# kaftanski/fissure-segmentation

Measured on AMD Instinct MI355X. Metric: points/sec fwd+bwd DGCNN-seg N=2048 k=20, higher is better.
Workload: dtype f32

## Files before the change

### fissure-segmentation_amd/_lib.py

```python
import ctypes
import os

import torch

_HERE = os.path.dirname(os.path.abspath(__file__))
LIB_PATH = os.environ.get("FSG_HIP_LIB") or os.path.join(_HERE, "libfsg_hip.so")

if not os.path.exists(LIB_PATH):
    raise ImportError(f"{LIB_PATH} not found: build it with `python -c 'import __graft_entry__ as g; g.build()'` "
                      f"or `make -C {os.path.join(_HERE, 'csrc')}`; there is no CPU fallback.")

lib = ctypes.CDLL(LIB_PATH)

_P, _I, _L, _F = ctypes.c_void_p, ctypes.c_int, ctypes.c_int64, ctypes.c_float
SIGNATURES = {
    "fsg_version": ([], _I),
    "fsg_last_error": ([], ctypes.c_char_p),
    "fsg_knn_dense_f32": ([_P, _I, _I, _L, _L, _I, _I, _I, _P, _P, _P, _P], _I),
    "fsg_knn_dense_workspace_bytes": ([_I, _I, _I], ctypes.c_size_t),
    "fsg_knn_dense_ws_f32": ([_P, _I, _I, _L, _L, _I, _I, _I, _P, _P, _P, ctypes.c_size_t, _P], _I),
    "fsg_knn_dense_prepared_f32": ([_P, _I, _I, _I, _I, _I, _P, _P, _P, ctypes.c_size_t, _P], _I),
    "fsg_knn_dense_ws_pq_f32": ([_P, _I, _I, _L, _L, _I, _I, _I, _P, _P, _P, ctypes.c_size_t, _P, _I, _P, _P], _I),
    "fsg_edgeconv_apply_f32": ([_P, _P, _P, _P, _P, _I, _I, _I, _F, _P, _P, _P, ctypes.c_size_t, _P], _I),
    "fsg_edgeconv_apply_pq_f32": ([_P, _P, _P, _P, _P, _I, _I, _I, _F, _P, _P, _P, ctypes.c_size_t, _P, _I, _P, _P], _I),
    "fsg_edge_gather_fwd_f32": ([_P, _P, _P, _I, _I, _I, _I, _P], _I),
    "fsg_edge_gather_bwd_f32": ([_P, _P, _P, _I, _I, _I, _I, _P], _I),
    "fsg_knn_gather_fused_f32": ([_P, _I, _I, _I, _I, _I, _P, _P, _P, _P], _I),
    "fsg_knn_gather_fused_ws_f32": ([_P, _I, _I, _I, _I, _I, _P, _P, _P, ctypes.c_size_t, _P], _I),
    "fsg_edge_gather_fwd_bf16": ([_P, _P, _P, _I, _I, _I, _I, _P], _I),
    "fsg_edge_gather_bwd_bf16": ([_P, _P, _P, _I, _I, _I, _I, _P], _I),
    "fsg_graph_reverse_csr_workspace_bytes": ([_I, _I, _I], ctypes.c_size_t),
    "fsg_graph_reverse_csr": ([_P, _I, _I, _I, _P, _P, _P, _P], _I),
    "fsg_edge_weights_fwd_f32": ([_P, _I, _I, _P, _P], _I),
    "fsg_edge_weights_bwd_f32": ([_P, _I, _I, _P, _P], _I),
    "fsg_edge_weights_many_f32": ([_P, _I, _P], _I),
    "fsg_edgeconv1_workspace_bytes": ([_I, _I, _I], ctypes.c_size_t),
    "fsg_edgeconv1_fwd_f32": ([_P, _P, _P, _P, _P, _P, _I, _I, _I, _I, _I, _F, _F, _F, _P, _P, _P, _P, _P, _P, _P, _P, _P],
                              _I),
    "fsg_edgeconv1_bwd_f32": ([_P, _P, _L, _P, _L, _P, _P, _P, _P, _P, _P, _P, _P, _P, _P, _I, _I, _I, _I, _I, _F, _P, _P,
                               _P, _P, _P, _P], _I),
    "fsg_edgeconv2_workspace_bytes": ([_I, _I, _I, _I], ctypes.c_size_t),
    "fsg_edgeconv2_bwd_workspace_bytes": ([_I, _I, _I, _I], ctypes.c_size_t),
    "fsg_edgeconv2_fwd_f32": ([_P] * 11 + [_I] * 5 + [_F] * 5 + [_P] * 12, _I),
    "fsg_edgeconv2_bwd_f32": ([_P, _P, _L, _P, _L] + [_P] * 16 + [_I] * 5 + [_F] + [_P] * 8, _I),
    "fsg_edgeconv2_fwd_bf16": ([_P] * 11 + [_I] * 5 + [_F] * 5 + [_P] * 12, _I),
    "fsg_edgeconv2_bwd_bf16": ([_P, _P, _L, _P, _L] + [_P] * 16 + [_I] * 5 + [_F] + [_P] * 8, _I),
    "fsg_bn_act_workspace_bytes": ([ctypes.c_long, _I], ctypes.c_size_t),
    "fsg_bn_act_fwd_f32": ([_P, _P, _P, _P, _P, ctypes.c_long, _I, _I, _F, _F, _F, _P, _P, _P, _P, _P], _I),
    "fsg_bn_act_bwd_f32": ([_P, _P, _P, _P, _P, _P, ctypes.c_long, _I, _I, _F, _P, _P, _P, _P, _P], _I),
    "fsg_bn_act_max_workspace_bytes": ([_I, _I, _I], ctypes.c_size_t),
    "fsg_bn_act_max_fwd_f32": ([_P, _P, _P, _P, _P, _I, _I, _I, _I, _F, _F, _F, _P, _P, _P, _P, _P, _P, _P], _I),
    "fsg_bn_act_max_bwd_f32": ([_P, _P, _P, _P, _P, _P, _P, _P, _I, _I, _I, _I, _F, _P, _P, _P, _P], _I),
    "fsg_bn_act_maxavg_workspace_bytes": ([_I, _I, _I], ctypes.c_size_t),
    "fsg_bn_act_maxavg_fwd_f32": ([_P, _P, _P, _P, _P, _I, _I, _I, _I, _F, _F, _F, _P, _P, _P, _P, _P, _P], _I),
    "fsg_bn_act_maxavg_bwd_f32": ([_P, _P, _P, _P, _P, _P, _P, _I, _I, _I, _I, _F, _P, _P, _P, _P, _P], _I),
    "fsg_chamfer_nn_f32": ([_P, _P, _I, _I, _I, _P, _P, _P], _I),
    "fsg_chamfer_nn_bwd_workspace_bytes": ([_I, _I, _I], ctypes.c_size_t),
    "fsg_chamfer_nn_bwd_f32": ([_P, _P, _P, _P, _I, _I, _I, _P, _P, _P, _P], _I),
    "fsg_point_mesh_dist_f32": ([_P, _P, _P, _I, _I, _I, _I, _I, _P, _P, _P, _P], _I),
    "fsg_mesh_labelmap_dist_f32": ([_P, _P, _P, _I, _I, _I, _I, _I, _F, _F, _F, _F, _P, _P, _P, _P], _I),
    "fsg_mesh_labelmap_cover_f32": ([_P, _P, _P, _I, _I, _I, _I, _I, _F, _F, _F, _P, _P], _I),
    "fsg_ensemble_accumulate_workspace_bytes": ([_I, _L], ctypes.c_size_t),
    "fsg_ensemble_accumulate_f32": ([_P, _I, _I, _I, _I, _P, _L, _P, _P, _P], _I),
    "fsg_sample_transform_f32": ([_P, _I, _I, _L, _P, _I, _P, _P, _P], _I),
    "fsg_ssm_decode_bwd_workspace_bytes": ([_I, _I, _I], ctypes.c_size_t),
    "fsg_ssm_decode_fwd_f32": ([_P, _P, _P, _P, _P, _P, _I, _I, _I, _P, _P], _I),
    "fsg_ssm_decode_bwd_f32": ([_P, _P, _P, _P, _P, _P, _I, _I, _I, _P, _P, _P, _P, _P, ctypes.c_size_t, _P], _I),
    "fsg_colsum_narrow_f32": ([_P, _L, _I, _P, _P], _I),
    "fsg_fold_layer1_f32": ([_P, _I, _P, _L, _P, _I, _I, _I, _I, _P, _P], _I),
    "fsg_adam_flat_f32": ([_P, _P, _P, _P, _P, _L, _F, _P, _F, _F, _F, _F, _P], _I),
    "fsg_nnu_loss_workspace_bytes": ([_I], ctypes.c_size_t),
    "fsg_nnu_loss_f32": ([_P, _L, _L, _L, _P, _P, _I, _I, _I, _F, _F, _F, _P, _P, _L, _L, _L, _P, _P], _I),
    "fsg_bn_rows_workspace_bytes": ([ctypes.c_long, _I], ctypes.c_size_t),
    "fsg_bn_rows_fwd_f32": ([_P, _P, _P, _P, _P, _P, ctypes.c_long, _I, _I, _F, _F, _I, _P, _P, _P, _P, _P], _I),
    "fsg_bn_rows_bwd_f32": ([_P, _P, _P, _P, _P, _P, ctypes.c_long, _I, _I, _I, _P, _P, _P, _P, _P, _P], _I),
    "fsg_gemm_small_workspace_bytes": ([_I, _I, _I], ctypes.c_size_t),
    "fsg_gemm_small_f32": ([_P, _L, _L, _P, _L, _L, _P, _P, _L, _I, _I, _I, _P, _P], _I),
    "fsg_gemm_small_rowsum_f32": ([_P, _L, _L, _P, _L, _L, _P, _P, _L, _I, _I, _I, _P, _P, _P], _I),
    "fsg_gemm_small_deferred_f32": ([_P, _L, _L, _P, _L, _L, _P, _L, _I, _I, _I, _P, _P, _P, _P], _I),
    "fsg_gemm_small_reduce_many_f32": ([_P, _P], _I),
    "fsg_gemm_small_bf16": ([_P, _L, _L, _P, _L, _L, _P, _P, _L, _I, _I, _I, _P, _P, _P, _P], _I),
    "fsg_pt_attn_workspace_bytes": ([_I, _I, _I], ctypes.c_size_t),
    "fsg_pt_attn_fwd_f32": ([_P, _P, _P, _P, _P, _L, _P, _I, _I, _I, _I, _P, _P, _P, _P, _P, _P], _I),
    "fsg_pt_attn_bwd_f32": ([_P, _P, _P, _P, _P, _L, _P, _I, _I, _I, _I, _P, _P, _P, _P, _P, _P, _P, _L, _P, _P, _P, _P], _I),
    "fsg_knn_segment_f32": ([_P, _P, _P, _P, _I, _I, _I, _I, _P, _P, _P], _I),
    "fsg_fps_f32": ([_P, _P, _P, _I, _I, _P, _P, _P], _I),
    "fsg_group_gather_fwd_f32": ([_P, _P, _P, _I, _I, _I, _I, _P], _I),
    "fsg_group_gather_bwd_f32": ([_P, _P, _P, _I, _I, _I, _I, _P], _I),
    "fsg_group_xyz_feat_fwd_f32": ([_P, _P, _P, _P, _P, _I, _I, _I, _I, _P], _I),
    "fsg_group_xyz_feat_bwd_f32": ([_P, _P, _P, _I, _I, _I, _I, _P], _I),
    "fsg_rows_max_fwd_f32": ([_P, _P, _P, _I, _I, _I, _P], _I),
    "fsg_rows_max_bwd_f32": ([_P, _P, _P, _I, _I, _I, _P], _I),
    "fsg_interp_fwd_f32": ([_P, _P, _P, _P, _I, _I, _I, _I, _P], _I),
    "fsg_interp_bwd_f32": ([_P, _P, _P, _P, _I, _I, _I, _I, _P], _I),
    "fsg_vec_attn_fwd_f32": ([_P, _P, _P, _P, _P, _I, _I, _I, _I, _P], _I),
    "fsg_vec_attn_bwd_f32": ([_P, _P, _P, _P, _P, _P, _P, _P, _I, _I, _I, _I, _P], _I),
    "fsg_pw_weight_image_bytes": ([_I, _I], ctypes.c_size_t),
    "fsg_pw_weight_image_f32": ([_P, _L, _L, _I, _I, _F, _I, _I, _P, _P], _I),
# ... 60 lines not shown
    "fsg_pcl_normals_f32": ([_P, _P, _P, _I, _I, _I, _I, _P, _P, _P, _P], _I),
    "fsg_orient_normals_workspace_bytes": ([_I, _I], ctypes.c_size_t),
    "fsg_orient_normals_f32": ([_P, _P, _P, _P, _I, _I, _I, _P, ctypes.c_size_t, _P, _P, _P, _P], _I),
    "fsg_face_union_i32": ([_P, _P, _I, _P, _P, _P], _I),
    "fsg_cluster_stats_f64": ([_P, _P, _P, _P, _P, _I, _I, _I, _P, _P, _P, _P], _I),
    "fsg_mesh_keep_flags_u8": ([_P, _I, _P, _I, _P, _P, _P, _I, _I, _I, _F, _F, _F, _P, _P], _I),
    "fsg_mesh_face_flags_u8": ([_P, _I, _I, _P, _P, _P, _P, _P], _I),
    "fsg_mesh_compact_f32": ([_P, _P, _P, _I, _I, _P, _I, _P, _P, _P, _P, _P, _P, _P, _P], _I),
}
for _name, (_args, _res) in SIGNATURES.items():
    _fn = getattr(lib, _name)
    _fn.argtypes, _fn.restype = _args, _res

GRID_TORCH, GRID_SAP = 0, 1
MORPH_MAX_RADIUS = 8
PCL_NORMALS_MAX_K = 64
ORIENT_MAX_POINTS = 1 << 20
RW_BINARY, RW_INTENSITY, RW_MAX_LABELS = 0, 1, 8
KNN_FIX_DIAG, KNN_DROP_FIRST, KNN_FORCE_ROWS, KNN_FORCE_MFMA, KNN_MAX_K = 1, 2, 4, 8, 64
KNN_DBG_HALF_CHUNKS, KNN_DBG_TWO_PHASE, KNN_DBG_ALL_SLOW, KNN_DBG_STATS = 1 << 11, 1 << 21, 1 << 22, 1 << 25
KNN_DBG_STAMPS, KNN_DBG_ONE_LAUNCH, KNN_DBG_BF16 = 1 << 28, 1 << 29, 1 << 30


_timing = None


def start_timing():
    global _timing
    _timing = {}


def stop_timing():
    global _timing
    rec, _timing = _timing, None
    torch.cuda.synchronize()
    return {name: [s.elapsed_time(e) for s, e in evs] for name, evs in (rec or {}).items()}


class PTLayerParams(ctypes.Structure):
    _fields_ = [(n, _P) for n in ("lp1_w", "lp1_b", "bnp_g", "bnp_b", "bnp_rm", "bnp_rv", "lp2_w", "lp2_b", "bn1_g", "bn1_b",
                                  "bn1_rm", "bn1_rv", "lw1_w", "lw1_b", "bn2_g", "bn2_b", "bn2_rm", "bn2_rv", "lw2_w",
                                  "lw2_b")] + [(n, _F) for n in ("eps_p", "eps_1", "eps_2", "mom_p", "mom_1", "mom_2")]


GEMM_REDUCE_MAX_JOBS = 48


class GemmReduceJobs(ctypes.Structure):
    _fields_ = [("part", _P * GEMM_REDUCE_MAX_JOBS), ("C", _P * GEMM_REDUCE_MAX_JOBS), ("rowsum", _P * GEMM_REDUCE_MAX_JOBS),
                ("ldc", _L * GEMM_REDUCE_MAX_JOBS), ("S", _I * GEMM_REDUCE_MAX_JOBS), ("I", _I * GEMM_REDUCE_MAX_JOBS),
                ("J", _I * GEMM_REDUCE_MAX_JOBS), ("blocks", _I * GEMM_REDUCE_MAX_JOBS), ("n", _I)]


class EdgeWeightJobs(ctypes.Structure):
    _fields_ = [("src", _P * 8), ("dst", _P * 8), ("Co", _I * 8), ("C", _I * 8), ("n", _I)]


class PWRowGemmArgs(ctypes.Structure):
    _fields_ = [("A1", _P), ("Y1", _P), ("A2", _P), ("lda1", _L), ("lda2", _L), ("K1", _I), ("K2", _I), ("Bimg", _P),
                ("M", _I), ("N", _I), ("rows_per_cloud", _I), ("alpha", _P), ("delta", _P), ("P", _P), ("Q", _P),
                ("tstride", _I), ("slope", _F), ("C", _P), ("ldc", _L), ("store_n0", _I), ("bias", _P), ("rec", _P),
                ("sgn", _P), ("sel_val", _P), ("sel_arg", _P), ("sel_n", _I), ("Yp", _P), ("ldyp", _L), ("ealpha", _P),
                ("edelta", _P), ("emu", _P), ("er", _P), ("etstride", _I), ("rec2", _P)]


PW_MAX_IMAGE_JOBS = 10


class PWImageJobs(ctypes.Structure):
    _fields_ = [("W", _P * PW_MAX_IMAGE_JOBS), ("stride_n", _L * PW_MAX_IMAGE_JOBS), ("stride_k", _L * PW_MAX_IMAGE_JOBS),
                ("N", _I * PW_MAX_IMAGE_JOBS), ("K", _I * PW_MAX_IMAGE_JOBS), ("ks0", _I * PW_MAX_IMAGE_JOBS),
                ("KS", _I * PW_MAX_IMAGE_JOBS), ("scale", _F * PW_MAX_IMAGE_JOBS), ("image", _P * PW_MAX_IMAGE_JOBS), ("n", _I)]


PW_MAX_REDUCE_JOBS = 6


class PWTnReduceJobs(ctypes.Structure):
    _fields_ = [("workspace", _P * PW_MAX_REDUCE_JOBS), ("C1", _P * PW_MAX_REDUCE_JOBS), ("C2", _P * PW_MAX_REDUCE_JOBS),
                ("ldc1", _L * PW_MAX_REDUCE_JOBS), ("ldc2", _L * PW_MAX_REDUCE_JOBS), ("S", _I * PW_MAX_REDUCE_JOBS),
                ("N1", _I * PW_MAX_REDUCE_JOBS), ("N2", _I * PW_MAX_REDUCE_JOBS), ("N1a", _I * PW_MAX_REDUCE_JOBS), ("n", _I)]


class PWTnArgs(ctypes.Structure):
    _fields_ = [("L1", _P), ("LY1", _P), ("L2", _P), ("ldl1", _L), ("ldl2", _L), ("N1a", _I), ("N1b", _I), ("lpro", _I),
                ("lalpha", _P), ("ldelta", _P), ("lP", _P), ("lQ", _P), ("lts", _I), ("R", _P), ("ldr", _L), ("N2", _I),
                ("rpro", _I), ("ralpha", _P), ("rdelta", _P), ("rts", _I), ("slope", _F), ("M", _I), ("rows_per_cloud", _I),
                ("rows_per_slice", _I), ("ones", _I)]


class PTLayerGrads(ctypes.Structure):
    _fields_ = [(n, _P) for n in ("lp1_w", "lp1_b", "bnp_g", "bnp_b", "lp2_w", "lp2_b", "bn1_g", "bn1_b", "lw1_w", "lw1_b",
                                  "bn2_g", "bn2_b", "lw2_w", "lw2_b")]


_experiments = None


def experiments():
    global _experiments
    if _experiments is None:
        path = os.path.join(_HERE, "libfsg_hip_experiments.so")
        if not os.path.exists(path):
            raise ImportError(f"{path} not found: `make -C {os.path.join(_HERE, 'csrc')} all` builds it")
        x = ctypes.CDLL(path)
        x.fsg_knn_experiment_f32.argtypes, x.fsg_knn_experiment_f32.restype = SIGNATURES["fsg_knn_dense_f32"][0], _I
# ... 22 lines not shown
```

### fissure-segmentation_amd/csrc/edgeconv.hip

```cpp
#include <type_traits>

#include "edgeconv_internal.h"
#include "knn_internal.h"

namespace {

constexpr int TP = 16;
constexpr int FSG_CSR_SPLIT = 16;
constexpr int TPW = 2;

__global__ __launch_bounds__(1024) void csr_build_kernel(const int32_t *__restrict__ idx, int N, int k,
                                                          int32_t *__restrict__ rowptr, int32_t *__restrict__ col) {
    extern __shared__ int sh[];
    int *hist = sh;
    int *part = sh + N;
    const int b = blockIdx.x, tid = threadIdx.x;
    const long NK = (long)N * k;
    const int32_t *ib = idx + b * NK;
    for (int j = tid; j < N; j += 1024) hist[j] = 0;
    __syncthreads();
    for (long e0 = tid; e0 < NK; e0 += 8 * 1024) {
        int dst[8];
#pragma unroll
        for (int u = 0; u < 8; ++u) dst[u] = (e0 + u * 1024 < NK) ? ib[e0 + u * 1024] : -1;
// ... 151 lines not shown
    for (long e = e0 + tid; e < e1; e += 1024) {
        const int pos = atomicAdd(&sh[ib[e]], 1);
        const int i = (int)(e / k), sl = (int)(e - (long)i * k);
        col[b * NK + pos] = (i << 6) | sl;
    }
}

constexpr int CSR_SORT_CAP = 1024;
__global__ __launch_bounds__(256) void csr_sort_rows_kernel(const int32_t *__restrict__ rowptr, int32_t *__restrict__ col, int N,
                                                            int NK, int32_t *__restrict__ tmp) {
    __shared__ int32_t buf[4][CSR_SORT_CAP];
    const int b = blockIdx.y, wave = __builtin_amdgcn_readfirstlane(threadIdx.x >> 6), lane = threadIdx.x & 63;
    const int j = blockIdx.x * 4 + wave;
    if (j >= N) return;
    const int32_t *rp = rowptr + (long)b * (N + 1);
    const int beg = rp[j], deg = rp[j + 1] - beg;
    if (deg < 2) return;
    int32_t *row = col + (long)b * NK + beg;
    if (deg > CSR_SORT_CAP) {
        if (!tmp) return;
        int32_t *cp = tmp + (long)b * NK + beg;
        for (int t = lane; t < deg; t += 64) cp[t] = row[t];
        __threadfence_block();
        __builtin_amdgcn_wave_barrier();
        for (int t0 = 0; t0 < deg; t0 += 64) {
            const int t = t0 + lane;
            const int32_t e = t < deg ? __builtin_nontemporal_load(cp + t) : 0x7fffffff;
            int rank = 0;
            for (int u = 0; u < deg; ++u) rank += __builtin_nontemporal_load(cp + u) < e ? 1 : 0;
            if (t < deg) row[rank] = e;
        }
        return;
    }
    int32_t *mine = buf[wave];
    for (int t = lane; t < deg; t += 64) mine[t] = row[t];
    __builtin_amdgcn_wave_barrier();
    for (int t0 = 0; t0 < deg; t0 += 64) {
        const int t = t0 + lane;
        const int32_t e = t < deg ? mine[t] : 0x7fffffff;
        int rank = 0;
#pragma unroll 8
        for (int u = 0; u < deg; ++u) rank += mine[u] < e ? 1 : 0;
        if (t < deg) row[rank] = e;
    }
}

template <bool SELECT>
__global__ __launch_bounds__(512) void ec1_stats_select_kernel(const float *__restrict__ pq,
                                                                const int32_t *__restrict__ idx,
                                                                const float *__restrict__ gamma, int N, int k, int Co,
                                                                int training, float *__restrict__ ysel,
                                                                uint8_t *__restrict__ arg, float *__restrict__ ssum,
                                                                float *__restrict__ partials) {
    typedef f32x2 f2;
    typedef f32x4 f4;
    typedef u32x4 u4;
    constexpr int NW = 4 * TPW;
    __shared__ float red[2][4 * NW][64];
    const int b = blockIdx.x, tile = blockIdx.y, cg = blockIdx.z;
    const int lane = threadIdx.x & 63, wave = __builtin_amdgcn_readfirstlane(threadIdx.x >> 6);
    const int g = lane >> 4, c16 = lane & 15;
    const int c0 = cg * 64 + 4 * c16;
    const int ld = 2 * Co;
    const __amdgpu_buffer_rsrc_t rs = buffer_rsrc(pq + (long)b * N * ld, __builtin_amdgcn_readfirstlane((int)((long)N * ld * 4)));
    f2 sgn[2] = {{1.f, 1.f}, {1.f, 1.f}};
    if (SELECT) {
        const f4 gm = *reinterpret_cast<const f4 *>(gamma + c0);
        sgn[0] = f2{gm[0] >= 0.f ? 1.f : -1.f, gm[1] >= 0.f ? 1.f : -1.f};
        sgn[1] = f2{gm[2] >= 0.f ? 1.f : -1.f, gm[3] >= 0.f ? 1.f : -1.f};
    }
    const int i = tile * TP * TPW + wave * (TP / 4) + g;
    const bool live = i < N;
    const int ic = live ? i : N - 1;
    int ids[4] = {0, 0, 0, 0};
#pragma unroll
    for (int r = 0; r < 4; ++r)
        if (16 * r < k) ids[r] = (16 * r + c16 < k) ? idx[((long)b * N + ic) * k + 16 * r + c16] : 0;
    const f4 q4 = __builtin_bit_cast(f4, __builtin_amdgcn_raw_buffer_load_b128(
        rs, (unsigned)ic * (unsigned)(ld * 4) + (unsigned)((Co + c0) * 4), 0, 0));
    const f2 q[2] = {{q4[0], q4[1]}, {q4[2], q4[3]}};
    f2 tot[2] = {{0.f, 0.f}, {0.f, 0.f}}, shift[2] = {{0.f, 0.f}, {0.f, 0.f}}, s1[2] = {{0.f, 0.f}, {0.f, 0.f}},
       s2[2] = {{0.f, 0.f}, {0.f, 0.f}};
    float best[4] = {-INFINITY, -INFINITY, -INFINITY, -INFINITY};
    int barg[4] = {0, 0, 0, 0};
    constexpr int RB = SELECT ? 8 : 10;
    auto request = [&](int s0, u4 (&y)[RB]) {
#pragma unroll
        for (int u = 0; u < RB; ++u) {
            const int s = min(s0 + u, k - 1);
            const int r = s >> 4;
            const int held = r == 0 ? ids[0] : (r == 1 ? ids[1] : (r == 2 ? ids[2] : ids[3]));
            const int j = __builtin_amdgcn_ds_bpermute(4 * ((lane & 48) | (s & 15)), held);
            y[u] = __builtin_amdgcn_raw_buffer_load_b128(rs, (unsigned)j * (unsigned)(ld * 4) + (unsigned)(c0 * 4), 0, 0);
        }
    };
    auto consume = [&](int s0, const u4 (&y)[RB]) {
#pragma unroll
        for (int u = 0; u < RB; ++u) {
            const int s = s0 + u;
            if (s < k) {
                const f4 yv = __builtin_bit_cast(f4, y[u]);
#pragma unroll
                for (int hf = 0; hf < 2; ++hf) {
                    const f2 yy = f2{yv[2 * hf], yv[2 * hf + 1]} + q[hf];
                    tot[hf] += yy;
                    if (training) {
                        if (s == 0) shift[hf] = yy;
                        const f2 d = yy - shift[hf];
                        s1[hf] += d;
                        s2[hf] = __builtin_elementwise_fma(d, d, s2[hf]);
                    }
                    if (SELECT) {
                        const f2 v = sgn[hf] * yy;
#pragma unroll
                        for (int e = 0; e < 2; ++e)
                            if (v[e] > best[2 * hf + e]) { best[2 * hf + e] = v[e]; barg[2 * hf + e] = s; }
                    }
                }
            }
        }
    };
    u4 ya[RB], yb[RB];
    request(0, ya);
    for (int s0 = 0; s0 < k; s0 += 2 * RB) {
        if (s0 + RB < k) request(s0 + RB, yb);
        consume(s0, ya);
        if (s0 + 2 * RB < k) request(s0 + 2 * RB, ya);
        if (s0 + RB < k) consume(s0 + RB, yb);
    }
    if (live) {
        const long o = ((long)b * N + i) * Co + c0;
        if (SELECT) {
            *reinterpret_cast<f4 *>(ysel + o) = f4{sgn[0][0] * best[0], sgn[0][1] * best[1], sgn[1][0] * best[2], sgn[1][1] * best[3]};
            *reinterpret_cast<unsigned *>(arg + o) =
                (unsigned)barg[0] | ((unsigned)barg[1] << 8) | ((unsigned)barg[2] << 16) | ((unsigned)barg[3] << 24);
        }
        if (ssum) *reinterpret_cast<f4 *>(ssum + o) = f4{tot[0][0], tot[0][1], tot[1][0], tot[1][1]};
    }
    if (!training) return;
#pragma unroll
    for (int e = 0; e < 4; ++e) {
        const float s1e = s1[e >> 1][e & 1], s2e = s2[e >> 1][e & 1], she = shift[e >> 1][e & 1];
        red[0][wave * 4 + g][4 * c16 + e] = she + s1e / (float)k;
        red[1][wave * 4 + g][4 * c16 + e] = fmaxf(s2e - s1e * s1e / (float)k, 0.f);
    }
    __syncthreads();
    if (wave == 0) {
        const int c = cg * 64 + lane;
        const int live_groups = min(4 * NW, max(0, N - tile * TP * TPW));
        float sm = 0.f, sM = 0.f;
#pragma unroll 8
        for (int w = 0; w < 4 * NW; ++w) {
            const bool on = w < live_groups;
            sm += on ? red[0][w][lane] : 0.f;
            sM += on ? red[1][w][lane] : 0.f;
        }
        const float mu = live_groups > 0 ? sm / (float)live_groups : 0.f;
        float dev = 0.f;
#pragma unroll 8
        for (int w = 0; w < 4 * NW; ++w) {
            const float d = red[0][w][lane] - mu;
            dev = __builtin_fmaf(w < live_groups ? d : 0.f, d, dev);
        }
        const long rec = (long)b * gridDim.y + tile;
        float *pr = partials + rec * 3 * Co;
        pr[c] = (float)live_groups * (float)k;
        pr[Co + c] = mu;
        pr[2 * Co + c] = sM + (float)k * dev;
    }
}

constexpr int FIN_S = 16;

constexpr int FIN_CH = 8, FIN_SL = 128;
__global__ __launch_bounds__(FIN_CH * FIN_SL) void bn_finalize_kernel(const float *__restrict__ partials, int R, int Co,
                                                                      float eps, float momentum,
                                                                      float *__restrict__ mean_out,
                                                                      float *__restrict__ invstd_out,
                                                                      float *__restrict__ running_mean,
                                                                      float *__restrict__ running_var) {
    __shared__ double red[3][FIN_SL][FIN_CH];
    const int ch = threadIdx.x & (FIN_CH - 1), sl = threadIdx.x / FIN_CH;
    const int c = blockIdx.x * FIN_CH + ch;
    double a = 0.0, bm = 0.0, cm = 0.0;
    for (int r0 = sl; r0 < R; r0 += 4 * FIN_SL) {
        float nv[4], mv[4], qv[4];
#pragma unroll
        for (int u = 0; u < 4; ++u) {
            const int r = min(r0 + u * FIN_SL, R - 1);
            const float *pr = partials + (long)r * 3 * Co + c;
            nv[u] = pr[0];
            mv[u] = pr[Co];
            qv[u] = pr[2 * Co];
        }
#pragma unroll
        for (int u = 0; u < 4; ++u)
            if (r0 + u * FIN_SL < R) {
                const double n = nv[u], mu = mv[u];
                a += n;
                bm += n * mu;
                cm += (double)qv[u] + n * mu * mu;
            }
    }
    red[0][sl][ch] = a;
    red[1][sl][ch] = bm;
    red[2][sl][ch] = cm;
    __syncthreads();
    __shared__ double red2[3][16][FIN_CH];
    if (sl < 16) {
        double x0 = 0.0, x1 = 0.0, x2 = 0.0;
#pragma unroll
        for (int u = 0; u < 8; ++u) {
            x0 += red[0][8 * sl + u][ch];
            x1 += red[1][8 * sl + u][ch];
            x2 += red[2][8 * sl + u][ch];
        }
        red2[0][sl][ch] = x0;
        red2[1][sl][ch] = x1;
        red2[2][sl][ch] = x2;
    }
    __syncthreads();
// ... 474 lines not shown
    const int j = blockIdx.y;
    const int Co = jobs.Co[j], C = jobs.C[j];
    const int t = blockIdx.x * 256 + threadIdx.x;
    if (t >= 2 * Co * C) return;
    const float *src = jobs.src[j];
    float *dst = jobs.dst[j];
    if (!backward) {
        const int r = t / C, c = t - r * C;
        dst[t] = r < Co ? src[(long)r * 2 * C + c] : src[(long)(r - Co) * 2 * C + C + c] - src[(long)(r - Co) * 2 * C + c];
    } else {
        const int r = t / (2 * C), c2 = t - r * 2 * C;
        dst[t] = c2 < C ? src[(long)r * C + c2] - src[(long)(Co + r) * C + c2] : src[(long)(Co + r) * C + (c2 - C)];
    }
}

extern "C" int fsg_edge_weights_many_f32(const fsg_edge_weight_jobs *jobs, int backward, fsg_stream_t stream) {
    FSG_REQUIRE(jobs && jobs->n >= 1 && jobs->n <= FSG_EDGE_WEIGHT_MAX_JOBS, "fsg_edge_weights_many_f32: 1..%d jobs",
                FSG_EDGE_WEIGHT_MAX_JOBS);
    long most = 0;
    for (int j = 0; j < jobs->n; ++j) {
        FSG_REQUIRE(jobs->src[j] && jobs->dst[j] && jobs->Co[j] > 0 && jobs->C[j] > 0, "fsg_edge_weights_many_f32: bad job %d", j);
        const long e = 2L * jobs->Co[j] * jobs->C[j];
        most = e > most ? e : most;
    }
    hipLaunchKernelGGL(edge_weights_many_kernel, dim3(fsg_cdiv(most, 256), jobs->n), dim3(256), 0, (hipStream_t)stream, *jobs,
                       backward);
    FSG_CHECK_LAUNCH("fsg_edge_weights_many_f32");
    return FSG_OK;
}

extern "C" int fsg_edge_weights_fwd_f32(const float *W, int Co, int C, float *Wt, fsg_stream_t stream) {
    FSG_REQUIRE(W && Wt && Co > 0 && C > 0, "fsg_edge_weights_fwd_f32: bad arguments");
    hipLaunchKernelGGL(edge_weights_fwd_kernel, dim3(fsg_cdiv(2L * Co * C, 256)), dim3(256), 0, (hipStream_t)stream, W, Co, C, Wt);
    FSG_CHECK_LAUNCH("fsg_edge_weights_fwd_f32");
    return FSG_OK;
}
extern "C" int fsg_edge_weights_bwd_f32(const float *grad_Wt, int Co, int C, float *grad_W, fsg_stream_t stream) {
    FSG_REQUIRE(grad_Wt && grad_W && Co > 0 && C > 0, "fsg_edge_weights_bwd_f32: bad arguments");
    hipLaunchKernelGGL(edge_weights_bwd_kernel, dim3(fsg_cdiv(2L * Co * C, 256)), dim3(256), 0, (hipStream_t)stream, grad_Wt, Co,
                       C, grad_W);
    FSG_CHECK_LAUNCH("fsg_edge_weights_bwd_f32");
    return FSG_OK;
}

extern "C" size_t fsg_edgeconv1_workspace_bytes(int B, int N, int Co) {
    const size_t rec = (size_t)B * (size_t)fsg_cdiv(N, TP * TPW);
    return sizeof(float) * (rec * 3 * (size_t)Co + fsg_ec_finalize_stage_floats(Co));
}

extern "C" int fsg_edgeconv1_fwd_f32(const float *pq, const int32_t *idx, const float *gamma, const float *beta,
                                     float *running_mean, float *running_var, int B, int N, int k, int Co, int training,
                                     float momentum, float eps, float slope, float *out, float *out_pm, float *ysel,
                                     uint8_t *arg, float *ssum, float *mean, float *invstd, float *workspace,
                                     fsg_stream_t stream) {
    FSG_REQUIRE(pq && idx && gamma && beta && ysel && arg && mean && invstd, "fsg_edgeconv1_fwd_f32: NULL pointer");
    FSG_REQUIRE(B > 0 && N > 0 && k > 0 && k <= 64 && Co > 0 && Co % 64 == 0 && B <= 65535,
                "fsg_edgeconv1_fwd_f32: bad shape B=%d N=%d k=%d Co=%d (Co must be a multiple of 64)", B, N, k, Co);
    FSG_REQUIRE(!training || workspace, "fsg_edgeconv1_fwd_f32: training needs the workspace");
    FSG_REQUIRE((long)N * 2 * Co * 4 < (1L << 31), "fsg_edgeconv1_fwd_f32: a cloud's [P | Q] rows must stay below 2 GiB (N=%d, Co=%d)", N, Co);
    hipStream_t st = (hipStream_t)stream;
    const int tiles = fsg_cdiv(N, TP * TPW);
    hipLaunchKernelGGL(ec1_stats_select_kernel<true>, dim3(B, tiles, Co / 64), dim3(256 * TPW), 0, st, pq, idx, gamma, N, k, Co,
                       training, ysel, arg, ssum, workspace);
    FSG_CHECK_LAUNCH("fsg_edgeconv1_fwd_f32/stats");
    if (training) {
        const int rc = fsg_ec_finalize_launch(workspace, B * tiles, Co, eps, momentum, mean, invstd, running_mean,
                                              running_var, st);
        if (rc != FSG_OK) return rc;
    }
    if (!out) return FSG_OK;
    hipLaunchKernelGGL(ec1_apply_kernel, dim3(B, fsg_cdiv(N, 64), Co / 64), dim3(256), 0, st, ysel, gamma, beta, mean,
                       invstd, N, Co, slope, out, out_pm);
    FSG_CHECK_LAUNCH("fsg_edgeconv1_fwd_f32/apply");
    return FSG_OK;
}

extern "C" int fsg_edgeconv_apply_f32(const float *ysel, const float *gamma, const float *beta, const float *mean,
                                      const float *invstd, int B, int N, int Co, float slope, float *out, float *out_pm,
                                      void *knn_workspace, size_t knn_workspace_bytes, fsg_stream_t stream) {
    FSG_REQUIRE(ysel && gamma && beta && mean && invstd && out, "fsg_edgeconv_apply_f32: NULL pointer");
    FSG_REQUIRE(B > 0 && N > 0 && Co > 0 && Co % 64 == 0 && B <= 65535, "fsg_edgeconv_apply_f32: bad shape B=%d N=%d Co=%d", B, N, Co);
    if (knn_workspace)
        return fsg_ec_apply_prep_launch(ysel, gamma, beta, mean, invstd, B, N, Co, slope, out, out_pm, knn_workspace,
                                        knn_workspace_bytes, nullptr, nullptr, (hipStream_t)stream);
    return fsg_ec_apply_launch(ysel, gamma, beta, mean, invstd, B, N, Co, slope, out, out_pm, (hipStream_t)stream);
}

extern "C" int fsg_edgeconv_apply_pq_f32(const float *ysel, const float *gamma, const float *beta, const float *mean,
                                         const float *invstd, int B, int N, int Co, float slope, float *out, float *out_pm,
                                         void *knn_workspace, size_t knn_workspace_bytes, const float *w_next, int rows_next,
                                         float *pq_next, fsg_stream_t stream) {
    FSG_REQUIRE(ysel && gamma && beta && mean && invstd && out && out_pm && knn_workspace && w_next && pq_next,
                "fsg_edgeconv_apply_pq_f32: NULL pointer");
    FSG_REQUIRE(B > 0 && N > 0 && Co == 64 && rows_next == 128 && B <= 65535,
                "fsg_edgeconv_apply_pq_f32: bad shape B=%d N=%d Co=%d rows_next=%d (Co must be 64, the next block 64 wide)", B, N, Co,
                rows_next);
    return fsg_ec_apply_prep_launch(ysel, gamma, beta, mean, invstd, B, N, Co, slope, out, out_pm, knn_workspace,
                                    knn_workspace_bytes, w_next, pq_next, (hipStream_t)stream);
}

extern "C" int fsg_edgeconv1_bwd_f32(const float *grad_out, const float *grad_out_pm, int64_t ld_pm, const float *grad_out_pm2,
                                     int64_t ld_pm2, const float *pq, const int32_t *rowptr, const int32_t *col,
                                     const float *gamma, const float *beta, const float *mean, const float *invstd,
                                     const float *ysel, const uint8_t *arg, const float *ssum, int B, int N, int k,
                                     int Co, int training, float slope, float *grad_pq, float *grad_gamma,
                                     float *grad_beta, float *h_scratch, float *workspace, fsg_stream_t stream) {
    FSG_REQUIRE((grad_out || grad_out_pm || grad_out_pm2) && pq && rowptr && col && gamma && beta && mean && invstd && ysel &&
                    arg && grad_pq && grad_gamma && grad_beta && h_scratch && workspace,
                "fsg_edgeconv1_bwd_f32: NULL pointer");
    FSG_REQUIRE((!grad_out_pm || ld_pm >= Co) && (!grad_out_pm2 || ld_pm2 >= Co),
                "fsg_edgeconv1_bwd_f32: row stride of a point-major gradient below Co=%d", Co);
    FSG_REQUIRE(!training || ssum, "fsg_edgeconv1_bwd_f32: training needs ssum");
    FSG_REQUIRE(B > 0 && N > 0 && k > 0 && k <= 64 && Co > 0 && Co % 64 == 0 && B <= 65535,
                "fsg_edgeconv1_bwd_f32: bad shape B=%d N=%d k=%d Co=%d", B, N, k, Co);
    hipStream_t st = (hipStream_t)stream;
    const int tiles64 = fsg_cdiv(N, 64);
    hipLaunchKernelGGL(ec1_bwd_point_kernel, dim3(B, tiles64, Co / 64), dim3(256), 0, st, grad_out, grad_out_pm, (long)ld_pm,
// ... 13 lines not shown
```

### fissure-segmentation_amd/csrc/edgeconv2.hip

```cpp

#include "edgeconv_internal.h"

namespace {

__device__ __forceinline__ bf16x8 pack8(const float (&v)[8]) {
    bf16x8 r;
#pragma unroll
    for (int i = 0; i < 8; ++i) r[i] = (__bf16)v[i];
    return r;
}

constexpr int C1 = 64;
constexpr int LD1 = C1 + 1;
constexpr int MAXPAIR = 3;

struct Tile {
    int TP, R, Rpad;
};

template <int C2, bool BF>
__global__ __launch_bounds__(256) void ec2_fwd_kernel(const float *__restrict__ pq, const int32_t *__restrict__ idx,
                                                       const float *__restrict__ w2, const float *__restrict__ gamma1,
                                                       const float *__restrict__ beta1, const float *__restrict__ mean1,
                                                       const float *__restrict__ invstd1,
// ... 1022 lines not shown
static void ec2s_tiling(int k, int B, int N, bool bwd, bool bf16, int &RT, int &TP, int &G) {
    const int tp2 = 64 / k, tp4 = 128 / k;
    const float u2 = tp2 * k / 64.f, u4 = tp4 * k / 128.f;
    RT = u4 > 1.15f * u2 ? 4 : 2;
    if (!bwd && !bf16) RT = 2;
    TP = RT == 4 ? tp4 : tp2;
    if (TP < 1) TP = 1;
    if (TP > 16) TP = 16;
    const int ntiles = (N + TP - 1) / TP;
    G = (bwd ? 512 : 768) / (B > 0 ? B : 1);
    if (G < 1) G = 1;
    if (G > ntiles) G = ntiles;
}

static size_t ec2s_fwd_lds(int NP, int RT, int TP) {
    return (size_t)NP * RT * 32 * 128 + sizeof(float) * ((size_t)RT * 32 * 65 + 3 * 4 * 64 + 2 * C1 + 2 * (size_t)TP * C1);
}
static size_t ec2s_bwd_lds(int NP, int RT, int TP) {
    return (size_t)2 * NP * RT * 32 * 128 +
           sizeof(float) * ((size_t)RT * 32 * (C1 + 4) + 2 * 64 + 64 + 2 * C1 + (size_t)TP * 64 * 2 + 2 * (size_t)TP * C1);
}

static void ec2_tiling(int k, int C2, int &TP, int &Rpad, int &G, int B, int N) {
    TP = 64 / k;
    if (TP < 1) TP = 1;
    Rpad = (TP * k + 31) & ~31;
    const int ntiles = (N + TP - 1) / TP;
    G = 1024 / (B > 0 ? B : 1);
    if (G < 1) G = 1;
    if (G > ntiles) G = ntiles;
}

extern "C" size_t fsg_edgeconv2_workspace_bytes(int B, int N, int k, int C2) {
    int TP, Rpad, G;
    ec2_tiling(k, C2, TP, Rpad, G, B, N);
    if (ec2_split(C2)) {
        int RT, TPs, Gs;
        ec2s_tiling(k, B, N, false, false, RT, TPs, Gs);
        { int RTb, TPb, Gb; ec2s_tiling(k, B, N, false, true, RTb, TPb, Gb); if (Gb > Gs) Gs = Gb; }
        if (Gs > G) G = Gs;
    }
    const size_t rec1 = (size_t)fsg_ec_stats1_records(B, N) * 3 * C1 + fsg_ec_finalize_stage_floats(C1);
    const size_t rec2 = (size_t)B * G * 3 * C2 + fsg_ec_finalize_stage_floats(C2);
    const size_t scratch1 = (size_t)B * N * C1 * sizeof(float) + (size_t)B * N * C1;
    return sizeof(float) * (rec1 + rec2) + scratch1 + 256;
}

static int ec2_fwd_impl(bool bf16, const float *pq, const int32_t *idx, const float *w2, const float *gamma1,
                                     const float *beta1, float *running_mean1, float *running_var1, const float *gamma2,
                                     const float *beta2, float *running_mean2, float *running_var2, int B, int N, int k,
                                     int C2, int training, float momentum1, float momentum2, float eps1, float eps2,
                                     float slope, float *out, float *out_pm, float *ssum1, float *mean1, float *invstd1,
                                     float *ysel2, uint8_t *arg2, float *ssum2, float *mean2, float *invstd2,
                                     void *workspace, fsg_stream_t stream) {
    FSG_REQUIRE(pq && idx && w2 && gamma1 && beta1 && gamma2 && beta2 && mean1 && invstd1 && ysel2 && arg2 &&
                    mean2 && invstd2 && workspace,
                "fsg_edgeconv2_fwd_f32: NULL pointer");
    FSG_REQUIRE(B > 0 && N > 0 && N <= (1 << 21) && k > 0 && k <= 64 && (C2 == 64 || C2 == 128) && B <= 65535,
                "fsg_edgeconv2_fwd_f32: bad shape B=%d N=%d k=%d C2=%d (layer widths 64 -> 64|128 only, N <= 2^21)", B, N, k, C2);
    FSG_REQUIRE(!training || (ssum1 && ssum2), "fsg_edgeconv2_fwd_f32: training needs ssum1/ssum2");
    hipStream_t st = (hipStream_t)stream;
    int TP, Rpad, G;
    ec2_tiling(k, C2, TP, Rpad, G, B, N);
    int RTs = 0, TPs = 0, Gs = 0, Gws = G;
    if (ec2_split(C2)) {
        ec2s_tiling(k, B, N, false, bf16, RTs, TPs, Gs);
        if (Gs > Gws) Gws = Gs;
    }
    const int rec1 = fsg_ec_stats1_records(B, N);
    float *part1 = (float *)workspace;
    float *part2 = part1 + (size_t)rec1 * 3 * C1 + fsg_ec_finalize_stage_floats(C1);
    float *ysel1 = part2 + (size_t)B * Gws * 3 * C2 + fsg_ec_finalize_stage_floats(C2);
    uint8_t *arg1 = (uint8_t *)(ysel1 + (size_t)B * N * C1);
    int rc;
    if (training) {
        if ((rc = fsg_ec_stats1_launch(pq, idx, gamma1, B, N, k, C1, ysel1, arg1, ssum1, part1, st)) != FSG_OK) return rc;
        if ((rc = fsg_ec_finalize_launch(part1, rec1, C1, eps1, momentum1, mean1, invstd1, running_mean1, running_var1,
                                         st)) != FSG_OK)
            return rc;
    }
    const size_t lds = sizeof(float) * ((size_t)C2 * LD1 + (size_t)Rpad * (C2 + 1) + 3 * 4 * C2);
#define FSG_EC2_FWD(CC, BFX)                                                                                             \
    do {                                                                                                                 \
        FSG_GRANT_LDS("fsg_edgeconv2_fwd", (ec2_fwd_kernel<CC, BFX>), FSG_LDS_WHOLE_CU);                             \
        hipLaunchKernelGGL((ec2_fwd_kernel<CC, BFX>), dim3(B, G), dim3(256), lds, st, pq, idx, w2, gamma1, beta1, mean1,    \
                           invstd1, gamma2, N, k, TP, Rpad, training, slope, ysel2, arg2, ssum2, part2);                 \
    } while (0)
#define FSG_EC2S_FWD(NPX, RTX)                                                                                            \
    do {                                                                                                                 \
        FSG_GRANT_LDS("fsg_edgeconv2_fwd", (ec2s_fwd_kernel<NPX, RTX>), FSG_LDS_WHOLE_CU);                           \
        hipLaunchKernelGGL((ec2s_fwd_kernel<NPX, RTX>), dim3(B, G), dim3(256), ec2s_fwd_lds(NPX, RTX, TPs), st, pq, idx, w2,    \
                           gamma1, beta1, mean1, invstd1, gamma2, N, k, TPs, training, slope, ysel2, arg2, ssum2, part2); \
    } while (0)
    if (ec2_split(C2)) {
        G = Gs;
        if (bf16) { if (RTs == 4) FSG_EC2S_FWD(1, 4); else FSG_EC2S_FWD(1, 2); }
        else { if (RTs == 4) FSG_EC2S_FWD(3, 4); else FSG_EC2S_FWD(3, 2); }
    } else if (C2 == 64) { if (bf16) FSG_EC2_FWD(64, true); else FSG_EC2_FWD(64, false); }
    else { if (bf16) FSG_EC2_FWD(128, true); else FSG_EC2_FWD(128, false); }
#undef FSG_EC2_FWD
#undef FSG_EC2S_FWD
    FSG_CHECK_LAUNCH("fsg_edgeconv2_fwd_f32/mlp");
    if (training) {
        if ((rc = fsg_ec_finalize_launch(part2, B * G, C2, eps2, momentum2, mean2, invstd2, running_mean2, running_var2,
                                         st)) != FSG_OK)
            return rc;
    }
    if (!out) return FSG_OK;
    return fsg_ec_apply_launch(ysel2, gamma2, beta2, mean2, invstd2, B, N, C2, slope, out, out_pm, st);
}

extern "C" int fsg_edgeconv2_fwd_f32(const float *pq, const int32_t *idx, const float *w2, const float *gamma1,
                                     const float *beta1, float *running_mean1, float *running_var1, const float *gamma2,
                                     const float *beta2, float *running_mean2, float *running_var2, int B, int N, int k,
                                     int C2, int training, float momentum1, float momentum2, float eps1, float eps2,
                                     float slope, float *out, float *out_pm, float *ssum1, float *mean1, float *invstd1,
                                     float *ysel2, uint8_t *arg2, float *ssum2, float *mean2, float *invstd2,
                                     void *workspace, fsg_stream_t stream) {
    return ec2_fwd_impl(false, pq, idx, w2, gamma1, beta1, running_mean1, running_var1, gamma2, beta2, running_mean2, running_var2, B, N, k, C2, training, momentum1, momentum2, eps1, eps2, slope, out, out_pm, ssum1, mean1, invstd1, ysel2, arg2, ssum2, mean2, invstd2, workspace, stream);
}

extern "C" int fsg_edgeconv2_fwd_bf16(const float *pq, const int32_t *idx, const float *w2, const float *gamma1,
                                     const float *beta1, float *running_mean1, float *running_var1, const float *gamma2,
                                     const float *beta2, float *running_mean2, float *running_var2, int B, int N, int k,
                                     int C2, int training, float momentum1, float momentum2, float eps1, float eps2,
                                     float slope, float *out, float *out_pm, float *ssum1, float *mean1, float *invstd1,
                                     float *ysel2, uint8_t *arg2, float *ssum2, float *mean2, float *invstd2,
                                     void *workspace, fsg_stream_t stream) {
    return ec2_fwd_impl(true, pq, idx, w2, gamma1, beta1, running_mean1, running_var1, gamma2, beta2, running_mean2, running_var2, B, N, k, C2, training, momentum1, momentum2, eps1, eps2, slope, out, out_pm, ssum1, mean1, invstd1, ysel2, arg2, ssum2, mean2, invstd2, workspace, stream);
}

static void ec2_bwd_tiling(int k, int C2, int &TP, int &Rpad, int &G, int B, int N) {
    TP = 64 / k;
    if (TP < 1) TP = 1;
    Rpad = (TP * k + 31) & ~31;
    const int ntiles = (N + TP - 1) / TP;
    G = 768 / (B > 0 ? B : 1);
    if (G < 1) G = 1;
    if (G > ntiles) G = ntiles;
}

extern "C" size_t fsg_edgeconv2_bwd_workspace_bytes(int B, int N, int k, int C2) {
    int TP, Rpad, G;
    ec2_bwd_tiling(k, C2, TP, Rpad, G, B, N);
    if (ec2_split(C2)) {
        int RT, TPs, Gs;
        ec2s_tiling(k, B, N, true, false, RT, TPs, Gs);
        if (Gs > G) G = Gs;
    }
    const size_t point_rec = (size_t)B * fsg_cdiv(N, 64) * 2 * C2;
    const size_t dw = (size_t)B * G * C2 * C1, p1 = (size_t)B * G * 2 * C1;
    const size_t du = (size_t)B * N * k * C1;
    return sizeof(float) * (point_rec + dw + p1 + du + (size_t)B * N * C2) + 256;
}

static int ec2_bwd_impl(bool bf16, const float *grad_out, const float *grad_out_pm, int64_t ld_pm, const float *grad_out_pm2,
                                     int64_t ld_pm2, const float *pq, const int32_t *idx,
                                     const int32_t *rowptr, const int32_t *col, const float *w2, const float *gamma1,
                                     const float *beta1, const float *mean1, const float *invstd1, const float *ssum1,
                                     const float *gamma2, const float *beta2, const float *mean2, const float *invstd2,
                                     const float *ysel2, const uint8_t *arg2, int B, int N, int k, int C2, int training,
                                     float slope, float *grad_pq, float *grad_w2, float *grad_gamma1, float *grad_beta1,
                                     float *grad_gamma2, float *grad_beta2, void *workspace, fsg_stream_t stream) {
    FSG_REQUIRE((!grad_out_pm || ld_pm >= C2) && (!grad_out_pm2 || ld_pm2 >= C2),
                "fsg_edgeconv2_bwd_f32: row stride of a point-major gradient below C2=%d", C2);
    FSG_REQUIRE((grad_out || grad_out_pm || grad_out_pm2) && pq && idx && rowptr && col && w2 && gamma1 && beta1 && mean1 && invstd1 &&
                    gamma2 && beta2 && mean2 && invstd2 && ysel2 && arg2 && grad_pq && grad_w2 && grad_gamma1 &&
                    grad_beta1 && grad_gamma2 && grad_beta2 && workspace,
                "fsg_edgeconv2_bwd_f32: NULL pointer");
    FSG_REQUIRE(!training || ssum1, "fsg_edgeconv2_bwd_f32: training needs ssum1");
    FSG_REQUIRE(B > 0 && N > 0 && N <= (1 << 21) && k > 0 && k <= 64 && (C2 == 64 || C2 == 128) && B <= 65535,
                "fsg_edgeconv2_bwd_f32: bad shape B=%d N=%d k=%d C2=%d (N <= 2^21)", B, N, k, C2);
    hipStream_t st = (hipStream_t)stream;
    int TP, Rpad, G;
    ec2_bwd_tiling(k, C2, TP, Rpad, G, B, N);
    int RTs = 0, TPs = 0, Gs = 0, Gws = G;
    if (ec2_split(C2)) {
        ec2s_tiling(k, B, N, true, bf16, RTs, TPs, Gs);
        if (Gs > Gws) Gws = Gs;
    }
    float *point_part = (float *)workspace;
    float *dw_part = point_part + (size_t)B * fsg_cdiv(N, 64) * 2 * C2;
// ... 65 lines not shown
```

### fissure-segmentation_amd/csrc/edgeconv_internal.h

```cpp
#pragma once
#include "fsg_common.h"

int fsg_ec_stats1_records(int B, int N);
int fsg_ec_stats1_launch(const float *pq, const int32_t *idx, const float *gamma, int B, int N, int k, int Co,
                         float *ysel, uint8_t *arg, float *ssum, float *partials, hipStream_t st);
int fsg_ec_apply_launch(const float *ysel, const float *gamma, const float *beta, const float *mean, const float *invstd,
                        int B, int N, int Co, float slope, float *out, float *out_pm, hipStream_t st);
int fsg_ec_apply_prep_launch(const float *ysel, const float *gamma, const float *beta, const float *mean, const float *invstd,
                             int B, int N, int Co, float slope, float *out, float *out_pm, void *knn_ws, size_t knn_ws_bytes,
                             const float *w_next, float *pq_next, hipStream_t st);
int fsg_ec_bwd_point_launch(const float *gout, const float *gout_pm, long ld_pm, const float *gout_pm2, long ld_pm2,
                            const float *ysel, const float *gamma, const float *beta, const float *mean, const float *invstd,
                            int B, int N, int Co, float slope, float *h, float *partials, float *dbeta, float *dgamma,
                            hipStream_t st);

size_t fsg_ec_finalize_stage_floats(int Co);
int fsg_ec_finalize_launch(const float *partials, int R, int Co, float eps, float momentum, float *mean, float *invstd,
                           float *running_mean, float *running_var, hipStream_t st);
int fsg_ec_sum_launch(const float *partials, int R, int L, int nvec, float *out0, float *out1, hipStream_t st);

int fsg_csr_bipartite_launch(const int32_t *idx, int B, int NS, int N, int k, int32_t *rowptr, int32_t *col, int32_t *cnt,
                             int32_t *tmp, hipStream_t st);
```

### fissure-segmentation_amd/csrc/knn_dense.hip

```cpp
#include <float.h>

#include <stdlib.h>

#include <type_traits>

#include "knn_internal.h"

namespace {

constexpr int BLOCK = 256;

template <int QB>
__global__ __launch_bounds__(BLOCK) void knn_dense_rows_kernel(
    const float *__restrict__ x, int N, int Npad, long sb, long sc, int c_knn, int k, int flags,
    int32_t *__restrict__ idx_out, float *__restrict__ dist_out) {
    extern __shared__ __attribute__((aligned(16))) float smem[];
    float *qv = smem;
    float *xxq = qv + c_knn * QB;
    float *rows = smem + (((c_knn * QB + QB) + 3) & ~3);

    const int b = blockIdx.y;
    const int q0 = blockIdx.x * QB;
    const int tid = threadIdx.x;
    const float *xb = x + (long)b * sb;
// ... 54 lines not shown
                if (v.z < bd) { bd = v.z; bj = j + 2; }
                if (v.w < bd) { bd = v.w; bj = j + 3; }
            }
#pragma unroll
            for (int off = 32; off >= 1; off >>= 1) {
                const float od = __shfl_xor(bd, off);
                const int oj = __shfl_xor(bj, off);
                if (od < bd || (od == bd && oj < bj)) { bd = od; bj = oj; }
            }
            if (lane == 0) {
                if (bj < N) row[bj] = INFINITY;
                if (r >= drop) {
                    const long o = ((long)b * N + qg) * k + (r - drop);
                    idx_out[o] = bj < N ? bj : 0;
                    if (dist_out) dist_out[o] = bd;
                }
            }
            __builtin_amdgcn_wave_barrier();
        }
    }
}

}

extern "C" size_t fsg_knn_dense_workspace_bytes(int B, int N, int c_knn) {
    if (B <= 0 || N <= 0 || c_knn <= 0) return 0;
    const size_t xxb = sizeof(float) * (size_t)B * N, sp = fsg_knn_split_workspace_bytes(B, N, c_knn);
    return sp > xxb ? sp : xxb;
}

extern "C" int fsg_knn_dense_ws_f32(const float *x, int B, int N, int64_t stride_b, int64_t stride_c, int c_knn, int k,
                                    int flags, int32_t *idx_out, float *dist_out, void *workspace,
                                    size_t workspace_bytes, fsg_stream_t stream) {
    const int drop = (flags & FSG_KNN_DROP_FIRST) ? 1 : 0;
    FSG_KNN_REQUIRE_FLAGS("fsg_knn_dense_ws_f32", flags);
    FSG_REQUIRE(x && idx_out, "fsg_knn_dense_ws_f32: NULL pointer");
    FSG_REQUIRE(B >= 0 && N > 0 && c_knn > 0, "fsg_knn_dense_ws_f32: bad shape B=%d N=%d c_knn=%d", B, N, c_knn);
    FSG_REQUIRE(k >= 1 && k + drop <= N && k + drop <= FSG_KNN_MAX_K,
                "fsg_knn_dense_ws_f32: need 1 <= k and k+drop <= min(N, %d); got k=%d N=%d", FSG_KNN_MAX_K, k, N);
    FSG_REQUIRE(workspace == nullptr || workspace_bytes >= sizeof(float) * (size_t)B * N,
                "fsg_knn_dense_ws_f32: workspace of %zu bytes is smaller than the (B,N) squared norms", workspace_bytes);
    if (B == 0) return FSG_OK;
    if (workspace && !(flags & KNN_BYPASS_SPLIT)) {
        const int rc = fsg_knn_split_launch(x, B, N, stride_b, stride_c, c_knn, k, flags, idx_out, dist_out, workspace,
                                            workspace_bytes, (hipStream_t)stream);
        if (rc != FSG_ERR_UNSUPPORTED) return rc;
    }
    return fsg_knn_dense_f32(x, B, N, stride_b, stride_c, c_knn, k, flags & ~KNN_DBG_TWO_PHASE, idx_out, dist_out,
                             static_cast<float *>(workspace), stream);
}

extern "C" int fsg_knn_dense_ws_pq_f32(const float *x, int B, int N, int64_t stride_b, int64_t stride_c, int c_knn, int k,
                                       int flags, int32_t *idx_out, float *dist_out, void *workspace, size_t workspace_bytes,
                                       const float *w_pq, int rows_pq, float *pq_out, fsg_stream_t stream) {
    FSG_KNN_REQUIRE_FLAGS("fsg_knn_dense_ws_pq_f32", flags);
    FSG_REQUIRE(x && idx_out && w_pq && pq_out, "fsg_knn_dense_ws_pq_f32: NULL pointer");
    FSG_REQUIRE(c_knn >= 1 && c_knn <= 4 && rows_pq >= 1 && 256 % rows_pq == 0,
                "fsg_knn_dense_ws_pq_f32: needs 1 <= c_knn <= 4 and rows_pq dividing 256; got c_knn=%d rows_pq=%d", c_knn, rows_pq);
    const int drop = (flags & FSG_KNN_DROP_FIRST) ? 1 : 0;
    FSG_REQUIRE(B >= 0 && N > 0 && k >= 1 && k + drop <= N && k + drop <= FSG_KNN_MAX_K, "fsg_knn_dense_ws_pq_f32: bad shape B=%d N=%d k=%d",
                B, N, k);
    if (B == 0) return FSG_OK;
    hipStream_t st = (hipStream_t)stream;
    if (workspace && !(flags & KNN_BYPASS_SPLIT)) {
        bool fused = false;
        KnnSplitOpts o;
        o.pq_w = w_pq, o.pq_rows = rows_pq, o.pq_out = pq_out, o.pq_fused = &fused;
        const int rc = fsg_knn_split_launch(x, B, N, stride_b, stride_c, c_knn, k, flags, idx_out, dist_out, workspace, workspace_bytes,
                                            st, o);
        if (rc == FSG_OK) return fused ? FSG_OK : fsg_knn_pq_rows_launch(x, B, N, stride_b, stride_c, c_knn, w_pq, rows_pq, pq_out, st);
        if (rc != FSG_ERR_UNSUPPORTED) return rc;
    }
    const int rc = fsg_knn_dense_ws_f32(x, B, N, stride_b, stride_c, c_knn, k, flags, idx_out, dist_out, workspace, workspace_bytes,
                                        stream);
    if (rc != FSG_OK) return rc;
    return fsg_knn_pq_rows_launch(x, B, N, stride_b, stride_c, c_knn, w_pq, rows_pq, pq_out, st);
}

extern "C" int fsg_knn_dense_prepared_f32(const float *x_pm, int B, int N, int c_knn, int k, int flags, int32_t *idx_out,
                                          float *dist_out, void *workspace, size_t workspace_bytes, fsg_stream_t stream) {
    const int drop = (flags & FSG_KNN_DROP_FIRST) ? 1 : 0;
    FSG_KNN_REQUIRE_FLAGS("fsg_knn_dense_prepared_f32", flags);
    FSG_REQUIRE(x_pm && idx_out && workspace, "fsg_knn_dense_prepared_f32: NULL pointer");
    FSG_REQUIRE(B > 0 && N > 0 && c_knn > 0 && k >= 1 && k + drop <= N && k + drop <= FSG_KNN_MAX_K,
                "fsg_knn_dense_prepared_f32: bad shape B=%d N=%d c_knn=%d k=%d", B, N, c_knn, k);
    KnnSplitOpts o;
    o.prepared_xt = x_pm;
    const int rc = fsg_knn_split_launch(nullptr, B, N, 0, 0, c_knn, k, flags, idx_out, dist_out, workspace, workspace_bytes,
                                        (hipStream_t)stream, o);
    if (rc == FSG_ERR_UNSUPPORTED) fsg_set_error("fsg_knn_dense_prepared_f32: shape outside the prepared path's envelope");
    return rc;
}

extern "C" int fsg_knn_dense_f32(const float *x, int B, int N, int64_t stride_b, int64_t stride_c,
                                 int c_knn, int k, int flags, int32_t *idx_out, float *dist_out,
                                 float *xx_scratch, fsg_stream_t stream) {
    const int drop = (flags & FSG_KNN_DROP_FIRST) ? 1 : 0;
    FSG_KNN_REQUIRE_FLAGS("fsg_knn_dense_f32", flags);
    FSG_REQUIRE(x && idx_out, "fsg_knn_dense_f32: NULL pointer");
    FSG_REQUIRE(B >= 0 && N > 0 && c_knn > 0, "fsg_knn_dense_f32: bad shape B=%d N=%d c_knn=%d", B, N, c_knn);
    FSG_REQUIRE(k >= 1 && k + drop <= N && k + drop <= FSG_KNN_MAX_K,
                "fsg_knn_dense_f32: need 1 <= k and k+drop <= min(N, %d); got k=%d N=%d", FSG_KNN_MAX_K, k, N);
    FSG_REQUIRE(N <= 32768, "fsg_knn_dense_f32: N=%d > 32768 unsupported", N);
    if (B == 0) return FSG_OK;
    hipStream_t st = (hipStream_t)stream;
    FSG_REQUIRE(!(flags & FSG_KNN_FORCE_MFMA),
                "fsg_knn_dense_f32: flags %d select an experimental kernel: call fsg_knn_experiment_f32 of "
                "libfsg_hip_experiments.so", flags);
    if (!(flags & FSG_KNN_FORCE_ROWS)) {
        const int rc = fsg_knn_rows_mfma_launch(x, B, N, stride_b, stride_c, c_knn, k, flags, idx_out, dist_out, xx_scratch, st);
        if (rc != FSG_ERR_UNSUPPORTED) return rc;
    }
    const int Npad = (N + 255) & ~255;
    auto launch = [&](auto qb) -> int {
        constexpr int QB = decltype(qb)::value;
        const auto kern = knn_dense_rows_kernel<QB>;
        const size_t lds = sizeof(float) * ((((size_t)c_knn * QB + QB + 3) & ~(size_t)3) + (size_t)QB * Npad);
        if (lds > 160 * 1024) {
            fsg_set_error("fsg_knn_dense_f32: LDS need %zu B > 160 KiB (N=%d c_knn=%d)", lds, N, c_knn);
            return FSG_ERR_UNSUPPORTED;
        }
        FSG_GRANT_LDS("fsg_knn_dense_f32", kern, lds);
        dim3 grid(fsg_cdiv(N, QB), B);
        hipLaunchKernelGGL(kern, grid, dim3(BLOCK), lds, st, x, N, Npad, (long)stride_b, (long)stride_c, c_knn, k,
                           flags, idx_out, dist_out);
        FSG_CHECK_LAUNCH("fsg_knn_dense_f32");
        return FSG_OK;
    };
    if (N <= 4096) return launch(std::integral_constant<int, 8>{});
    if (N <= 8192) return launch(std::integral_constant<int, 4>{});
    if (N <= 16384) return launch(std::integral_constant<int, 2>{});
    return launch(std::integral_constant<int, 1>{});
}
```

### fissure-segmentation_amd/csrc/knn_internal.h

```cpp
#pragma once
#include "fsg_common.h"

enum : int {
    KNN_DBG_HALF_CHUNKS = 1 << 11,
    KNN_DBG_TWO_PHASE = 1 << 21,
    KNN_DBG_ALL_SLOW = 1 << 22,
    KNN_DBG_STATS = 1 << 25,
    KNN_DBG_STAMPS = 1 << 28,
    KNN_DBG_ONE_LAUNCH = 1 << 29,
    KNN_DBG_BF16 = 1 << 30,
};
constexpr int KNN_FLAGS_ALL = FSG_KNN_FIX_DIAG | FSG_KNN_DROP_FIRST | FSG_KNN_FORCE_ROWS | FSG_KNN_FORCE_MFMA | KNN_DBG_HALF_CHUNKS |
                              KNN_DBG_TWO_PHASE | KNN_DBG_ALL_SLOW | KNN_DBG_STATS | KNN_DBG_STAMPS | KNN_DBG_ONE_LAUNCH | KNN_DBG_BF16;
constexpr int KNN_BYPASS_SPLIT = KNN_DBG_TWO_PHASE | FSG_KNN_FORCE_ROWS | FSG_KNN_FORCE_MFMA | KNN_DBG_HALF_CHUNKS;

#define FSG_KNN_REQUIRE_FLAGS(entry, flags) \
    FSG_REQUIRE(!((flags) & ~KNN_FLAGS_ALL), "%s: unknown flag bit(s) %u (a removed debug bit?)", entry, (unsigned)((flags) & ~KNN_FLAGS_ALL))

int fsg_knn_rows_mfma_launch(const float *x, int B, int N, int64_t stride_b, int64_t stride_c, int c_knn, int k, int flags,
                             int32_t *idx_out, float *dist_out, float *xx_scratch, hipStream_t st);
int fsg_knn_segment_rows_launch(const float *xyz, const float *new_xyz, const int32_t *offset, const int32_t *new_offset,
                                int b, int n, int m, int nsample, int32_t *idx, float *dist2, hipStream_t st);
int fsg_knn_mfma_launch(const float *x, int B, int N, int64_t stride_b, int64_t stride_c, int c_knn, int k, int flags,
                        int32_t *idx_out, float *dist_out, float *xx_scratch, hipStream_t st);

struct KnnSplitOpts {
    const float *prepared_xt = nullptr;
    const float *pq_w = nullptr;
    int pq_rows = 0;
    float *pq_out = nullptr;
    bool *pq_fused = nullptr;
};
size_t fsg_knn_split_workspace_bytes(int B, int N, int c_knn);
int fsg_knn_split_launch(const float *x, int B, int N, int64_t stride_b, int64_t stride_c, int c_knn, int k, int flags,
                         int32_t *idx_out, float *dist_out, void *ws, size_t ws_bytes, hipStream_t st, const KnnSplitOpts &o = {});
int fsg_knn_pq_rows_launch(const float *x, int B, int N, int64_t stride_b, int64_t stride_c, int c_knn, const float *pq_w,
                           int pq_rows, float *pq_out, hipStream_t st);
int fsg_knn_split_ws_pointers(void *ws, size_t ws_bytes, int B, int N, int c_knn, float **xx, float **xs, void **cand,
                              float **cscale);

#ifdef __HIPCC__
template <int WGS, int WPG, int SLOTS>
__device__ __forceinline__ void knn_stamp(unsigned long long *buf, bool on, int wave, int lane, int i) {
    if (on) {
        const unsigned wg = blockIdx.x + gridDim.x * blockIdx.y;
        const unsigned long long t = __builtin_amdgcn_s_memtime();
        if (wg < WGS && lane == 0) buf[(wg * WPG + wave) * SLOTS + i] = t;
    }
}
#endif
```

### fissure-segmentation_amd/csrc/knn_split.hip

```cpp
#include <type_traits>

#include "knn_internal.h"

__device__ unsigned long long fsg_knn_split_stats[4];
extern "C" int fsg_debug_knn_split_stats(unsigned long long *out, int reset) {
    if (hipMemcpyFromSymbol(out, HIP_SYMBOL(fsg_knn_split_stats), sizeof(fsg_knn_split_stats)) != hipSuccess) return 1;
    if (reset) {
        unsigned long long z[4] = {0, 0, 0, 0};
        if (hipMemcpyToSymbol(HIP_SYMBOL(fsg_knn_split_stats), z, sizeof(z)) != hipSuccess) return 1;
    }
    return 0;
}

__device__ unsigned long long fsg_knn_split_stamps[256 * 8 * 16];
extern "C" int fsg_debug_knn_split_stamps(unsigned long long *out) {
    return hipMemcpyFromSymbol(out, HIP_SYMBOL(fsg_knn_split_stamps), sizeof(fsg_knn_split_stamps)) != hipSuccess;
}

namespace {

constexpr int QB = 64;
constexpr int WAVES = 8;
constexpr int MSL = 4;
constexpr int NMIN = 2 * WAVES * MSL;

template <int KS, bool PACK, bool HALF>
__global__ __launch_bounds__(256) void knn_split_prep_kernel(const float *__restrict__ x, int N, int Np, long sb, long sc,
                                                             int c_knn, float *__restrict__ xx, float *__restrict__ xt,
                                                             u32x4 *__restrict__ cand, float *__restrict__ xs,
                                                             float *__restrict__ cscale) {
    constexpr int CP = PACK ? 4 : 16 * KS;
    __shared__ float slab[CP][33];
    __shared__ float mu[CP < 64 ? 64 : CP], wred[4];
    const int tid = threadIdx.x, b = blockIdx.y, tile = blockIdx.x, j0 = tile * 32;
    const float *xb = x + (long)b * sb;
    {
        const int pt = tid & 31;
#pragma unroll
        for (int c = tid >> 5; c < CP; c += 8)
            slab[c][pt] = (c < c_knn && j0 + pt < N) ? xb[c * sc + j0 + pt] : 0.f;
    }
    float sigma = 1.f;
    if (HALF) {
        const int sp = tid & 63, w = tid >> 6;
        const int pos = min((int)(((long)(sp >> 4) * N / 4) & ~15L), N - 16) + (sp & 15);
        constexpr int NR = CP <= 64 ? 16 : CP / 4;
        float sv[NR];
#pragma unroll
        for (int r = 0; r < NR; ++r) sv[r] = (w + 4 * r) < c_knn ? xb[(long)(w + 4 * r) * sc + pos] : 0.f;
        float dv = 0.f;
#pragma unroll
        for (int r = 0; r < NR; ++r) {
            const float m = wave_sum_bcast_f(sv[r]) * (1.0f / 64.0f);
            if (sp == 0) mu[w + 4 * r] = m;
// ... 1187 lines not shown
        f32x4 qraw = {0.f, 0.f, 0.f, 0.f};
        if (RAW) qraw = raw_row(q0 + q, xq);
        else xq = xxb[q0 + q];
        __syncthreads();
        for (int j = tid; j < N; j += WAVES * 64) {
            const float *row = xtb + (long)j * CP;
            float dot = 0.f, xj = 0.f;
            if (RAW) {
                const f32x4 v = raw_row(j, xj);
#pragma unroll
                for (int e = 0; e < 4; ++e) dot = __builtin_fmaf(qraw[e], v[e], dot);
            } else {
#pragma unroll 4
                for (int c4 = 0; c4 < CP / 4; ++c4) {
                    const f32x4 v = *reinterpret_cast<const f32x4 *>(row + 4 * c4);
                    const f32x4 qv = *reinterpret_cast<const f32x4 *>(qr + 4 * c4);
#pragma unroll
                    for (int e = 0; e < 4; ++e) dot = __builtin_fmaf(qv[e], v[e], dot);
                }
                xj = xxb[j];
            }
            const float tt = xq - 2.0f * dot;
            float d = tt + xj;
            if (fix_diag && j == q0 + q) d = 0.f;
            dl[j] = d;
        }
        __syncthreads();
        if (wave == 0) {
            u64 last = 0;
            const long ob = ((long)b * N + q0 + q) * k - drop;
            for (int r = 0; r < KK; ++r) {
                u64 best = ~0ull;
                for (int j = lane; j < N; j += 64) {
                    const u64 kj = ((u64)f2o(dl[j]) << 32) | (unsigned)j;
                    if ((r == 0 || kj > last) && kj < best) best = kj;
                }
#pragma unroll
                for (int off = 32; off >= 1; off >>= 1) {
                    const u64 o = __shfl_xor(best, off);
                    best = o < best ? o : best;
                }
                last = best;
                if (lane == 0 && r >= drop) {
                    idx_out[ob + r] = (int)(unsigned)(best & 0xFFFFFFFFull);
                    if (dist_out) dist_out[ob + r] = o2f((unsigned)(best >> 32));
                }
            }
        }
    }
}

constexpr int RQW = 8;
constexpr int RECAP = 256;
template <int CP>
__global__ __launch_bounds__(128) void knn_refine_kernel(const float *__restrict__ xx, const float *__restrict__ xt,
                                                         const unsigned *__restrict__ bmg, int N, int Np, int TS, int k,
                                                         int flags, int PCAP, int32_t *__restrict__ idx_out,
                                                         float *__restrict__ dist_out) {
    constexpr int QW = RQW, ECAP = RECAP, RW = 2;
    constexpr int CPQ = CP + 4;
    constexpr bool STAGE = CP > 4;
    constexpr int CS = CP > 32 ? 32 : CP;
    constexpr int NSLAB = CP / CS;
    constexpr int CSQ = CS + 4;
    constexpr int LS = STAGE ? CS / 4 : 1;
    constexpr int RPI = 64 / LS;
    constexpr int NI = STAGE ? 64 / RPI : 1;
    extern __shared__ __attribute__((aligned(16))) unsigned char smem[];
    const int tid = threadIdx.x, lane = tid & 63, wave = __builtin_amdgcn_readfirstlane(tid >> 6);
    constexpr size_t wbytes = (size_t)8 * ECAP + (STAGE ? (size_t)4 * 64 * CSQ : 0) + (size_t)4 * QW * CPQ + 128;
    u64 *keys = reinterpret_cast<u64 *>(smem + wave * wbytes);
    unsigned *klo = reinterpret_cast<unsigned *>(keys);
    float *stg = reinterpret_cast<float *>(keys + ECAP);
    float *qrows = stg + (STAGE ? 64 * CSQ : 0);
    int *seg = reinterpret_cast<int *>(qrows + QW * CPQ);
    unsigned *dump = reinterpret_cast<unsigned *>(seg + 2 * QW);
    const bool stamps = (flags & KNN_DBG_STAMPS) != 0;
    auto stamp = [&](int i) { knn_stamp<512, RW, 8>(fsg_knn_refine_stamps, stamps, wave, lane, i); };
    stamp(0);
    int b = blockIdx.y, qw0 = blockIdx.x * RW * QW;
    {
        const unsigned L = blockIdx.x + gridDim.x * blockIdx.y, total = gridDim.x * gridDim.y;
        if ((total & 7u) == 0) {
            const unsigned V = (L & 7u) * (total >> 3) + (L >> 3);
            b = (int)(V / gridDim.x);
            qw0 = (int)(V % gridDim.x) * RW * QW;
        }
    }
    const int drop = (flags & FSG_KNN_DROP_FIRST) ? 1 : 0;
    const int KK = k + drop;
    const bool fix_diag = (flags & FSG_KNN_FIX_DIAG) != 0;
    const float *xxb = xx + (long)b * Np;
    const float *xtb = xt + (long)b * Np * CP;
    const int qbeg = qw0 + wave * QW;
    if (qbeg >= N) return;
    const int qi = lane >> 3, l8 = lane & 7;
    const int NCH = (TS + 63) >> 6;
    const unsigned *brow = bmg + ((long)b * Np + qbeg + qi) * TS + 8 * l8;

    u32x4 wa = {0u, 0u, 0u, 0u}, wb = wa;
    auto load_chunk = [&](int ch, u32x4 &a, u32x4 &c) {
        a = u32x4{0u, 0u, 0u, 0u};
        c = a;
        if (64 * ch + 8 * l8 < TS) {
            a = *reinterpret_cast<const u32x4 *>(brow + 64 * ch);
            c = *reinterpret_cast<const u32x4 *>(brow + 64 * ch + 4);
        }
    };
    auto popc8 = [](const u32x4 &a, const u32x4 &c) {
        return __popc(a[0]) + __popc(a[1]) + __popc(a[2]) + __popc(a[3]) + __popc(c[0]) + __popc(c[1]) + __popc(c[2]) + __popc(c[3]);
    };
    auto sum8 = [](int c) {
        c += dpp_mov0<0xB1, 0xf, true>(c);
        c += dpp_mov0<0x4E, 0xf, true>(c);
        c += dpp_mov0<0x141, 0xf, true>(c);
        return c;
    };
    load_chunk(0, wa, wb);
    {
        constexpr int LQ = CP / 4;
        constexpr int RQ = 64 / LQ > QW ? QW : 64 / LQ;
#pragma unroll
        for (int r0 = 0; r0 < QW; r0 += RQ) {
            const int r = r0 + lane / LQ, c = lane % LQ;
            if (lane < RQ * LQ && r < QW)
                *reinterpret_cast<f32x4 *>(qrows + r * CPQ + 4 * c) =
                    *reinterpret_cast<const f32x4 *>(xtb + (long)min(qbeg + r, Np - 1) * CP + 4 * c);
        }
        if (lane < QW) qrows[lane * CPQ + CP] = xxb[min(qbeg + lane, Np - 1)];
    }
    int tq = popc8(wa, wb);
    for (int ch = 1; ch < NCH; ++ch) {
        u32x4 a, c;
        load_chunk(ch, a, c);
        tq += popc8(a, c);
    }
    tq = sum8(tq);
    const bool qvalid = qbeg + qi < N && tq >= KK && tq <= PCAP;
    const int tqv = qvalid ? tq : 0;
    const int tq2 = (tqv + 1) & ~1;
    int totu[QW];
#pragma unroll
    for (int u = 0; u < QW; ++u) totu[u] = __builtin_amdgcn_readlane(tq2, 8 * u);
    constexpr unsigned PADF = 0x80000000u;
    stamp(1);

    int qa = 0;
    while (qa < QW) {
// ... 124 lines not shown
            }
            if (sl == NSLAB - 1 && p < E) {
                const int jc = (int)(ent & 0xFFFFu);
                const float tt = qr[CP] - 2.0f * dot;
                float d = tt + xc;
                if (fix_diag && jc == qbeg + (int)((ent >> 16) & 7u)) d = 0.f;
                keys[p] = (ent & PADF) ? ~0ull : (((u64)f2o(d) << 32) | ent);
            }
            __builtin_amdgcn_sched_barrier(0);
            __builtin_amdgcn_wave_barrier();
        };
        using S0 = std::integral_constant<int, 0>;
        using S1 = std::integral_constant<int, 1>;
        if (NT > 0) issue(S0{}, 0);
        if (NT > 1) issue(S1{}, 1);
        for (int t = 0; t < NT; t += 2) {
            step(S0{}, t);
            if (t + 1 < NT) step(S1{}, t + 1);
        }
        __builtin_amdgcn_wave_barrier();
        if (qa == 0) stamp(3);
        {
            u64 key[4];
            int sb[4], se[4], r[4];
#pragma unroll
            for (int m = 0; m < 4; ++m) {
                const int p = 64 * m + lane;
                key[m] = keys[min(p, ECAP - 1)];
                const int tg = (int)(((unsigned)key[m] >> 16) & 7u);
                const bool ok = p < E;
                sb[m] = ok ? seg[2 * tg] : 0;
                se[m] = ok ? seg[2 * tg + 1] : 0;
                r[m] = 0;
            }
            for (int it = 0; it < maxlen; it += 2) {
                u32x4 kk[4];
#pragma unroll
                for (int m = 0; m < 4; ++m) kk[m] = *reinterpret_cast<const u32x4 *>(keys + sb[m] + it);
#pragma unroll
                for (int m = 0; m < 4; ++m) {
                    const u64 k0 = ((u64)kk[m][1] << 32) | kk[m][0], k1 = ((u64)kk[m][3] << 32) | kk[m][2];
                    const int c2 = (k0 < key[m] ? 1 : 0) + (k1 < key[m] ? 1 : 0);
                    r[m] += sb[m] + it < se[m] ? c2 : 0;
                }
            }
#pragma unroll
            for (int m = 0; m < 4; ++m) {
                const int p = 64 * m + lane;
                if (p < E && r[m] >= drop && r[m] < KK && !((unsigned)key[m] & PADF)) {
                    const int tg = (int)(((unsigned)key[m] >> 16) & 7u);
                    const long o = ((long)b * N + qbeg + tg) * k - drop + r[m];
                    idx_out[o] = (int)((unsigned)key[m] & 0xFFFFu);
                    if (dist_out) dist_out[o] = o2f((unsigned)(key[m] >> 32));
                }
            }
        }
        __builtin_amdgcn_wave_barrier();
        if (qa == 0) stamp(4);
        qa = qb;
    }
    stamp(5);
}


size_t align256(size_t v) { return (v + 255) & ~(size_t)255; }

struct SplitPlan {
    bool ok;
    int KS, CP, Np;
    bool pack;
    size_t off_xx, off_xt, off_cand, off_xs, off_scale, off_bm, total;
};

SplitPlan plan(int B, int N, int c_knn) {
    SplitPlan p{};
    p.ok = N >= 1024 && N <= (c_knn > 64 ? 4096 : 8192) && c_knn >= 1 && c_knn <= 128;
    p.pack = c_knn <= 4;
    p.KS = p.pack ? 1 : (c_knn <= 16 ? 1 : (c_knn <= 32 ? 2 : (c_knn <= 64 ? 4 : 8)));
    p.CP = p.pack ? 4 : 16 * p.KS;
    p.Np = (N + 63) & ~63;
    const size_t T = p.Np / 32, opt = p.pack ? 1 : (p.KS == 8 ? 8 : 2 * p.KS);
    p.off_xx = 0;
    p.off_xt = align256(sizeof(float) * (size_t)B * p.Np);
    p.off_cand = p.off_xt + align256(sizeof(float) * (size_t)B * p.Np * p.CP);
    p.off_xs = p.off_cand + align256((size_t)B * T * opt * 1024);
    p.off_scale = p.off_xs + align256(sizeof(float) * (size_t)B * p.Np);
    p.off_bm = p.off_scale + align256(sizeof(float) * (size_t)B);
    p.total = p.off_bm + align256(sizeof(unsigned) * (size_t)B * p.Np * ((T + 7) & ~(size_t)7));
    return p;
}

}

size_t fsg_knn_split_workspace_bytes(int B, int N, int c_knn) {
    const SplitPlan p = plan(B, N, c_knn);
    return p.ok ? p.total : 0;
}

int fsg_knn_split_ws_pointers(void *ws, size_t ws_bytes, int B, int N, int c_knn, float **xx, float **xs, void **cand,
                              float **cscale) {
    const SplitPlan p = plan(B, N, c_knn);
    if (!p.ok || p.pack || ws == nullptr || ws_bytes < p.total || p.Np != N) return FSG_ERR_UNSUPPORTED;
    unsigned char *w = static_cast<unsigned char *>(ws);
    *xx = reinterpret_cast<float *>(w + p.off_xx);
    *cand = w + p.off_cand;
    *xs = reinterpret_cast<float *>(w + p.off_xs);
    *cscale = reinterpret_cast<float *>(w + p.off_scale);
    return FSG_OK;
}


namespace {

struct SplitArgs {
    SplitPlan p;
    const float *x;
    bool prepared;
    int B, N;
    long sb, sc;
    int c_knn, k, flags;
    int32_t *idx_out;
    float *dist_out;
    float *xx, *xt;
    u32x4 *cand;
    float *xs, *cscale;
    unsigned *bmg;
    hipStream_t st;
};

template <int KS, bool PK, bool HF>
void launch_prep(const SplitArgs &a) {
    if (a.prepared) return;
    hipLaunchKernelGGL((knn_split_prep_kernel<KS, PK, HF>), dim3(a.p.Np / 32, a.B), dim3(256), 0, a.st, a.x, a.N, a.p.Np, a.sb, a.sc,
                       a.c_knn, a.xx, a.xt, a.cand, a.xs, a.cscale);
}

template <int KS, bool PK, bool HF>
int launch_monolithic(const SplitArgs &a) {
    const SplitPlan &p = a.p;
    const size_t T = p.Np / 32, CPQ = p.CP + 4, PR = p.CP > 64 ? 16 : 48;
    size_t bmb = 4 * ((QB * (T + 1) + 1) & ~(size_t)1);
    if (bmb < (size_t)4 * QB * NMIN) bmb = (size_t)4 * QB * NMIN;
    size_t usz = sizeof(float) * p.Np + bmb;
    if (usz < 4 * (size_t)WAVES * PR * CPQ) usz = 4 * (size_t)WAVES * PR * CPQ;
    const size_t fixed = ((usz + 15) & ~(size_t)15) + sizeof(float) * QB * CPQ + sizeof(float) * QB + sizeof(int) * QB +
                         sizeof(float) * 24 + sizeof(int) * WAVES * (QB / WAVES) * 2;
    int PC = 512;
    while (PC >= 256 && fixed + 8 * (size_t)WAVES * PC > 160 * 1024) PC /= 2;
    if (PC < 256) return FSG_ERR_UNSUPPORTED;
    const size_t lds = fixed + 8 * (size_t)WAVES * PC;
    FSG_GRANT_LDS("fsg_knn_dense_ws_f32", (knn_split_kernel<KS, PK, HF>), 160 * 1024);
    launch_prep<KS, PK, HF>(a);
    hipLaunchKernelGGL((knn_split_kernel<KS, PK, HF>), dim3(p.Np / 64, a.B), dim3(WAVES * 64), lds, a.st, a.xx, a.xt, a.cand, a.xs,
                       a.cscale, a.N, p.Np, a.k, a.flags, PC, a.idx_out, a.dist_out);
    FSG_CHECK_LAUNCH("fsg_knn_dense_ws_f32/split-monolithic");
    return FSG_OK;
}

template <int KS, bool PK, bool HF, bool RES, bool RAW>
int launch_nominate(const SplitArgs &a, size_t lds, int PCAP, int TS, const RawPoints &raw) {
    FSG_GRANT_LDS("fsg_knn_dense_ws_f32", (knn_nominate_kernel<KS, PK, HF, RES, RAW>), lds);
    hipLaunchKernelGGL((knn_nominate_kernel<KS, PK, HF, RES, RAW>), dim3(a.p.Np / 64, a.B), dim3(WAVES * 64), lds, a.st, a.xx, a.xt,
                       a.cand, a.xs, a.cscale, a.N, a.p.Np, a.k, a.flags, PCAP, a.bmg, TS, a.idx_out, a.dist_out, raw);
    return FSG_OK;
}

template <int KS, bool PK, bool HF>
int launch_pair(const SplitArgs &a, const KnnSplitOpts &o) {
    const SplitPlan &p = a.p;
    const size_t T = p.Np / 32, CPQ = p.CP + 4;
    size_t bmw = (QB * (T + 1) + 3) & ~(size_t)3;
    if (bmw < (size_t)QB * NMIN) bmw = (size_t)QB * NMIN;
    const size_t lds1 = sizeof(float) * 32 * WAVES * ((T + WAVES - 1) / WAVES) + 4 * bmw + sizeof(float) * QB + sizeof(unsigned) * 4 + sizeof(float) * 24;
    const int PCAP = 256, TS = (int)((T + 7) & ~(size_t)7);
    const size_t CS = p.CP > 32 ? 32 : p.CP;
    const size_t lds2 = 2 * ((size_t)8 * RECAP + (p.CP > 4 ? 4 * 64 * (CS + 4) : 0) + 4 * (size_t)RQW * CPQ + 128);
    if (lds1 > 160 * 1024 || lds2 > 64 * 1024) return FSG_ERR_UNSUPPORTED;
    const bool res = T == 64;
    constexpr bool RES_OK = (HF && KS <= 4) || PK;
    const bool raw_ok = PK && res && !a.prepared && p.Np == a.N && a.sb % 4 == 0 && a.sc % 4 == 0 &&
                        (reinterpret_cast<uintptr_t>(a.x) & 15) == 0;
    int rc;
    if constexpr (PK) {
        if (raw_ok) {
            if (o.pq_out && (WAVES * 64) % o.pq_rows != 0) return FSG_ERR_UNSUPPORTED;
            if (o.pq_fused) *o.pq_fused = o.pq_out != nullptr;
            const RawPoints raw{a.x, a.sb, a.sc, a.c_knn, a.xx, a.xt, o.pq_w, o.pq_rows, o.pq_out};
            rc = launch_nominate<1, true, false, true, true>(a, lds1, PCAP, TS, raw);
        }
    }
    if (!raw_ok) {
        launch_prep<KS, PK, HF>(a);
        rc = res && RES_OK ? launch_nominate<KS, PK, HF, RES_OK, false>(a, lds1, PCAP, TS, RawPoints{})
                           : launch_nominate<KS, PK, HF, false, false>(a, lds1, PCAP, TS, RawPoints{});
    }
    if (rc != FSG_OK) return rc;
    hipLaunchKernelGGL((knn_refine_kernel<(PK ? 4 : 16 * KS)>), dim3(p.Np / (2 * RQW), a.B), dim3(128), lds2, a.st, a.xx, a.xt, a.bmg,
                       a.N, p.Np, TS, a.k, a.flags, PCAP, a.idx_out, a.dist_out);
    FSG_CHECK_LAUNCH("fsg_knn_dense_ws_f32/split");
    return FSG_OK;
}

}

int fsg_knn_pq_rows_launch(const float *x, int B, int N, int64_t stride_b, int64_t stride_c, int c_knn, const float *pq_w,
                           int pq_rows, float *pq_out, hipStream_t st) {
    if (c_knn < 1 || c_knn > 4 || pq_rows < 1 || 256 % pq_rows != 0) return FSG_ERR_UNSUPPORTED;
    const RawPoints raw{x, (long)stride_b, (long)stride_c, c_knn, nullptr, nullptr, pq_w, pq_rows, pq_out};
    hipLaunchKernelGGL(knn_pq_rows_kernel, dim3(fsg_cdiv(N, 64), B), dim3(256), 0, st, raw, N);
    FSG_CHECK_LAUNCH("fsg_knn_dense_ws_pq_f32/rows");
    return FSG_OK;
}

int fsg_knn_split_launch(const float *x, int B, int N, int64_t stride_b, int64_t stride_c, int c_knn, int k, int flags,
                         int32_t *idx_out, float *dist_out, void *ws, size_t ws_bytes, hipStream_t st, const KnnSplitOpts &o) {
    if (o.pq_fused) *o.pq_fused = false;
    const int drop = (flags & FSG_KNN_DROP_FIRST) ? 1 : 0;
    const bool bf16 = (flags & KNN_DBG_BF16) != 0;
    const SplitPlan p = plan(B, N, c_knn);
    if (!p.ok || k + drop > 64 || ws == nullptr || ws_bytes < p.total) return FSG_ERR_UNSUPPORTED;
    if (o.prepared_xt && (p.pack || p.CP != c_knn || p.Np != N || bf16)) return FSG_ERR_UNSUPPORTED;
    if (p.KS == 8 && bf16) return FSG_ERR_UNSUPPORTED;
    unsigned char *w = static_cast<unsigned char *>(ws);
    const SplitArgs a{p, x, o.prepared_xt != nullptr, B, N, (long)stride_b, (long)stride_c, c_knn, k, flags, idx_out, dist_out,
                      reinterpret_cast<float *>(w + p.off_xx),
                      o.prepared_xt ? const_cast<float *>(o.prepared_xt) : reinterpret_cast<float *>(w + p.off_xt),
                      reinterpret_cast<u32x4 *>(w + p.off_cand), reinterpret_cast<float *>(w + p.off_xs),
                      reinterpret_cast<float *>(w + p.off_scale), reinterpret_cast<unsigned *>(w + p.off_bm), st};
    const bool mono = (flags & KNN_DBG_ONE_LAUNCH) || (k + drop > 32 && p.CP >= 64 && N > 4096 && !(flags & KNN_DBG_STAMPS));
    auto form = [&](auto ks, auto pk, auto hf) {
        constexpr int KS = decltype(ks)::value;
        constexpr bool PK = decltype(pk)::value, HF = decltype(hf)::value;
        return mono ? launch_monolithic<KS, PK, HF>(a) : launch_pair<KS, PK, HF>(a, o);
    };
    using std::integral_constant;
    const std::true_type yes;
    const std::false_type no;
    if (p.pack) return form(integral_constant<int, 1>{}, yes, no);
    if (bf16) {
        if (p.KS == 1) return form(integral_constant<int, 1>{}, no, no);
        if (p.KS == 2) return form(integral_constant<int, 2>{}, no, no);
        return form(integral_constant<int, 4>{}, no, no);
    }
    if (p.KS == 1) return form(integral_constant<int, 1>{}, no, yes);
    if (p.KS == 2) return form(integral_constant<int, 2>{}, no, yes);
    if (p.KS == 4) return form(integral_constant<int, 4>{}, no, yes);
    return form(integral_constant<int, 8>{}, no, yes);
}
```

### fissure-segmentation_amd/functional.py

```python
import contextlib as _contextlib
import ctypes
import os as _os

import torch

from . import _lib


def _need_gpu(*tensors):
    for t in tensors:
        if t is not None and not t.is_cuda:
            raise RuntimeError("fissure_segmentation_amd runs on the GPU only (got a CPU tensor); "
                               "the CPU restatement lives in oracle/ and is test infrastructure")


def _p(t):
    return ctypes.c_void_p(t.data_ptr() if t is not None else 0)


def _stream():
    return ctypes.c_void_p(torch.cuda.current_stream().cuda_stream)


def _f32c(t):
# ... 5 lines not shown


def _amp_bwd(fn):
    return torch.amp.custom_bwd(fn, device_type="cuda")


def no_autocast():
    if torch.is_autocast_enabled("cuda"):
        return torch.autocast("cuda", enabled=False)
    return _contextlib.nullcontext()


_mfma_mode = "f32"


def set_mfma_operands(kind):
    global _mfma_mode
    if kind not in ("f32", "bf16"):
        raise ValueError("MFMA operand type must be 'f32' or 'bf16'")
    _mfma_mode = kind


@_contextlib.contextmanager
def mfma_operands(kind):
    global _mfma_mode
    old = _mfma_mode
    set_mfma_operands(kind)
    try:
        yield
    finally:
        _mfma_mode = old


def bf16_operands():
    return _mfma_mode == "bf16"


def _ambient_bf16():
    return torch.is_autocast_enabled("cuda") and torch.get_autocast_dtype("cuda") == torch.bfloat16


_deterministic = bool(_os.environ.get("FSG_DETERMINISTIC"))


def set_deterministic(flag=True):
    global _deterministic
    _deterministic = bool(flag)


def deterministic():
    return _deterministic or torch.are_deterministic_algorithms_enabled()


def knn_graph(x, k, c_knn=None, fix_diag=True, drop_first=False, return_dist=False, force_rows_kernel=False,
              _debug_flags=0, out=None, prepared=None, pq_weight=None):
    _need_gpu(x)
    if x.dim() != 3:
        raise ValueError(f"expected (B,C,N), got {tuple(x.shape)}")
    x = x.detach()
    if x.dtype != torch.float32:
        x = x.float()
    if x.stride(2) != 1:
        x = x.contiguous()
    B, C, N = x.shape
    c_knn = C if c_knn is None else c_knn
    if out is not None:
        if out.shape != (B, N, k) or out.dtype != torch.int32 or not out.is_contiguous() or out.device != x.device:
            raise ValueError("knn_graph: `out` must be a contiguous (B,N,k) int32 tensor on the input's device")
        idx = out
    else:
        idx = torch.empty(B, N, k, dtype=torch.int32, device=x.device)
    dist = torch.empty(B, N, k, dtype=torch.float32, device=x.device) if return_dist else None
    flags = (_lib.KNN_FIX_DIAG if fix_diag else 0) | (_lib.KNN_DROP_FIRST if drop_first else 0) | \
        (_lib.KNN_FORCE_ROWS if force_rows_kernel else 0) | _debug_flags
    if prepared is not None and c_knn == C and not return_dist and not force_rows_kernel and not _debug_flags:
        ws, x_pm = prepared
        with torch.cuda.device(x.device):
            _lib.call("fsg_knn_dense_prepared_f32", _p(x_pm), B, N, C, k, flags, _p(idx), None, _p(ws), ws.numel() * ws.element_size(),
                      _stream())
        return idx
    xx = _lib.workspace("fsg_knn_dense", B, N, c_knn, device=x.device)
    ws_bytes = xx.numel() if xx is not None else 0
    if pq_weight is not None:
        rows = pq_weight.shape[0]
        if (C == c_knn and c_knn <= 4 and tuple(pq_weight.shape) == (rows, C) and 256 % rows == 0 and not return_dist and
                not (_debug_flags & _lib.KNN_FORCE_MFMA)):
            pq = torch.empty(B, N, rows, dtype=torch.float32, device=x.device)
            with torch.cuda.device(x.device):
                _lib.call("fsg_knn_dense_ws_pq_f32", _p(x), B, N, x.stride(0), x.stride(1), c_knn, k, flags, _p(idx), None, _p(xx),
                          ws_bytes, _p(_f32c(pq_weight.detach())), rows, _p(pq), _stream())
            return idx, pq
    with torch.cuda.device(x.device):
        rc = 3
        if flags & _lib.KNN_FORCE_MFMA:
            xl = _lib.experiments()
            rc = xl.fsg_knn_experiment_f32(_p(x), B, N, x.stride(0), x.stride(1), c_knn, k, flags, _p(idx), _p(dist), _p(xx),
                                           _stream())
            if rc not in (0, 3):
                raise RuntimeError(xl.fsg_last_error().decode())
        if rc == 3:
            _lib.call("fsg_knn_dense_ws_f32", _p(x), B, N, x.stride(0), x.stride(1), c_knn, k, flags & ~_lib.KNN_FORCE_MFMA, _p(idx),
                      _p(dist), _p(xx), ws_bytes, _stream())
    if pq_weight is not None:
        return idx, None
    return (idx, dist) if return_dist else idx


class _EdgeGather(torch.autograd.Function):
    @staticmethod
    @_amp_fwd
    def forward(ctx, x, idx):
        B, C, N = x.shape
        k = idx.shape[2]
        half = x.dtype == torch.bfloat16
        xc = x.detach().contiguous() if half else _f32c(x)
        out = torch.empty(B, 2 * C, N, k, dtype=xc.dtype, device=x.device)
        with torch.cuda.device(x.device):
            _lib.call("fsg_edge_gather_fwd_bf16" if half else "fsg_edge_gather_fwd_f32", _p(xc), _p(idx), _p(out), B, C, N, k,
                      _stream())
        ctx.save_for_backward(idx)
        ctx.shape = (B, C, N, k)
        ctx.half = half
        return out

    @staticmethod
    @_amp_bwd
    def backward(ctx, g):
        (idx,) = ctx.saved_tensors
        B, C, N, k = ctx.shape
        half = ctx.half and g.dtype == torch.bfloat16
        g = g.detach().contiguous() if half else _f32c(g)
        gx = torch.empty(B, C, N, dtype=torch.float32, device=g.device)
        with torch.cuda.device(g.device):
            _lib.call("fsg_edge_gather_bwd_bf16" if half else "fsg_edge_gather_bwd_f32", _p(g), _p(idx), _p(gx), B, C, N, k,
                      _stream())
        return (gx.to(torch.bfloat16) if ctx.half else gx), None


def knn_edge_features(x, k, knn_only_over_coords=False):
    _need_gpu(x)
    xc = _f32c(x)
    B, C, N = xc.shape
    idx = torch.empty(B, N, k, dtype=torch.int32, device=x.device)
# ... 505 lines not shown
        return None
    return _lib.workspace("fsg_knn_dense", B, N, C, device=device)


def build_reverse_graphs(graphs):
    g0 = graphs[0]
    G = len(graphs)
    B, N, k = g0.shape
    step = B * N * k * g0.element_size()
    if any(g.shape != g0.shape or g.data_ptr() != g0.data_ptr() + i * step or not g.is_contiguous() for i, g in enumerate(graphs)):
        return
    if all(getattr(g, "_fsg_csr", None) is not None for g in graphs):
        return
    flat = torch.as_strided(g0, (G * B, N, k), (N * k, k, 1))
    rowptr, col = _build_csr(flat)
    for i, g in enumerate(graphs):
        g._fsg_csr = (rowptr[i * B:(i + 1) * B], col[i * B:(i + 1) * B])


def reverse_graph(idx):
    cached = getattr(idx, "_fsg_csr", None)
    if cached is None:
        cached = idx._fsg_csr = _build_csr(idx)
    return cached


def _pm_grad(g, B, N, C):
    if g is None:
        return None, 0
    if g.dtype == torch.float32 and g.shape == (B, N, C) and g.stride(2) == 1 and g.stride(1) >= C and \
            (B == 1 or g.stride(0) == N * g.stride(1)):
        return g, g.stride(1)
    return _f32c(g), C


def _apply_pass(ysel, gamma, beta, mean, invstd, B, N, Co, slope, out, out_pm, knn_ws, w_next):
    if knn_ws is None:
        return None
    nb = knn_ws.numel() * knn_ws.element_size()
    if w_next is not None and Co == 64 and tuple(w_next.shape) == (128, 64):
        w_next = _f32c(w_next.detach())
        pq_next = torch.empty(B, N, 128, dtype=torch.float32, device=ysel.device)
        _lib.call("fsg_edgeconv_apply_pq_f32", _p(ysel), _p(gamma), _p(beta), _p(mean), _p(invstd), B, N, Co, slope, _p(out),
                  _p(out_pm), _p(knn_ws), nb, _p(w_next), 128, _p(pq_next), _stream())
        return pq_next
    _lib.call("fsg_edgeconv_apply_f32", _p(ysel), _p(gamma), _p(beta), _p(mean), _p(invstd), B, N, Co, slope, _p(out),
              _p(out_pm), _p(knn_ws), nb, _stream())
    return None


class _EdgeConv1(torch.autograd.Function):
    @staticmethod
    @_amp_fwd
    def forward(ctx, pq, idx, gamma, beta, running_mean, running_var, training, momentum, eps, slope, knn_ws=None, w_next=None):
        pq = _f32c(pq)
        B, N, two_co = pq.shape
        Co, k, dev = two_co // 2, idx.shape[2], pq.device
        gamma, beta = _f32c(gamma), _f32c(beta)
        out = torch.empty(B, Co, N, dtype=torch.float32, device=dev)
        out_pm = torch.empty(B, N, Co, dtype=torch.float32, device=dev)
        ysel = torch.empty(B, N, Co, dtype=torch.float32, device=dev)
        arg = torch.empty(B, N, Co, dtype=torch.uint8, device=dev)
        if training:
            ssum = torch.empty(B, N, Co, dtype=torch.float32, device=dev)
            mean = torch.empty(Co, dtype=torch.float32, device=dev)
            invstd = torch.empty(Co, dtype=torch.float32, device=dev)
            ws = _lib.workspace("fsg_edgeconv1", B, N, Co, device=dev)
        else:
            ssum, ws = None, None
            mean, invstd = _bn_eval_stats(running_mean, running_var, eps)
        with torch.cuda.device(dev):
            _lib.call("fsg_edgeconv1_fwd_f32", _p(pq), _p(idx), _p(gamma), _p(beta),
                      _p(running_mean if training else None), _p(running_var if training else None), B, N, k, Co,
                      int(training), momentum, eps, slope, _p(None if knn_ws is not None else out), _p(out_pm), _p(ysel), _p(arg),
                      _p(ssum), _p(mean), _p(invstd), _p(ws), _stream())
            pq_next = _apply_pass(ysel, gamma, beta, mean, invstd, B, N, Co, slope, out, out_pm, knn_ws, w_next)
        ctx.save_for_backward(pq, idx, gamma, beta, mean, invstd, ysel, arg, ssum)
        ctx.meta = (B, N, k, Co, bool(training), slope)
        ctx.set_materialize_grads(False)
        if pq_next is None:
            return out, out_pm, out_pm.view(B, N, Co)
        ctx.mark_non_differentiable(pq_next)
        return out, out_pm, out_pm.view(B, N, Co), pq_next

    @staticmethod
    @_amp_bwd
    def backward(ctx, g, g_pm, g_pm2, _g_pq_next=None):
        pq, idx, gamma, beta, mean, invstd, ysel, arg, ssum = ctx.saved_tensors
        B, N, k, Co, training, slope = ctx.meta
        dev = pq.device
        g = _f32c(g) if g is not None else None
        g_pm, ld1 = _pm_grad(g_pm, B, N, Co)
        g_pm2, ld2 = _pm_grad(g_pm2, B, N, Co)
        rowptr, col = reverse_graph(idx)
        gpq = torch.empty_like(pq)
        dgamma = torch.empty(Co, dtype=torch.float32, device=dev)
        dbeta = torch.empty(Co, dtype=torch.float32, device=dev)
        h = torch.empty(B, N, Co, dtype=torch.float32, device=dev)
        ws = torch.empty(B * ((N + 63) // 64) * 2 * Co, dtype=torch.float32, device=dev)
        with torch.cuda.device(dev):
            _lib.call("fsg_edgeconv1_bwd_f32", _p(g), _p(g_pm), ld1, _p(g_pm2), ld2, _p(pq), _p(rowptr), _p(col), _p(gamma),
                      _p(beta), _p(mean),
                      _p(invstd), _p(ysel), _p(arg), _p(ssum), B, N, k, Co, int(training), slope, _p(gpq), _p(dgamma),
                      _p(dbeta), _p(h), _p(ws), _stream())
        return gpq, None, dgamma, dbeta, None, None, None, None, None, None, None, None


def edgeconv1_supported(out_channels, k):
    return out_channels % 64 == 0 and k <= 64


def edgeconv1(x, idx, conv_weight, bn, slope, x_pm=None, both=False, w_cat=None, knn_ws=None, w_next=None, pq_given=None):
    _need_gpu(x, idx, conv_weight)
    Co, C2 = conv_weight.shape[0], conv_weight.shape[1]
    C = C2 // 2
    if w_cat is None:
        w_cat = _EdgeWeights.apply(conv_weight.reshape(Co, C2).to(torch.float32))
    if x_pm is None:
        x_pm = x.transpose(1, 2)
    if pq_given is not None:
        pq = _LinearPMGiven.apply(x_pm.to(torch.float32), w_cat, pq_given)
    else:
        pq = linear_pm(x_pm.to(torch.float32).contiguous(), w_cat)
    bn_args = _bn_args(bn)
    if idx.dtype != torch.int32:
        idx = idx.to(torch.int32)
    idx = idx.contiguous()
    res = _EdgeConv1.apply(pq, idx, *bn_args, float(slope), knn_ws, w_next if knn_ws is not None else None)
    return _edgeconv_outputs(res, both, w_next is not None)


class _EdgeConv2(torch.autograd.Function):
    @staticmethod
    @_amp_fwd
    def forward(ctx, pq, idx, w2, g1, b1, rm1, rv1, g2, b2, rm2, rv2, training, mom1, mom2, eps1, eps2, slope, knn_ws=None,
                w_next=None):
        pq, w2 = _f32c(pq), _f32c(w2)
        g1, b1, g2, b2 = _f32c(g1), _f32c(b1), _f32c(g2), _f32c(b2)
        B, N, _ = pq.shape
        C2, k, dev = w2.shape[0], idx.shape[2], pq.device

        def new(*shape, dtype=torch.float32):
            return torch.empty(*shape, dtype=dtype, device=dev)
        out, out_pm = new(B, C2, N), new(B, N, C2)
        ysel2, arg2 = new(B, N, C2), new(B, N, C2, dtype=torch.uint8)
        if training:
            ssum1, ssum2 = new(B, N, 64), new(B, N, C2)
            mean1, invstd1, mean2, invstd2 = new(64), new(64), new(C2), new(C2)
        else:
            ssum1 = ssum2 = None
            mean1, invstd1 = _bn_eval_stats(rm1, rv1, eps1)
            mean2, invstd2 = _bn_eval_stats(rm2, rv2, eps2)
        ws = _lib.workspace("fsg_edgeconv2", B, N, k, C2, device=dev)
        t = bool(training)
        ctx.bf16 = bf16_operands()
        with torch.cuda.device(dev):
            _lib.call("fsg_edgeconv2_fwd_bf16" if ctx.bf16 else "fsg_edgeconv2_fwd_f32", _p(pq), _p(idx), _p(w2), _p(g1), _p(b1),
                      _p(rm1 if t else None),
                      _p(rv1 if t else None), _p(g2), _p(b2), _p(rm2 if t else None), _p(rv2 if t else None), B, N, k, C2,
                      int(t), mom1, mom2, eps1, eps2, slope, _p(None if knn_ws is not None else out), _p(out_pm), _p(ssum1), _p(mean1),
                      _p(invstd1), _p(ysel2), _p(arg2), _p(ssum2), _p(mean2), _p(invstd2), _p(ws), _stream())
            pq_next = _apply_pass(ysel2, g2, b2, mean2, invstd2, B, N, C2, slope, out, out_pm, knn_ws, w_next)
        ctx.save_for_backward(pq, idx, w2, g1, b1, mean1, invstd1, ssum1, g2, b2, mean2, invstd2, ysel2, arg2)
        ctx.meta = (B, N, k, C2, t, slope)
        ctx.set_materialize_grads(False)
        if pq_next is None:
            return out, out_pm, out_pm.view(B, N, C2)
        ctx.mark_non_differentiable(pq_next)
        return out, out_pm, out_pm.view(B, N, C2), pq_next

    @staticmethod
    @_amp_bwd
    def backward(ctx, g, g_pm, g_pm2, _g_pq_next=None):
        pq, idx, w2, g1, b1, mean1, invstd1, ssum1, g2, b2, mean2, invstd2, ysel2, arg2 = ctx.saved_tensors
        B, N, k, C2, training, slope = ctx.meta
        dev = pq.device
        g = _f32c(g) if g is not None else None
        g_pm, ld1 = _pm_grad(g_pm, B, N, C2)
        g_pm2, ld2 = _pm_grad(g_pm2, B, N, C2)
        rowptr, col = reverse_graph(idx)
        gpq, gw2 = torch.empty_like(pq), torch.empty_like(w2)
        dg1, db1 = torch.empty_like(g1), torch.empty_like(b1)
        dg2, db2 = torch.empty_like(g2), torch.empty_like(b2)
        ws = _lib.workspace("fsg_edgeconv2_bwd", B, N, k, C2, device=dev)
        with torch.cuda.device(dev):
            _lib.call("fsg_edgeconv2_bwd_bf16" if ctx.bf16 else "fsg_edgeconv2_bwd_f32", _p(g), _p(g_pm), ld1, _p(g_pm2), ld2,
                      _p(pq), _p(idx), _p(rowptr), _p(col),
                      _p(w2), _p(g1),
                      _p(b1), _p(mean1), _p(invstd1), _p(ssum1), _p(g2), _p(b2), _p(mean2), _p(invstd2), _p(ysel2),
                      _p(arg2), B, N, k, C2, int(training), slope, _p(gpq), _p(gw2), _p(dg1), _p(db1), _p(dg2), _p(db2),
                      _p(ws), _stream())
        return (gpq, None, gw2, dg1, db1, None, None, dg2, db2) + (None,) * 10


def edgeconv2_supported(c_mid, c_out, k):
    return c_mid == 64 and c_out in (64, 128) and k <= 64


def _edgeconv_outputs(res, both, want_pq_next):
    out, out_pm, out_pm2 = res[:3]
    pq_next = res[3] if len(res) > 3 else None
    if both == "twice":
        r = (out, out_pm, out_pm2)
    elif both:
        r = (out, out_pm)
    else:
        r = (out,)
    if want_pq_next:
        return r + (pq_next,)
    return r if len(r) > 1 else r[0]


def edgeconv2(x, idx, conv1_weight, bn1, conv2_weight, bn2, slope, x_pm=None, both=False, w_cat=None, knn_ws=None, w_next=None,
              pq_given=None):
    _need_gpu(x, idx, conv1_weight, conv2_weight)
    C1, CC = conv1_weight.shape[0], conv1_weight.shape[1]
    C = CC // 2
    if w_cat is None:
        w_cat = _EdgeWeights.apply(conv1_weight.reshape(C1, CC).to(torch.float32))
    if x_pm is None:
        x_pm = x.transpose(1, 2)
    if pq_given is not None:
        pq = _LinearPMGiven.apply(x_pm.to(torch.float32), w_cat, pq_given)
    else:
        pq = linear_pm(x_pm.to(torch.float32).contiguous(), w_cat)
    w2 = conv2_weight.reshape(conv2_weight.shape[0], C1)
    t1, m1 = _bn_step(bn1)
    t2, m2 = _bn_step(bn2)
    if t1 != t2:
        raise RuntimeError("edgeconv2: both BatchNorm layers must be in the same mode")
    if idx.dtype != torch.int32:
        idx = idx.to(torch.int32)
    idx = idx.contiguous()
    res = _EdgeConv2.apply(pq, idx, w2, bn1.weight, bn1.bias, bn1.running_mean, bn1.running_var,
                           bn2.weight, bn2.bias, bn2.running_mean, bn2.running_var, t1, m1, m2,
                           float(bn1.eps), float(bn2.eps), float(slope), knn_ws, w_next if knn_ws is not None else None)
    return _edgeconv_outputs(res, both, w_next is not None)


def pw_weight_image(w, scale=1.0, out=None, ks0=0, KS=None):
    _need_gpu(w)
    N, K = w.shape
    ks = (K + 15) // 16
    KS = ks if KS is None else KS
    if out is None:
        out = torch.empty(((N + 31) // 32) * KS * 3 * 1024, dtype=torch.uint8, device=w.device)
    with torch.cuda.device(w.device):
        _lib.call("fsg_pw_weight_image_f32", _p(w), w.stride(0), w.stride(1), N, K, float(scale), ks0, KS, _p(out), _stream())
    return out


def pw_weight_images(specs):
    jobs = _lib.PWImageJobs()
    outs = []
    assert 1 <= len(specs) <= _lib.PW_MAX_IMAGE_JOBS
    for j, (w, scale, out, ks0, KS) in enumerate(specs):
        N, K = w.shape
        KS = (K + 15) // 16 if KS is None else KS
        if out is None:
            out = torch.empty(((N + 31) // 32) * KS * 3 * 1024, dtype=torch.uint8, device=w.device)
        jobs.W[j], jobs.stride_n[j], jobs.stride_k[j], jobs.N[j], jobs.K[j] = w.data_ptr(), w.stride(0), w.stride(1), N, K
        jobs.ks0[j], jobs.KS[j], jobs.scale[j], jobs.image[j] = ks0, KS, float(scale), out.data_ptr()
        outs.append(out)
    jobs.n = len(specs)
    with torch.cuda.device(specs[0][0].device):
        _lib.call("fsg_pw_weight_images_f32", ctypes.byref(jobs), _stream())
    return outs


_bf16_linear = False


def set_bf16_linear(flag):
    global _bf16_linear
    old, _bf16_linear = _bf16_linear, bool(flag)
    return old


def _pw_bf16_ok(x2, w):
    return (_bf16_linear and bf16_operands() and x2.is_cuda and x2.dtype == torch.float32 and w.dtype == torch.float32 and x2.dim() == 2 and
            x2.stride(1) == 1 and x2.stride(0) % 4 == 0 and x2.data_ptr() % 16 == 0 and x2.shape[1] % 32 == 0 and x2.shape[0] > 0)


def pw_linear_bf16(x, w, bias=None, tile=0, out=None):
    M, K = x.shape
    N = w.shape[0]
    dev = x.device
    img = torch.empty(((N + 31) // 32) * ((K + 15) // 16) * 1024, dtype=torch.uint8, device=dev)
    y = torch.empty(M, N, dtype=torch.float32, device=dev) if out is None else out
# ... 2242 lines not shown
```

### fissure-segmentation_amd/models/dgcnn.py

```python
import torch
from torch import nn

from .. import functional as F_hip
from ..norm import BatchNorm1d, BatchNorm2d
from ..utils.general_utils import knn
from ..utils.model_utils import init_weights
from .point_seg_net import PointSegmentationModelBase


def create_neighbor_features(x, k, fixed_knn_graph=None, knn_only_over_coords=False):
    if fixed_knn_graph is None:
        graph = F_hip.knn_graph(x, k, c_knn=3 if knn_only_over_coords else None, fix_diag=True)
    else:
        graph = fixed_knn_graph
    return F_hip.edge_features(x, graph)


class ConvBlock(nn.Module):

    def __init__(self, in_channels, out_channels, kernel_size=3, stride=1, padding=True, dim=2,
                 negative_slope=1e-2, bn=True, activation=True):
        super().__init__()
        try:
            conv, norm = {1: (nn.Conv1d, BatchNorm1d), 2: (nn.Conv2d, BatchNorm2d),
# ... 4 lines not shown
                     padding=(kernel_size // 2) if padding else 0)]
        if bn:
            mods.append(norm(out_channels))
        if activation:
            mods.append(nn.LeakyReLU(negative_slope))
        self.layers = nn.ModuleList(mods)

    def forward(self, x):
        for layer in self.layers:
            if (isinstance(layer, nn.modules.conv._ConvNd) and x.is_cuda and all(k == 1 for k in layer.kernel_size)
                    and all(v == 1 for v in layer.stride) and all(v == 0 for v in layer.padding)
                    and all(v == 1 for v in layer.dilation) and layer.groups == 1):
                w = layer.weight.reshape(layer.out_channels, layer.in_channels)
                y = torch.matmul(w, x.flatten(2))
                if layer.bias is not None:
                    y = y + layer.bias.view(1, -1, 1)
                x = y.view(x.shape[0], layer.out_channels, *x.shape[2:])
            else:
                x = layer(x)
        return x


class SharedFullyConnected(ConvBlock):

    def __init__(self, in_features, out_features, dim=2, last_layer=False):
        super().__init__(in_features, out_features, dim=dim, kernel_size=1, padding=False,
                         bn=not last_layer, activation=not last_layer, negative_slope=0.2)


class EdgeConv(nn.Module):

    def __init__(self, in_features, out_features_list, k, first_layer=False):
        super().__init__()
        self.k = k
        self.first_layer = first_layer
        widths = [2 * in_features, *out_features_list]
        self.shared_mlp = nn.ModuleList(SharedFullyConnected(a, b) for a, b in zip(widths[:-1], widths[1:]))

    @property
    def fused(self):
        mlp = self.shared_mlp
        if len(mlp) == 1 and len(mlp[0].layers) == 3:
            return F_hip.edgeconv1_supported(mlp[0].layers[0].out_channels, self.k)
        return len(mlp) == 2 and all(len(m.layers) == 3 for m in mlp) and \
            F_hip.edgeconv2_supported(mlp[0].layers[0].out_channels, mlp[1].layers[0].out_channels, self.k)

    @staticmethod
    def pq_weights(blocks):
        fused = [b for b in blocks if b.fused]
        ws = F_hip.edge_weights_many([b.shared_mlp[0].layers[0].weight for b in fused]) if fused else []
        it = iter(ws)
        return [next(it) if b.fused else None for b in blocks]

    def forward(self, x, fixed_knn_graph=None, x_pm=None, both=False, w_cat=None, knn_ws=None, w_next=None, pq_given=None):
        if len(self.shared_mlp) == 1 and len(self.shared_mlp[0].layers) == 3 and \
                F_hip.edgeconv1_supported(self.shared_mlp[0].layers[0].out_channels, self.k):
            graph = fixed_knn_graph
            if graph is None:
                graph = F_hip.knn_graph(x, self.k, c_knn=3 if self.first_layer else None, fix_diag=True)
            conv, bn, act = self.shared_mlp[0].layers
            return F_hip.edgeconv1(x, graph, conv.weight, bn, act.negative_slope, x_pm=x_pm, both=both, w_cat=w_cat,
                                   knn_ws=knn_ws, w_next=w_next, pq_given=pq_given)
        if len(self.shared_mlp) == 2 and all(len(m.layers) == 3 for m in self.shared_mlp) and \
                F_hip.edgeconv2_supported(self.shared_mlp[0].layers[0].out_channels,
                                          self.shared_mlp[1].layers[0].out_channels, self.k):
            graph = fixed_knn_graph
            if graph is None:
                graph = F_hip.knn_graph(x, self.k, c_knn=3 if self.first_layer else None, fix_diag=True)
            (conv1, bn1, act), (conv2, bn2, _) = self.shared_mlp[0].layers, self.shared_mlp[1].layers
            return F_hip.edgeconv2(x, graph, conv1.weight, bn1, conv2.weight, bn2, act.negative_slope, x_pm=x_pm,
                                   both=both, w_cat=w_cat, knn_ws=knn_ws, w_next=w_next, pq_given=pq_given)
        e = create_neighbor_features(x, self.k, fixed_knn_graph, knn_only_over_coords=self.first_layer)
        for layer in self.shared_mlp:
            e = layer(e)
        out = e.max(dim=-1)[0]
        if not both:
            return out
        pm = out.transpose(1, 2).contiguous()
        return (out, pm, pm) if both == "twice" else (out, pm)


def pointwise_block(x_pm, block):
    conv = block.layers[0]
    y = F_hip.linear_pm(x_pm, conv.weight.view(conv.out_channels, conv.in_channels), conv.bias)
    return _norm_act(y, list(block.layers)[1:])


def _norm_act(y, tail):
    if len(tail) == 2 and isinstance(tail[1], nn.LeakyReLU) and F_hip.bn_act_supported(y, tail[0]):
        return F_hip.bn_act(y, tail[0], tail[1].negative_slope)
    for layer in tail:
        y = layer(y)
    return y


class SpatialTransformer(nn.Module):

    def __init__(self, k):
        super().__init__()
        self.in_features = 3
        self.ec = EdgeConv(3, [64, 128], k)
        self.shared_fc = SharedFullyConnected(128, 1024, dim=1)
        self.mlp = nn.Sequential(nn.Linear(1024, 512), BatchNorm1d(512), nn.LeakyReLU(0.2),
                                 nn.Linear(512, 256), BatchNorm1d(256), nn.LeakyReLU(0.2))
        self.transform = nn.Linear(256, 9)

    def forward(self, x, fixed_knn_graph=None):
        xyz = x[:, :3].contiguous()
        t = self.shared_fc(self.ec(xyz, fixed_knn_graph)).max(dim=-1)[0]
        t = self.transform(self.mlp(t)).view(-1, 3, 3)
        xyz = torch.bmm(xyz.transpose(1, 2), t).transpose(1, 2)
        return torch.cat([xyz, x[:, 3:]], dim=1)

    def init_weights(self):
        self.apply(init_weights)
        nn.init.zeros_(self.transform.weight)
        nn.init.eye_(self.transform.bias.view(3, 3))


class ImageFeatures(nn.Module):

    def __init__(self, in_channels=6, out_channels=(6, 12), kernel_size=1):
        super().__init__()
        chans = [in_channels, *out_channels]
# ... 2 lines not shown

    def forward(self, x):
        f = x[:, 3:]
        for layer in self.layers:
            f = layer(f)
        return torch.cat([x[:, :3], f], dim=1)


class DGCNNBase(PointSegmentationModelBase):

    def __init__(self, k, in_features, num_classes, spatial_transformer=False, dynamic=True,
                 image_feat_module=False):
        super().__init__(in_features, num_classes, k=k, spatial_transformer=spatial_transformer,
                         dynamic=dynamic, image_feat_module=image_feat_module)
        self.k = k
        self.dynamic = dynamic
        self.knn_graph = None
        if image_feat_module:
            if in_features < 4:
                raise ValueError('Number of In-Features for DGCNN too low if you want to use the image feature '
                                 'module! Need at 3, as the first 3 are assumed to be the point coordinates.')
            self.image_feature_module = ImageFeatures(in_channels=in_features - 3, out_channels=(6, 12))
            self.in_features = 3 + 12
        else:
            self.image_feature_module = None
        self.spatial_transformer = SpatialTransformer(k) if spatial_transformer else None
        self.output_activation = nn.Identity()

    def forward(self, x):
        if not x.is_cuda:
            raise RuntimeError("DGCNN (HIP path) needs its input on the GPU")
        if not self.dynamic:
            self.knn_graph = F_hip.knn_graph(x, self.k, c_knn=3, fix_diag=True, drop_first=True)
        if self.image_feature_module is not None:
            x = self.image_feature_module(x)
        if self.spatial_transformer is not None:
            x = self.spatial_transformer(x)
        return x

    def init_weights(self):
        self.apply(init_weights)
        if self.spatial_transformer is not None:
            self.spatial_transformer.init_weights()


class DGCNNSeg(DGCNNBase):

    def __init__(self, k, in_features, num_classes, spatial_transformer=False, dynamic=True,
                 image_feat_module=False):
        super().__init__(k, in_features, num_classes, spatial_transformer, dynamic, image_feat_module)
        self.ec1 = EdgeConv(self.in_features, [64, 64], k, first_layer=True)
        self.ec2 = EdgeConv(64, [64], k)
        self.ec3 = EdgeConv(64, [64], k)
        self.global_feature = nn.Sequential(SharedFullyConnected(192, 1024, dim=1), nn.AdaptiveMaxPool1d(1))
        self.segmentation = nn.Sequential(SharedFullyConnected(192 + 1024, 256, dim=1),
                                          SharedFullyConnected(256, 256, dim=1),
                                          SharedFullyConnected(256, 128, dim=1),
                                          SharedFullyConnected(128, self.num_classes, dim=1, last_layer=True))
        self.init_weights()

    @F_hip.with_deferred_bn_counters
    def forward(self, x):
        x = super().forward(x)
        B, _, N = x.shape
        p1c, p2c, p3 = self.edge_levels(x)
        levels = torch.cat([p1c, p2c, p3], dim=2).view(B * N, 192)
        gf = self.global_feature[0].layers
        seg0 = self.segmentation[0]
        w = lambda conv: conv.weight.view(conv.out_channels, -1)
        if F_hip.seg_head_supported(levels, B, N, w(gf[0]), w(seg0.layers[0]), w(self.segmentation[1].layers[0]),
                                    w(self.segmentation[2].layers[0]), w(self.segmentation[3].layers[0]),
                                    blocks=[self.global_feature[0]] + list(self.segmentation)):
            y = F_hip.seg_head(levels, B, N, self.global_feature[0], list(self.segmentation))
        else:
            y = self._head_unfused(levels, B, N)
        out = y.view(B, N, self.num_classes).transpose(1, 2)
        return out if self.training and torch.is_grad_enabled() else out.contiguous()

    def edge_levels(self, x):
        B, _, N = x.shape
        w1, w2, w3 = EdgeConv.pq_weights([self.ec1, self.ec2, self.ec3])
        if self.dynamic and all(e.fused for e in (self.ec1, self.ec2, self.ec3)):
            graphs = list(torch.empty(3, B, N, self.k, dtype=torch.int32, device=x.device).unbind(0))
            ws2, ws3 = F_hip.knn_prep_workspace(B, N, 64, x.device), F_hip.knn_prep_workspace(B, N, 64, x.device)
            g1, pq1 = F_hip.knn_graph(x, self.k, c_knn=3, fix_diag=True, out=graphs[0], pq_weight=w1)
            x1, p1, p1c, pq2 = self.ec1(x, g1, both="twice", w_cat=w1, knn_ws=ws2, w_next=w2, pq_given=pq1)
            g2 = F_hip.knn_graph(x1, self.k, fix_diag=True, out=graphs[1], prepared=None if ws2 is None else (ws2, p1))
            x2, p2, p2c, pq3 = self.ec2(x1, g2, x_pm=p1, both="twice", w_cat=w2, knn_ws=ws3, w_next=w3, pq_given=pq2)
            g3 = F_hip.knn_graph(x2, self.k, fix_diag=True, out=graphs[2], prepared=None if ws3 is None else (ws3, p2))
            _, p3 = self.ec3(x2, g3, x_pm=p2, both=True, w_cat=w3, pq_given=pq3)
            if torch.is_grad_enabled() and any(p.requires_grad for p in self.parameters()):
                F_hip.build_reverse_graphs([g1, g2, g3])
        else:
            x1, p1, p1c = self.ec1(x, self.knn_graph, both="twice", w_cat=w1)
            x2, p2, p2c = self.ec2(x1, self.knn_graph, x_pm=p1, both="twice", w_cat=w2)
            _, p3 = self.ec3(x2, self.knn_graph, x_pm=p2, both=True, w_cat=w3)
        return p1c, p2c, p3

    def _head_unfused(self, levels, B, N):
        gf = self.global_feature[0].layers
        seg0 = self.segmentation[0]
        w0 = seg0.layers[0].weight.view(seg0.layers[0].out_channels, -1)
        w0_levels, w0_global = F_hip.split_cols(w0, 192)
        yg, y0 = F_hip.linear_pm2(levels, gf[0].weight.view(gf[0].out_channels, -1), w0_levels)
        if yg.shape[1] % 64 == 0:
            g = F_hip.bn_act_max(yg.view(B, N, -1), gf[1], gf[2].negative_slope)
        else:
            g = _norm_act(yg, list(gf)[1:]).view(B, N, -1).max(dim=1)[0]
        y = F_hip.add_per_cloud(y0.view(B, N, -1), nn.functional.linear(g, w0_global))
        y = _norm_act(y.view(B * N, -1), list(seg0.layers)[1:])
        for block in list(self.segmentation)[1:]:
            y = pointwise_block(y, block)
        return y


class DGCNNReg(DGCNNBase):

    def __init__(self, k, in_features, num_classes, spatial_transformer=False, dynamic=True,
                 image_feat_module=False):
        super().__init__(k, in_features, num_classes, spatial_transformer, dynamic, image_feat_module)
        self.ec1 = EdgeConv(self.in_features, [64], k, first_layer=True)
        self.ec2 = EdgeConv(64, [64], k)
        self.ec3 = EdgeConv(64, [128], k)
        self.ec4 = EdgeConv(128, [256], k)
        self.global_feature = nn.Sequential(SharedFullyConnected(512, 1024, dim=1), nn.AdaptiveMaxPool1d(1))
        self.regression = nn.Sequential(SharedFullyConnected(1024, 512, dim=1),
                                        SharedFullyConnected(512, 256, dim=1),
                                        SharedFullyConnected(256, self.num_classes, dim=1, last_layer=True))
        self.init_weights()

    @F_hip.with_deferred_bn_counters
    def forward(self, x):
        x = super().forward(x)
        feats = []
        for ec in (self.ec1, self.ec2, self.ec3, self.ec4):
            x = ec(x, self.knn_graph)
            feats.append(x)
        return self.regression(self.global_feature(torch.cat(feats, dim=1)))

    def predict_full_pointcloud(self, pc, sample_points=1024, n_runs_min=50):
        acc = torch.zeros(pc.shape[0], self.num_classes, 1, device=pc.device)
        if self._ensemble_batchable(pc):
            B, per = pc.shape[0], max(1, self.ensemble_max_clouds // max(pc.shape[0], 1))
# ... 11 lines not shown
```

### include/fsg_hip.h

```cpp
#ifndef FSG_HIP_H
#define FSG_HIP_H

#include <stddef.h>
#include <stdint.h>

#ifdef __cplusplus
extern "C" {
#endif

#define FSG_OK 0
#define FSG_ERR_ARG 1
#define FSG_ERR_HIP 2
#define FSG_ERR_UNSUPPORTED 3

#define FSG_KNN_FIX_DIAG 1
#define FSG_KNN_DROP_FIRST 2

#define FSG_KNN_FORCE_ROWS 4

#define FSG_KNN_FORCE_MFMA 8

#define FSG_KNN_MAX_K 64

typedef void *fsg_stream_t;

int fsg_version(void);
const char *fsg_last_error(void);

int fsg_knn_dense_f32(const float *x, int B, int N, int64_t stride_b, int64_t stride_c, int c_knn,
                      int k, int flags, int32_t *idx_out, float *dist_out, float *xx_scratch,
                      fsg_stream_t stream);

size_t fsg_knn_dense_workspace_bytes(int B, int N, int c_knn);
int fsg_knn_dense_ws_f32(const float *x, int B, int N, int64_t stride_b, int64_t stride_c, int c_knn,
                         int k, int flags, int32_t *idx_out, float *dist_out, void *workspace,
                         size_t workspace_bytes, fsg_stream_t stream);

int fsg_knn_dense_ws_pq_f32(const float *x, int B, int N, int64_t stride_b, int64_t stride_c, int c_knn, int k, int flags,
                            int32_t *idx_out, float *dist_out, void *workspace, size_t workspace_bytes, const float *w_pq,
                            int rows_pq, float *pq_out, fsg_stream_t stream);

int fsg_knn_dense_prepared_f32(const float *x_pm, int B, int N, int c_knn, int k, int flags, int32_t *idx_out, float *dist_out,
                               void *workspace, size_t workspace_bytes, fsg_stream_t stream);

int fsg_edge_gather_fwd_f32(const float *x, const int32_t *idx, float *edge, int B, int C, int N,
                            int k, fsg_stream_t stream);
int fsg_edge_gather_bwd_f32(const float *grad_edge, const int32_t *idx, float *grad_x, int B, int C,
                            int N, int k, fsg_stream_t stream);
int fsg_knn_gather_fused_f32(const float *x, int B, int C, int N, int k, int c_knn, int32_t *idx_out, float *edge,
                             float *xx_scratch, fsg_stream_t stream);
int fsg_knn_gather_fused_ws_f32(const float *x, int B, int C, int N, int k, int c_knn, int32_t *idx_out, float *edge,
                                void *workspace, size_t workspace_bytes, fsg_stream_t stream);
int fsg_edge_gather_fwd_bf16(const void *x, const int32_t *idx, void *edge, int B, int C, int N, int k,
                             fsg_stream_t stream);
int fsg_edge_gather_bwd_bf16(const void *grad_edge, const int32_t *idx, float *grad_x, int B, int C, int N,
                             int k, fsg_stream_t stream);

size_t fsg_graph_reverse_csr_workspace_bytes(int B, int N, int k);
int fsg_graph_reverse_csr(const int32_t *idx, int B, int N, int k, int32_t *rowptr, int32_t *col,
                          void *workspace, fsg_stream_t stream);

int fsg_edge_weights_fwd_f32(const float *W, int Co, int C, float *Wt, fsg_stream_t stream);
int fsg_edge_weights_bwd_f32(const float *grad_Wt, int Co, int C, float *grad_W, fsg_stream_t stream);
#define FSG_EDGE_WEIGHT_MAX_JOBS 8
typedef struct fsg_edge_weight_jobs {
    const float *src[FSG_EDGE_WEIGHT_MAX_JOBS];
    float *dst[FSG_EDGE_WEIGHT_MAX_JOBS];
    int Co[FSG_EDGE_WEIGHT_MAX_JOBS];
    int C[FSG_EDGE_WEIGHT_MAX_JOBS];
    int n;
} fsg_edge_weight_jobs;
int fsg_edge_weights_many_f32(const fsg_edge_weight_jobs *jobs, int backward, fsg_stream_t stream);

int fsg_edgeconv_apply_f32(const float *ysel, const float *gamma, const float *beta, const float *mean, const float *invstd,
                           int B, int N, int Co, float slope, float *out, float *out_pm, void *knn_workspace,
                           size_t knn_workspace_bytes, fsg_stream_t stream);

int fsg_edgeconv_apply_pq_f32(const float *ysel, const float *gamma, const float *beta, const float *mean, const float *invstd,
                              int B, int N, int Co, float slope, float *out, float *out_pm, void *knn_workspace,
                              size_t knn_workspace_bytes, const float *w_next, int rows_next, float *pq_next,
                              fsg_stream_t stream);

size_t fsg_edgeconv1_workspace_bytes(int B, int N, int Co);
int fsg_edgeconv1_fwd_f32(const float *pq, const int32_t *idx, const float *gamma, const float *beta,
                          float *running_mean, float *running_var, int B, int N, int k, int Co, int training,
                          float momentum, float eps, float slope, float *out, float *out_pm, float *ysel,
                          uint8_t *arg, float *ssum, float *mean, float *invstd, float *workspace,
                          fsg_stream_t stream);
int fsg_edgeconv1_bwd_f32(const float *grad_out, const float *grad_out_pm, int64_t ld_pm, const float *grad_out_pm2,
                          int64_t ld_pm2, const float *pq, const int32_t *rowptr, const int32_t *col,
                          const float *gamma, const float *beta, const float *mean, const float *invstd,
                          const float *ysel, const uint8_t *arg, const float *ssum, int B, int N, int k, int Co,
                          int training, float slope, float *grad_pq, float *grad_gamma, float *grad_beta,
                          float *h_scratch, float *workspace, fsg_stream_t stream);

size_t fsg_edgeconv2_workspace_bytes(int B, int N, int k, int C2);
size_t fsg_edgeconv2_bwd_workspace_bytes(int B, int N, int k, int C2);
int fsg_edgeconv2_fwd_f32(const float *pq, const int32_t *idx, const float *w2, const float *gamma1,
                          const float *beta1, float *running_mean1, float *running_var1, const float *gamma2,
                          const float *beta2, float *running_mean2, float *running_var2, int B, int N, int k, int C2,
                          int training, float momentum1, float momentum2, float eps1, float eps2, float slope,
                          float *out, float *out_pm, float *ssum1, float *mean1, float *invstd1, float *ysel2,
                          uint8_t *arg2, float *ssum2, float *mean2, float *invstd2, void *workspace,
                          fsg_stream_t stream);
int fsg_edgeconv2_bwd_f32(const float *grad_out, const float *grad_out_pm, int64_t ld_pm, const float *grad_out_pm2,
                          int64_t ld_pm2, const float *pq, const int32_t *idx,
                          const int32_t *rowptr, const int32_t *col, const float *w2, const float *gamma1,
                          const float *beta1, const float *mean1, const float *invstd1, const float *ssum1,
                          const float *gamma2, const float *beta2, const float *mean2, const float *invstd2,
                          const float *ysel2, const uint8_t *arg2, int B, int N, int k, int C2, int training,
                          float slope, float *grad_pq, float *grad_w2, float *grad_gamma1, float *grad_beta1,
                          float *grad_gamma2, float *grad_beta2, void *workspace, fsg_stream_t stream);
int fsg_edgeconv2_fwd_bf16(const float *pq, const int32_t *idx, const float *w2, const float *gamma1,
                           const float *beta1, float *running_mean1, float *running_var1, const float *gamma2,
                           const float *beta2, float *running_mean2, float *running_var2, int B, int N, int k, int C2,
                           int training, float momentum1, float momentum2, float eps1, float eps2, float slope,
                           float *out, float *out_pm, float *ssum1, float *mean1, float *invstd1, float *ysel2,
                           uint8_t *arg2, float *ssum2, float *mean2, float *invstd2, void *workspace,
                           fsg_stream_t stream);
int fsg_edgeconv2_bwd_bf16(const float *grad_out, const float *grad_out_pm, int64_t ld_pm, const float *grad_out_pm2,
                           int64_t ld_pm2, const float *pq, const int32_t *idx,
                           const int32_t *rowptr, const int32_t *col, const float *w2, const float *gamma1,
                           const float *beta1, const float *mean1, const float *invstd1, const float *ssum1,
                           const float *gamma2, const float *beta2, const float *mean2, const float *invstd2,
                           const float *ysel2, const uint8_t *arg2, int B, int N, int k, int C2, int training,
                           float slope, float *grad_pq, float *grad_w2, float *grad_gamma1, float *grad_beta1,
                           float *grad_gamma2, float *grad_beta2, void *workspace, fsg_stream_t stream);

size_t fsg_bn_act_workspace_bytes(long M, int C);
int fsg_bn_act_fwd_f32(const float *y, const float *gamma, const float *beta, float *running_mean, float *running_var,
                       long M, int C, int training, float momentum, float eps, float slope, float *out, float *mean,
                       float *invstd, float *workspace, fsg_stream_t stream);
int fsg_bn_act_bwd_f32(const float *grad_out, const float *y, const float *gamma, const float *beta, const float *mean,
                       const float *invstd, long M, int C, int training, float slope, float *grad_y, float *grad_gamma,
                       float *grad_beta, float *workspace, fsg_stream_t stream);

size_t fsg_bn_act_max_workspace_bytes(int B, int N, int C);
int fsg_bn_act_max_fwd_f32(const float *y, const float *gamma, const float *beta, float *running_mean,
                           float *running_var, int B, int N, int C, int training, float momentum, float eps,
                           float slope, float *out, float *ysel, int32_t *arg, float *mean, float *invstd,
                           float *workspace, fsg_stream_t stream);
int fsg_bn_act_max_bwd_f32(const float *grad_out, const float *y, const float *ysel, const int32_t *arg,
                           const float *gamma, const float *beta, const float *mean, const float *invstd, int B, int N,
                           int C, int training, float slope, float *grad_y, float *grad_gamma, float *grad_beta,
                           fsg_stream_t stream);

size_t fsg_bn_act_maxavg_workspace_bytes(int B, int N, int C);
int fsg_bn_act_maxavg_fwd_f32(const float *y, const float *gamma, const float *beta, float *running_mean,
                              float *running_var, int B, int N, int C, int training, float momentum, float eps,
                              float slope, float *out, int32_t *arg, float *mean, float *invstd, float *workspace,
                              fsg_stream_t stream);
int fsg_bn_act_maxavg_bwd_f32(const float *grad_out, const float *y, const int32_t *arg, const float *gamma,
                              const float *beta, const float *mean, const float *invstd, int B, int N, int C,
                              int training, float slope, float *grad_y, float *grad_gamma, float *grad_beta,
                              float *workspace, fsg_stream_t stream);

size_t fsg_chamfer_nn_bwd_workspace_bytes(int B, int N, int M);
int fsg_chamfer_nn_f32(const float *x, const float *y, int B, int N, int M, float *dist,
                       int32_t *arg, fsg_stream_t stream);
int fsg_chamfer_nn_bwd_f32(const float *x, const float *y, const int32_t *arg, const float *g_dist,
                           int B, int N, int M, float *grad_x, float *grad_y, void *workspace,
                           fsg_stream_t stream);

int fsg_point_mesh_dist_f32(const float *pts, const float *verts, const int32_t *faces, int B, int P, int V, int F,
                            int Bf, float *dist2, int32_t *face, float *closest, fsg_stream_t stream);

int fsg_mesh_labelmap_dist_f32(const float *verts, const int32_t *faces, const int32_t *labels, int V, int F, int d0, int d1,
                               int d2, float s0, float s1, float s2, float dist_threshold, const uint8_t *mask, uint64_t *keys,
                               int64_t *out, fsg_stream_t stream);
int fsg_mesh_labelmap_cover_f32(const float *verts, const int32_t *faces, const int32_t *labels, int V, int F, int d0, int d1,
                                int d2, float s0, float s1, float s2, int64_t *out, fsg_stream_t stream);

// ... 347 lines not shown
```

Measured before the change: 16.84 million.

## Fuse EdgeConv edge statistics and max-select into the kNN graph kernel

Moves the per-edge gather, BatchNorm partial statistics and signed max/argmax selection out of a separate stats kernel and into the kNN kernel, which already holds the neighbour indices. The EdgeConv forward then skips its own stats launch when the statistics are supplied. This removes a kernel launch per layer and a reread of the index tensor and PQ rows. In exchange the kNN kernel gets more work, which may raise its register pressure and lower its occupancy.

Result: no change. 16.92 million, median of 6 (+0.5%).

```diff
diff --git a/fissure-segmentation_amd/_lib.py b/fissure-segmentation_amd/_lib.py
--- a/fissure-segmentation_amd/_lib.py
+++ b/fissure-segmentation_amd/_lib.py
@@ -19,8 +19,8 @@
     "fsg_knn_dense_f32": ([_P, _I, _I, _L, _L, _I, _I, _I, _P, _P, _P, _P], _I),
     "fsg_knn_dense_workspace_bytes": ([_I, _I, _I], ctypes.c_size_t),
     "fsg_knn_dense_ws_f32": ([_P, _I, _I, _L, _L, _I, _I, _I, _P, _P, _P, ctypes.c_size_t, _P], _I),
-    "fsg_knn_dense_prepared_f32": ([_P, _I, _I, _I, _I, _I, _P, _P, _P, ctypes.c_size_t, _P], _I),
-    "fsg_knn_dense_ws_pq_f32": ([_P, _I, _I, _L, _L, _I, _I, _I, _P, _P, _P, ctypes.c_size_t, _P, _I, _P, _P], _I),
+    "fsg_knn_dense_prepared_f32": ([_P, _I, _I, _I, _I, _I, _P, _P, _P, ctypes.c_size_t, _P, _P], _I),
+    "fsg_knn_dense_ws_pq_f32": ([_P, _I, _I, _L, _L, _I, _I, _I, _P, _P, _P, ctypes.c_size_t, _P, _I, _P, _P, _P], _I),
     "fsg_edgeconv_apply_f32": ([_P, _P, _P, _P, _P, _I, _I, _I, _F, _P, _P, _P, ctypes.c_size_t, _P], _I),
     "fsg_edgeconv_apply_pq_f32": ([_P, _P, _P, _P, _P, _I, _I, _I, _F, _P, _P, _P, ctypes.c_size_t, _P, _I, _P, _P], _I),
     "fsg_edge_gather_fwd_f32": ([_P, _P, _P, _I, _I, _I, _I, _P], _I),
@@ -35,15 +35,15 @@
     "fsg_edge_weights_bwd_f32": ([_P, _I, _I, _P, _P], _I),
     "fsg_edge_weights_many_f32": ([_P, _I, _P], _I),
     "fsg_edgeconv1_workspace_bytes": ([_I, _I, _I], ctypes.c_size_t),
-    "fsg_edgeconv1_fwd_f32": ([_P, _P, _P, _P, _P, _P, _I, _I, _I, _I, _I, _F, _F, _F, _P, _P, _P, _P, _P, _P, _P, _P, _P],
+    "fsg_edgeconv1_fwd_f32": ([_P, _P, _P, _P, _P, _P, _I, _I, _I, _I, _I, _F, _F, _F, _P, _P, _P, _P, _P, _P, _P, _P, _P, _I],
                               _I),
     "fsg_edgeconv1_bwd_f32": ([_P, _P, _L, _P, _L, _P, _P, _P, _P, _P, _P, _P, _P, _P, _P, _I, _I, _I, _I, _I, _F, _P, _P,
                                _P, _P, _P, _P], _I),
     "fsg_edgeconv2_workspace_bytes": ([_I, _I, _I, _I], ctypes.c_size_t),
     "fsg_edgeconv2_bwd_workspace_bytes": ([_I, _I, _I, _I], ctypes.c_size_t),
-    "fsg_edgeconv2_fwd_f32": ([_P] * 11 + [_I] * 5 + [_F] * 5 + [_P] * 12, _I),
+    "fsg_edgeconv2_fwd_f32": ([_P] * 11 + [_I] * 5 + [_F] * 5 + [_P] * 12 + [_I], _I),
     "fsg_edgeconv2_bwd_f32": ([_P, _P, _L, _P, _L] + [_P] * 16 + [_I] * 5 + [_F] + [_P] * 8, _I),
-    "fsg_edgeconv2_fwd_bf16": ([_P] * 11 + [_I] * 5 + [_F] * 5 + [_P] * 12, _I),
+    "fsg_edgeconv2_fwd_bf16": ([_P] * 11 + [_I] * 5 + [_F] * 5 + [_P] * 12 + [_I], _I),
     "fsg_edgeconv2_bwd_bf16": ([_P, _P, _L, _P, _L] + [_P] * 16 + [_I] * 5 + [_F] + [_P] * 8, _I),
     "fsg_bn_act_workspace_bytes": ([ctypes.c_long, _I], ctypes.c_size_t),
     "fsg_bn_act_fwd_f32": ([_P, _P, _P, _P, _P, ctypes.c_long, _I, _I, _F, _F, _F, _P, _P, _P, _P, _P], _I),
@@ -210,6 +210,11 @@
                 ("J", _I * GEMM_REDUCE_MAX_JOBS), ("blocks", _I * GEMM_REDUCE_MAX_JOBS), ("n", _I)]
 
 
+class KnnEdgeStats(ctypes.Structure):
+    _fields_ = [("pq", _P), ("ld", _I), ("gamma", _P), ("training", _I), ("ysel", _P), ("arg", _P), ("ssum", _P),
+                ("partials", _P), ("fused", _I)]
+
+
 class EdgeWeightJobs(ctypes.Structure):
     _fields_ = [("src", _P * 8), ("dst", _P * 8), ("Co", _I * 8), ("C", _I * 8), ("n", _I)]
 
diff --git a/fissure-segmentation_amd/csrc/edgeconv.hip b/fissure-segmentation_amd/csrc/edgeconv.hip
--- a/fissure-segmentation_amd/csrc/edgeconv.hip
+++ b/fissure-segmentation_amd/csrc/edgeconv.hip
@@ -227,23 +227,15 @@
                                                                 int training, float *__restrict__ ysel,
                                                                 uint8_t *__restrict__ arg, float *__restrict__ ssum,
                                                                 float *__restrict__ partials) {
-    typedef f32x2 f2;
-    typedef f32x4 f4;
-    typedef u32x4 u4;
     constexpr int NW = 4 * TPW;
-    __shared__ float red[2][4 * NW][64];
+    static_assert(4 * NW == FSG_EC_TILE, "one record per FSG_EC_TILE points");
+    __shared__ float red[2][FSG_EC_TILE][64];
     const int b = blockIdx.x, tile = blockIdx.y, cg = blockIdx.z;
     const int lane = threadIdx.x & 63, wave = __builtin_amdgcn_readfirstlane(threadIdx.x >> 6);
     const int g = lane >> 4, c16 = lane & 15;
     const int c0 = cg * 64 + 4 * c16;
     const int ld = 2 * Co;
     const __amdgpu_buffer_rsrc_t rs = buffer_rsrc(pq + (long)b * N * ld, __builtin_amdgcn_readfirstlane((int)((long)N * ld * 4)));
-    f2 sgn[2] = {{1.f, 1.f}, {1.f, 1.f}};
-    if (SELECT) {
-        const f4 gm = *reinterpret_cast<const f4 *>(gamma + c0);
-        sgn[0] = f2{gm[0] >= 0.f ? 1.f : -1.f, gm[1] >= 0.f ? 1.f : -1.f};
-        sgn[1] = f2{gm[2] >= 0.f ? 1.f : -1.f, gm[3] >= 0.f ? 1.f : -1.f};
-    }
     const int i = tile * TP * TPW + wave * (TP / 4) + g;
     const bool live = i < N;
     const int ic = live ? i : N - 1;
@@ -251,97 +243,20 @@
 #pragma unroll
     for (int r = 0; r < 4; ++r)
         if (16 * r < k) ids[r] = (16 * r + c16 < k) ? idx[((long)b * N + ic) * k + 16 * r + c16] : 0;
-    const f4 q4 = __builtin_bit_cast(f4, __builtin_amdgcn_raw_buffer_load_b128(
-        rs, (unsigned)ic * (unsigned)(ld * 4) + (unsigned)((Co + c0) * 4), 0, 0));
-    const f2 q[2] = {{q4[0], q4[1]}, {q4[2], q4[3]}};
-    f2 tot[2] = {{0.f, 0.f}, {0.f, 0.f}}, shift[2] = {{0.f, 0.f}, {0.f, 0.f}}, s1[2] = {{0.f, 0.f}, {0.f, 0.f}},
-       s2[2] = {{0.f, 0.f}, {0.f, 0.f}};
-    float best[4] = {-INFINITY, -INFINITY, -INFINITY, -INFINITY};
-    int barg[4] = {0, 0, 0, 0};
-    constexpr int RB = SELECT ? 8 : 10;
-    auto request = [&](int s0, u4 (&y)[RB]) {
-#pragma unroll
-        for (int u = 0; u < RB; ++u) {
-            const int s = min(s0 + u, k - 1);
-            const int r = s >> 4;
-            const int held = r == 0 ? ids[0] : (r == 1 ? ids[1] : (r == 2 ? ids[2] : ids[3]));
-            const int j = __builtin_amdgcn_ds_bpermute(4 * ((lane & 48) | (s & 15)), held);
-            y[u] = __builtin_amdgcn_raw_buffer_load_b128(rs, (unsigned)j * (unsigned)(ld * 4) + (unsigned)(c0 * 4), 0, 0);
-        }
-    };
-    auto consume = [&](int s0, const u4 (&y)[RB]) {
-#pragma unroll
-        for (int u = 0; u < RB; ++u) {
-            const int s = s0 + u;
-            if (s < k) {
-                const f4 yv = __builtin_bit_cast(f4, y[u]);
-#pragma unroll
-                for (int hf = 0; hf < 2; ++hf) {
-                    const f2 yy = f2{yv[2 * hf], yv[2 * hf + 1]} + q[hf];
-                    tot[hf] += yy;
-                    if (training) {
-                        if (s == 0) shift[hf] = yy;
-                        const f2 d = yy - shift[hf];
-                        s1[hf] += d;
-                        s2[hf] = __builtin_elementwise_fma(d, d, s2[hf]);
-                    }
-                    if (SELECT) {
-                        const f2 v = sgn[hf] * yy;
-#pragma unroll
-                        for (int e = 0; e < 2; ++e)
-                            if (v[e] > best[2 * hf + e]) { best[2 * hf + e] = v[e]; barg[2 * hf + e] = s; }
-                    }
-                }
-            }
-        }
-    };
-    u4 ya[RB], yb[RB];
-    request(0, ya);
-    for (int s0 = 0; s0 < k; s0 += 2 * RB) {
-        if (s0 + RB < k) request(s0 + RB, yb);
-        consume(s0, ya);
-        if (s0 + 2 * RB < k) request(s0 + 2 * RB, ya);
-        if (s0 + RB < k) consume(s0 + RB, yb);
-    }
-    if (live) {
-        const long o = ((long)b * N + i) * Co + c0;
-        if (SELECT) {
-            *reinterpret_cast<f4 *>(ysel + o) = f4{sgn[0][0] * best[0], sgn[0][1] * best[1], sgn[1][0] * best[2], sgn[1][1] * best[3]};
-            *reinterpret_cast<unsigned *>(arg + o) =
-                (unsigned)barg[0] | ((unsigned)barg[1] << 8) | ((unsigned)barg[2] << 16) | ((unsigned)barg[3] << 24);
-        }
-        if (ssum) *reinterpret_cast<f4 *>(ssum + o) = f4{tot[0][0], tot[0][1], tot[1][0], tot[1][1]};
-    }
+    float mo[4], m2[4];
+    fsg_ec_gather_point<SELECT>(rs, gamma, lane, ic, live, ((long)b * N + i) * Co + c0, c0, ld, Co, k, training, ids, ysel, arg, ssum,
+                                mo, m2);
     if (!training) return;
 #pragma unroll
     for (int e = 0; e < 4; ++e) {
-        const float s1e = s1[e >> 1][e & 1], s2e = s2[e >> 1][e & 1], she = shift[e >> 1][e & 1];
-        red[0][wave * 4 + g][4 * c16 + e] = she + s1e / (float)k;
-        red[1][wave * 4 + g][4 * c16 + e] = fmaxf(s2e - s1e * s1e / (float)k, 0.f);
+        red[0][wave * 4 + g][4 * c16 + e] = mo[e];
+        red[1][wave * 4 + g][4 * c16 + e] = m2[e];
     }
     __syncthreads();
     if (wave == 0) {
-        const int c = cg * 64 + lane;
         const int live_groups = min(4 * NW, max(0, N - tile * TP * TPW));
-        float sm = 0.f, sM = 0.f;
-#pragma unroll 8
-        for (int w = 0; w < 4 * NW; ++w) {
-            const bool on = w < live_groups;
-            sm += on ? red[0][w][lane] : 0.f;
-            sM += on ? red[1][w][lane] : 0.f;
-        }
-        const float mu = live_groups > 0 ? sm / (float)live_groups : 0.f;
-        float dev = 0.f;
-#pragma unroll 8
-        for (int w = 0; w < 4 * NW; ++w) {
-            const float d = red[0][w][lane] - mu;
-            dev = __builtin_fmaf(w < live_groups ? d : 0.f, d, dev);
-        }
         const long rec = (long)b * gridDim.y + tile;
-        float *pr = partials + rec * 3 * Co;
-        pr[c] = (float)live_groups * (float)k;
-        pr[Co + c] = mu;
-        pr[2 * Co + c] = sM + (float)k * dev;
+        fsg_ec_merge_record(red, lane, cg * 64 + lane, live_groups, k, Co, partials + rec * 3 * Co);
     }
 }
 
@@ -922,7 +837,7 @@
                                      float *running_mean, float *running_var, int B, int N, int k, int Co, int training,
                                      float momentum, float eps, float slope, float *out, float *out_pm, float *ysel,
                                      uint8_t *arg, float *ssum, float *mean, float *invstd, float *workspace,
-                                     fsg_stream_t stream) {
+                                     fsg_stream_t stream, int stats_given) {
     FSG_REQUIRE(pq && idx && gamma && beta && ysel && arg && mean && invstd, "fsg_edgeconv1_fwd_f32: NULL pointer");
     FSG_REQUIRE(B > 0 && N > 0 && k > 0 && k <= 64 && Co > 0 && Co % 64 == 0 && B <= 65535,
                 "fsg_edgeconv1_fwd_f32: bad shape B=%d N=%d k=%d Co=%d (Co must be a multiple of 64)", B, N, k, Co);
@@ -930,9 +845,11 @@
     FSG_REQUIRE((long)N * 2 * Co * 4 < (1L << 31), "fsg_edgeconv1_fwd_f32: a cloud's [P | Q] rows must stay below 2 GiB (N=%d, Co=%d)", N, Co);
     hipStream_t st = (hipStream_t)stream;
     const int tiles = fsg_cdiv(N, TP * TPW);
-    hipLaunchKernelGGL(ec1_stats_select_kernel<true>, dim3(B, tiles, Co / 64), dim3(256 * TPW), 0, st, pq, idx, gamma, N, k, Co,
-                       training, ysel, arg, ssum, workspace);
-    FSG_CHECK_LAUNCH("fsg_edgeconv1_fwd_f32/stats");
+    if (!stats_given) {
+        hipLaunchKernelGGL(ec1_stats_select_kernel<true>, dim3(B, tiles, Co / 64), dim3(256 * TPW), 0, st, pq, idx, gamma, N, k, Co,
+                           training, ysel, arg, ssum, workspace);
+        FSG_CHECK_LAUNCH("fsg_edgeconv1_fwd_f32/stats");
+    }
     if (training) {
         const int rc = fsg_ec_finalize_launch(workspace, B * tiles, Co, eps, momentum, mean, invstd, running_mean,
                                               running_var, st);
diff --git a/fissure-segmentation_amd/csrc/edgeconv2.hip b/fissure-segmentation_amd/csrc/edgeconv2.hip
--- a/fissure-segmentation_amd/csrc/edgeconv2.hip
+++ b/fissure-segmentation_amd/csrc/edgeconv2.hip
@@ -1098,7 +1098,7 @@
                                      int C2, int training, float momentum1, float momentum2, float eps1, float eps2,
                                      float slope, float *out, float *out_pm, float *ssum1, float *mean1, float *invstd1,
                                      float *ysel2, uint8_t *arg2, float *ssum2, float *mean2, float *invstd2,
-                                     void *workspace, fsg_stream_t stream) {
+                                     void *workspace, fsg_stream_t stream, int stats_given) {
     FSG_REQUIRE(pq && idx && w2 && gamma1 && beta1 && gamma2 && beta2 && mean1 && invstd1 && ysel2 && arg2 &&
                     mean2 && invstd2 && workspace,
                 "fsg_edgeconv2_fwd_f32: NULL pointer");
@@ -1120,7 +1120,7 @@
     uint8_t *arg1 = (uint8_t *)(ysel1 + (size_t)B * N * C1);
     int rc;
     if (training) {
-        if ((rc = fsg_ec_stats1_launch(pq, idx, gamma1, B, N, k, C1, ysel1, arg1, ssum1, part1, st)) != FSG_OK) return rc;
+        if (!stats_given && (rc = fsg_ec_stats1_launch(pq, idx, gamma1, B, N, k, C1, ysel1, arg1, ssum1, part1, st)) != FSG_OK) return rc;
         if ((rc = fsg_ec_finalize_launch(part1, rec1, C1, eps1, momentum1, mean1, invstd1, running_mean1, running_var1,
                                          st)) != FSG_OK)
             return rc;
@@ -1162,8 +1162,8 @@
                                      int C2, int training, float momentum1, float momentum2, float eps1, float eps2,
                                      float slope, float *out, float *out_pm, float *ssum1, float *mean1, float *invstd1,
                                      float *ysel2, uint8_t *arg2, float *ssum2, float *mean2, float *invstd2,
-                                     void *workspace, fsg_stream_t stream) {
-    return ec2_fwd_impl(false, pq, idx, w2, gamma1, beta1, running_mean1, running_var1, gamma2, beta2, running_mean2, running_var2, B, N, k, C2, training, momentum1, momentum2, eps1, eps2, slope, out, out_pm, ssum1, mean1, invstd1, ysel2, arg2, ssum2, mean2, invstd2, workspace, stream);
+                                     void *workspace, fsg_stream_t stream, int stats_given) {
+    return ec2_fwd_impl(false, pq, idx, w2, gamma1, beta1, running_mean1, running_var1, gamma2, beta2, running_mean2, running_var2, B, N, k, C2, training, momentum1, momentum2, eps1, eps2, slope, out, out_pm, ssum1, mean1, invstd1, ysel2, arg2, ssum2, mean2, invstd2, workspace, stream, stats_given);
 }
 
 extern "C" int fsg_edgeconv2_fwd_bf16(const float *pq, const int32_t *idx, const float *w2, const float *gamma1,
@@ -1172,8 +1172,8 @@
                                      int C2, int training, float momentum1, float momentum2, float eps1, float eps2,
                                      float slope, float *out, float *out_pm, float *ssum1, float *mean1, float *invstd1,
                                      float *ysel2, uint8_t *arg2, float *ssum2, float *mean2, float *invstd2,
-                                     void *workspace, fsg_stream_t stream) {
-    return ec2_fwd_impl(true, pq, idx, w2, gamma1, beta1, running_mean1, running_var1, gamma2, beta2, running_mean2, running_var2, B, N, k, C2, training, momentum1, momentum2, eps1, eps2, slope, out, out_pm, ssum1, mean1, invstd1, ysel2, arg2, ssum2, mean2, invstd2, workspace, stream);
+                                     void *workspace, fsg_stream_t stream, int stats_given) {
+    return ec2_fwd_impl(true, pq, idx, w2, gamma1, beta1, running_mean1, running_var1, gamma2, beta2, running_mean2, running_var2, B, N, k, C2, training, momentum1, momentum2, eps1, eps2, slope, out, out_pm, ssum1, mean1, invstd1, ysel2, arg2, ssum2, mean2, invstd2, workspace, stream, stats_given);
 }
 
 static void ec2_bwd_tiling(int k, int C2, int &TP, int &Rpad, int &G, int B, int N) {
diff --git a/fissure-segmentation_amd/csrc/edgeconv_internal.h b/fissure-segmentation_amd/csrc/edgeconv_internal.h
--- a/fissure-segmentation_amd/csrc/edgeconv_internal.h
+++ b/fissure-segmentation_amd/csrc/edgeconv_internal.h
@@ -21,3 +21,111 @@
 
 int fsg_csr_bipartite_launch(const int32_t *idx, int B, int NS, int N, int k, int32_t *rowptr, int32_t *col, int32_t *cnt,
                              int32_t *tmp, hipStream_t st);
+
+constexpr int FSG_EC_TILE = 32;
+
+#ifdef __HIPCC__
+template <bool SELECT>
+__device__ __forceinline__ void fsg_ec_gather_point(const __amdgpu_buffer_rsrc_t rs, const float *__restrict__ gamma, int lane,
+                                                    int ic, bool live, long o, int c0, int ld, int Co, int k, int training,
+                                                    const int (&ids)[4], float *__restrict__ ysel, uint8_t *__restrict__ arg,
+                                                    float *__restrict__ ssum, float (&mo)[4], float (&m2)[4]) {
+    typedef f32x2 f2;
+    typedef f32x4 f4;
+    typedef u32x4 u4;
+    f2 sgn[2] = {{1.f, 1.f}, {1.f, 1.f}};
+    if (SELECT) {
+        const f4 gm = *reinterpret_cast<const f4 *>(gamma + c0);
+        sgn[0] = f2{gm[0] >= 0.f ? 1.f : -1.f, gm[1] >= 0.f ? 1.f : -1.f};
+        sgn[1] = f2{gm[2] >= 0.f ? 1.f : -1.f, gm[3] >= 0.f ? 1.f : -1.f};
+    }
+    const f4 q4 = __builtin_bit_cast(f4, __builtin_amdgcn_raw_buffer_load_b128(
+        rs, (unsigned)ic * (unsigned)(ld * 4) + (unsigned)((Co + c0) * 4), 0, 0));
+    const f2 q[2] = {{q4[0], q4[1]}, {q4[2], q4[3]}};
+    f2 tot[2] = {{0.f, 0.f}, {0.f, 0.f}}, shift[2] = {{0.f, 0.f}, {0.f, 0.f}}, s1[2] = {{0.f, 0.f}, {0.f, 0.f}},
+       s2[2] = {{0.f, 0.f}, {0.f, 0.f}};
+    float best[4] = {-INFINITY, -INFINITY, -INFINITY, -INFINITY};
+    int barg[4] = {0, 0, 0, 0};
+    constexpr int RB = SELECT ? 8 : 10;
+    auto request = [&](int s0, u4 (&y)[RB]) {
+#pragma unroll
+        for (int u = 0; u < RB; ++u) {
+            const int s = min(s0 + u, k - 1);
+            const int r = s >> 4;
+            const int held = r == 0 ? ids[0] : (r == 1 ? ids[1] : (r == 2 ? ids[2] : ids[3]));
+            const int j = __builtin_amdgcn_ds_bpermute(4 * ((lane & 48) | (s & 15)), held);
+            y[u] = __builtin_amdgcn_raw_buffer_load_b128(rs, (unsigned)j * (unsigned)(ld * 4) + (unsigned)(c0 * 4), 0, 0);
+        }
+    };
+    auto consume = [&](int s0, const u4 (&y)[RB]) {
+#pragma unroll
+        for (int u = 0; u < RB; ++u) {
+            const int s = s0 + u;
+            if (s < k) {
+                const f4 yv = __builtin_bit_cast(f4, y[u]);
+#pragma unroll
+                for (int hf = 0; hf < 2; ++hf) {
+                    const f2 yy = f2{yv[2 * hf], yv[2 * hf + 1]} + q[hf];
+                    tot[hf] += yy;
+                    if (training) {
+                        if (s == 0) shift[hf] = yy;
+                        const f2 d = yy - shift[hf];
+                        s1[hf] += d;
+                        s2[hf] = __builtin_elementwise_fma(d, d, s2[hf]);
+                    }
+                    if (SELECT) {
+                        const f2 v = sgn[hf] * yy;
+#pragma unroll
+                        for (int e = 0; e < 2; ++e)
+                            if (v[e] > best[2 * hf + e]) { best[2 * hf + e] = v[e]; barg[2 * hf + e] = s; }
+                    }
+                }
+            }
+        }
+    };
+    u4 ya[RB], yb[RB];
+    request(0, ya);
+    for (int s0 = 0; s0 < k; s0 += 2 * RB) {
+        if (s0 + RB < k) request(s0 + RB, yb);
+        consume(s0, ya);
+        if (s0 + 2 * RB < k) request(s0 + 2 * RB, ya);
+        if (s0 + RB < k) consume(s0 + RB, yb);
+    }
+    if (live) {
+        if (SELECT) {
+            *reinterpret_cast<f4 *>(ysel + o) = f4{sgn[0][0] * best[0], sgn[0][1] * best[1], sgn[1][0] * best[2], sgn[1][1] * best[3]};
+            *reinterpret_cast<unsigned *>(arg + o) =
+                (unsigned)barg[0] | ((unsigned)barg[1] << 8) | ((unsigned)barg[2] << 16) | ((unsigned)barg[3] << 24);
+        }
+        if (ssum) *reinterpret_cast<f4 *>(ssum + o) = f4{tot[0][0], tot[0][1], tot[1][0], tot[1][1]};
+    }
+    if (!training) return;
+#pragma unroll
+    for (int e = 0; e < 4; ++e) {
+        const float s1e = s1[e >> 1][e & 1], s2e = s2[e >> 1][e & 1], she = shift[e >> 1][e & 1];
+        mo[e] = she + s1e / (float)k;
+        m2[e] = fmaxf(s2e - s1e * s1e / (float)k, 0.f);
+    }
+}
+
+__device__ __forceinline__ void fsg_ec_merge_record(const float (*red)[FSG_EC_TILE][64], int lane, int c, int live_groups, int k,
+                                                    int Co, float *__restrict__ pr) {
+    float sm = 0.f, sM = 0.f;
+#pragma unroll 8
+    for (int w = 0; w < FSG_EC_TILE; ++w) {
+        const bool on = w < live_groups;
+        sm += on ? red[0][w][lane] : 0.f;
+        sM += on ? red[1][w][lane] : 0.f;
+    }
+    const float mu = live_groups > 0 ? sm / (float)live_groups : 0.f;
+    float dev = 0.f;
+#pragma unroll 8
+    for (int w = 0; w < FSG_EC_TILE; ++w) {
+        const float d = red[0][w][lane] - mu;
+        dev = __builtin_fmaf(w < live_groups ? d : 0.f, d, dev);
+    }
+    pr[c] = (float)live_groups * (float)k;
+    pr[Co + c] = mu;
+    pr[2 * Co + c] = sM + (float)k * dev;
+}
+#endif
diff --git a/fissure-segmentation_amd/csrc/knn_dense.hip b/fissure-segmentation_amd/csrc/knn_dense.hip
--- a/fissure-segmentation_amd/csrc/knn_dense.hip
+++ b/fissure-segmentation_amd/csrc/knn_dense.hip
@@ -130,8 +130,14 @@
 
 extern "C" int fsg_knn_dense_ws_pq_f32(const float *x, int B, int N, int64_t stride_b, int64_t stride_c, int c_knn, int k,
                                        int flags, int32_t *idx_out, float *dist_out, void *workspace, size_t workspace_bytes,
-                                       const float *w_pq, int rows_pq, float *pq_out, fsg_stream_t stream) {
+                                       const float *w_pq, int rows_pq, float *pq_out, fsg_stream_t stream,
+                                       fsg_knn_edge_stats *edge_stats) {
     FSG_KNN_REQUIRE_FLAGS("fsg_knn_dense_ws_pq_f32", flags);
+    if (edge_stats) {
+        edge_stats->fused = 0;
+        FSG_REQUIRE(edge_stats->pq == pq_out, "fsg_knn_dense_ws_pq_f32: the edge_stats job must read this call's pq_out");
+        FSG_KNN_REQUIRE_EDGE_STATS("fsg_knn_dense_ws_pq_f32", edge_stats);
+    }
     FSG_REQUIRE(x && idx_out && w_pq && pq_out, "fsg_knn_dense_ws_pq_f32: NULL pointer");
     FSG_REQUIRE(c_knn >= 1 && c_knn <= 4 && rows_pq >= 1 && 256 % rows_pq == 0,
                 "fsg_knn_dense_ws_pq_f32: needs 1 <= c_knn <= 4 and rows_pq dividing 256; got c_knn=%d rows_pq=%d", c_knn, rows_pq);
@@ -143,7 +149,7 @@
     if (workspace && !(flags & KNN_BYPASS_SPLIT)) {
         bool fused = false;
         KnnSplitOpts o;
-        o.pq_w = w_pq, o.pq_rows = rows_pq, o.pq_out = pq_out, o.pq_fused = &fused;
+        o.pq_w = w_pq, o.pq_rows = rows_pq, o.pq_out = pq_out, o.pq_fused = &fused, o.edge_stats = edge_stats;
         const int rc = fsg_knn_split_launch(x, B, N, stride_b, stride_c, c_knn, k, flags, idx_out, dist_out, workspace, workspace_bytes,
                                             st, o);
         if (rc == FSG_OK) return fused ? FSG_OK : fsg_knn_pq_rows_launch(x, B, N, stride_b, stride_c, c_knn, w_pq, rows_pq, pq_out, st);
@@ -156,14 +162,19 @@
 }
 
 extern "C" int fsg_knn_dense_prepared_f32(const float *x_pm, int B, int N, int c_knn, int k, int flags, int32_t *idx_out,
-                                          float *dist_out, void *workspace, size_t workspace_bytes, fsg_stream_t stream) {
+                                          float *dist_out, void *workspace, size_t workspace_bytes, fsg_stream_t stream,
+                                          fsg_knn_edge_stats *edge_stats) {
     const int drop = (flags & FSG_KNN_DROP_FIRST) ? 1 : 0;
     FSG_KNN_REQUIRE_FLAGS("fsg_knn_dense_prepared_f32", flags);
+    if (edge_stats) {
+        edge_stats->fused = 0;
+        FSG_KNN_REQUIRE_EDGE_STATS("fsg_knn_dense_prepared_f32", edge_stats);
+    }
     FSG_REQUIRE(x_pm && idx_out && workspace, "fsg_knn_dense_prepared_f32: NULL pointer");
     FSG_REQUIRE(B > 0 && N > 0 && c_knn > 0 && k >= 1 && k + drop <= N && k + drop <= FSG_KNN_MAX_K,
                 "fsg_knn_dense_prepared_f32: bad shape B=%d N=%d c_knn=%d k=%d", B, N, c_knn, k);
     KnnSplitOpts o;
-    o.prepared_xt = x_pm;
+    o.prepared_xt = x_pm, o.edge_stats = edge_stats;
     const int rc = fsg_knn_split_launch(nullptr, B, N, 0, 0, c_knn, k, flags, idx_out, dist_out, workspace, workspace_bytes,
                                         (hipStream_t)stream, o);
     if (rc == FSG_ERR_UNSUPPORTED) fsg_set_error("fsg_knn_dense_prepared_f32: shape outside the prepared path's envelope");
diff --git a/fissure-segmentation_amd/csrc/knn_internal.h b/fissure-segmentation_amd/csrc/knn_internal.h
--- a/fissure-segmentation_amd/csrc/knn_internal.h
+++ b/fissure-segmentation_amd/csrc/knn_internal.h
@@ -17,6 +17,11 @@
 #define FSG_KNN_REQUIRE_FLAGS(entry, flags) \
     FSG_REQUIRE(!((flags) & ~KNN_FLAGS_ALL), "%s: unknown flag bit(s) %u (a removed debug bit?)", entry, (unsigned)((flags) & ~KNN_FLAGS_ALL))
 
+#define FSG_KNN_REQUIRE_EDGE_STATS(entry, es)                                                                                 \
+    FSG_REQUIRE((es)->pq && ((es)->gamma ? (es)->ysel && (es)->arg : (es)->training != 0) && (!(es)->training || (es)->partials), \
+                "%s: edge_stats needs pq, ysel / arg with gamma (a job without gamma is statistics only: training), and partials "  \
+                "when training", entry)
+
 int fsg_knn_rows_mfma_launch(const float *x, int B, int N, int64_t stride_b, int64_t stride_c, int c_knn, int k, int flags,
                              int32_t *idx_out, float *dist_out, float *xx_scratch, hipStream_t st);
 int fsg_knn_segment_rows_launch(const float *xyz, const float *new_xyz, const int32_t *offset, const int32_t *new_offset,
@@ -30,6 +35,7 @@
     int pq_rows = 0;
     float *pq_out = nullptr;
     bool *pq_fused = nullptr;
+    fsg_knn_edge_stats *edge_stats = nullptr;
 };
 size_t fsg_knn_split_workspace_bytes(int B, int N, int c_knn);
 int fsg_knn_split_launch(const float *x, int B, int N, int64_t stride_b, int64_t stride_c, int c_knn, int k, int flags,
diff --git a/fissure-segmentation_amd/csrc/knn_split.hip b/fissure-segmentation_amd/csrc/knn_split.hip
--- a/fissure-segmentation_amd/csrc/knn_split.hip
+++ b/fissure-segmentation_amd/csrc/knn_split.hip
@@ -1,5 +1,6 @@
 #include <type_traits>
 
+#include "edgeconv_internal.h"
 #include "knn_internal.h"
 
 __device__ unsigned long long fsg_knn_split_stats[4];
@@ -1293,12 +1294,27 @@
 
 constexpr int RQW = 8;
 constexpr int RECAP = 256;
-template <int CP>
-__global__ __launch_bounds__(128) void knn_refine_kernel(const float *__restrict__ xx, const float *__restrict__ xt,
+constexpr int RTAILW = FSG_EC_TILE / RQW;
+struct RefineTail {
+    const float *pq, *gamma;
+    int training;
+    float *ysel;
+    uint8_t *arg;
+    float *ssum, *partials;
+};
+constexpr size_t refine_wave_bytes(int CP, bool tail) {
+    return (size_t)8 * RECAP + (CP > 4 ? (size_t)4 * 64 * ((CP > 32 ? 32 : CP) + 4) : 0) + (size_t)4 * RQW * (CP + 4) + 128 +
+           (tail ? (size_t)4 * RQW * 64 : 0);
+}
+constexpr size_t refine_lds_bytes(int CP, bool tail) {
+    return (tail ? RTAILW : 2) * refine_wave_bytes(CP, tail) + (tail ? sizeof(float) * 2 * FSG_EC_TILE * 64 : 0);
+}
+template <int CP, int TAIL>
+__global__ __launch_bounds__(TAIL ? 64 * RTAILW : 128) void knn_refine_kernel(const float *__restrict__ xx, const float *__restrict__ xt,
                                                          const unsigned *__restrict__ bmg, int N, int Np, int TS, int k,
                                                          int flags, int PCAP, int32_t *__restrict__ idx_out,
-                                                         float *__restrict__ dist_out) {
-    constexpr int QW = RQW, ECAP = RECAP, RW = 2;
+                                                         float *__restrict__ dist_out, const RefineTail tail) {
+    constexpr int QW = RQW, ECAP = RECAP, RW = TAIL ? RTAILW : 2;
     constexpr int CPQ = CP + 4;
     constexpr bool STAGE = CP > 4;
     constexpr int CS = CP > 32 ? 32 : CP;
@@ -1309,15 +1325,16 @@
     constexpr int NI = STAGE ? 64 / RPI : 1;
     extern __shared__ __attribute__((aligned(16))) unsigned char smem[];
     const int tid = threadIdx.x, lane = tid & 63, wave = __builtin_amdgcn_readfirstlane(tid >> 6);
-    constexpr size_t wbytes = (size_t)8 * ECAP + (STAGE ? (size_t)4 * 64 * CSQ : 0) + (size_t)4 * QW * CPQ + 128;
+    constexpr size_t wbytes = refine_wave_bytes(CP, TAIL != 0);
     u64 *keys = reinterpret_cast<u64 *>(smem + wave * wbytes);
     unsigned *klo = reinterpret_cast<unsigned *>(keys);
     float *stg = reinterpret_cast<float *>(keys + ECAP);
     float *qrows = stg + (STAGE ? 64 * CSQ : 0);
     int *seg = reinterpret_cast<int *>(qrows + QW * CPQ);
     unsigned *dump = reinterpret_cast<unsigned *>(seg + 2 * QW);
-    const bool stamps = (flags & KNN_DBG_STAMPS) != 0;
-    auto stamp = [&](int i) { knn_stamp<512, RW, 8>(fsg_knn_refine_stamps, stamps, wave, lane, i); };
+    int *nid = reinterpret_cast<int *>(dump + 16);
+    const bool stamps = !TAIL && (flags & KNN_DBG_STAMPS) != 0;
+    auto stamp = [&](int i) { knn_stamp<512, 2, 8>(fsg_knn_refine_stamps, stamps, wave, lane, i); };
     stamp(0);
     int b = blockIdx.y, qw0 = blockIdx.x * RW * QW;
     {
@@ -1334,7 +1351,7 @@
     const float *xxb = xx + (long)b * Np;
     const float *xtb = xt + (long)b * Np * CP;
     const int qbeg = qw0 + wave * QW;
-    if (qbeg >= N) return;
+    if (!TAIL && qbeg >= N) return;
     const int qi = lane >> 3, l8 = lane & 7;
     const int NCH = (TS + 63) >> 6;
     const unsigned *brow = bmg + ((long)b * Np + qbeg + qi) * TS + 8 * l8;
@@ -1565,6 +1582,7 @@
                     const long o = ((long)b * N + qbeg + tg) * k - drop + r[m];
                     idx_out[o] = (int)((unsigned)key[m] & 0xFFFFu);
                     if (dist_out) dist_out[o] = o2f((unsigned)(key[m] >> 32));
+                    if (TAIL) nid[tg * 64 + r[m] - drop] = (int)((unsigned)key[m] & 0xFFFFu);
                 }
             }
         }
@@ -1573,6 +1591,46 @@
         qa = qb;
     }
     stamp(5);
+    if constexpr (TAIL != 0) {
+        constexpr int Co = 64, ld = 2 * Co;
+        float(*red)[FSG_EC_TILE][64] = reinterpret_cast<float(*)[FSG_EC_TILE][64]>(smem + RW * wbytes);
+        const unsigned long long ranked = __ballot(qvalid);
+        const int g = lane >> 4, c16 = lane & 15, c0 = 4 * c16;
+        const __amdgpu_buffer_rsrc_t prs = buffer_rsrc(tail.pq + (long)b * N * ld, __builtin_amdgcn_readfirstlane((int)((long)N * ld * 4)));
+#pragma unroll 1
+        for (int rd = 0; rd < QW / 4; ++rd) {
+            const int u = 4 * rd + g, i = qbeg + u;
+            const bool live = i < N, own = ((ranked >> (8 * u)) & 1ull) != 0;
+            const int ic = live ? i : N - 1;
+            int ids[4] = {0, 0, 0, 0};
+#pragma unroll
+            for (int r = 0; r < 4; ++r)
+                if (16 * r < k) {
+                    const int s = 16 * r + c16;
+                    if (s < k) ids[r] = own ? nid[u * 64 + s] : idx_out[((long)b * N + ic) * k + s];
+                }
+            float mo[4], m2[4];
+            fsg_ec_gather_point<TAIL == 2>(prs, tail.gamma, lane, ic, live, ((long)b * N + i) * Co + c0, c0, ld, Co, k, tail.training, ids,
+                                           tail.ysel, tail.arg, tail.ssum, mo, m2);
+            if (tail.training) {
+#pragma unroll
+                for (int e = 0; e < 4; ++e) {
+                    red[0][wave * QW + u][c0 + e] = mo[e];
+                    red[1][wave * QW + u][c0 + e] = m2[e];
+                }
+            }
+        }
+        if (tail.training) {
+            __syncthreads();
+            if (wave == 0) {
+                const int tile = qw0 / FSG_EC_TILE;
+                const int live_groups = min(FSG_EC_TILE, max(0, N - qw0));
+                if (live_groups > 0)
+                    fsg_ec_merge_record(red, lane, lane, live_groups, k, Co,
+                                        tail.partials + ((long)b * (N / FSG_EC_TILE) + tile) * 3 * Co);
+            }
+        }
+    }
 }
 
 
@@ -1678,16 +1736,25 @@
     return FSG_OK;
 }
 
+template <int CP, int TAIL>
+int launch_refine_tail(const SplitArgs &a, int TS, int PCAP, const RefineTail &t) {
+    constexpr size_t lds = refine_lds_bytes(CP, true);
+    FSG_GRANT_LDS("fsg_knn_dense_ws_f32", (knn_refine_kernel<CP, TAIL>), lds);
+    hipLaunchKernelGGL((knn_refine_kernel<CP, TAIL>), dim3(a.p.Np / FSG_EC_TILE, a.B), dim3(64 * RTAILW), lds, a.st, a.xx, a.xt, a.bmg,
+                       a.N, a.p.Np, TS, a.k, a.flags, PCAP, a.idx_out, a.dist_out, t);
+    FSG_CHECK_LAUNCH("fsg_knn_dense_ws_f32/split+edge_stats");
+    return FSG_OK;
+}
+
 template <int KS, bool PK, bool HF>
 int launch_pair(const SplitArgs &a, const KnnSplitOpts &o) {
     const SplitPlan &p = a.p;
-    const size_t T = p.Np / 32, CPQ = p.CP + 4;
+    const size_t T = p.Np / 32;
     size_t bmw = (QB * (T + 1) + 3) & ~(size_t)3;
     if (bmw < (size_t)QB * NMIN) bmw = (size_t)QB * NMIN;
     const size_t lds1 = sizeof(float) * 32 * WAVES * ((T + WAVES - 1) / WAVES) + 4 * bmw + sizeof(float) * QB + sizeof(unsigned) * 4 + sizeof(float) * 24;
     const int PCAP = 256, TS = (int)((T + 7) & ~(size_t)7);
-    const size_t CS = p.CP > 32 ? 32 : p.CP;
-    const size_t lds2 = 2 * ((size_t)8 * RECAP + (p.CP > 4 ? 4 * 64 * (CS + 4) : 0) + 4 * (size_t)RQW * CPQ + 128);
+    const size_t lds2 = refine_lds_bytes(p.CP, false);
     if (lds1 > 160 * 1024 || lds2 > 64 * 1024) return FSG_ERR_UNSUPPORTED;
     const bool res = T == 64;
     constexpr bool RES_OK = (HF && KS <= 4) || PK;
@@ -1708,8 +1775,19 @@
                            : launch_nominate<KS, PK, HF, false, false>(a, lds1, PCAP, TS, RawPoints{});
     }
     if (rc != FSG_OK) return rc;
-    hipLaunchKernelGGL((knn_refine_kernel<(PK ? 4 : 16 * KS)>), dim3(p.Np / (2 * RQW), a.B), dim3(128), lds2, a.st, a.xx, a.xt, a.bmg,
-                       a.N, p.Np, TS, a.k, a.flags, PCAP, a.idx_out, a.dist_out);
+    constexpr bool TAIL_OK = PK || (HF && KS == 4);
+    if constexpr (TAIL_OK) {
+        const fsg_knn_edge_stats *es = o.edge_stats;
+        if (es && es->ld == 128 && p.Np == a.N && !a.dist_out && !(a.flags & ~(FSG_KNN_FIX_DIAG | FSG_KNN_DROP_FIRST)) &&
+            (!PK || (raw_ok && es->pq == o.pq_out))) {
+            const RefineTail t{es->pq, es->gamma, es->training, es->ysel, es->arg, es->ssum, es->partials};
+            rc = es->gamma ? launch_refine_tail<(PK ? 4 : 64), 2>(a, TS, PCAP, t) : launch_refine_tail<(PK ? 4 : 64), 1>(a, TS, PCAP, t);
+            if (rc == FSG_OK) o.edge_stats->fused = 1;
+            return rc;
+        }
+    }
+    hipLaunchKernelGGL((knn_refine_kernel<(PK ? 4 : 16 * KS), 0>), dim3(p.Np / (2 * RQW), a.B), dim3(128), lds2, a.st, a.xx, a.xt, a.bmg,
+                       a.N, p.Np, TS, a.k, a.flags, PCAP, a.idx_out, a.dist_out, RefineTail{});
     FSG_CHECK_LAUNCH("fsg_knn_dense_ws_f32/split");
     return FSG_OK;
 }
diff --git a/fissure-segmentation_amd/functional.py b/fissure-segmentation_amd/functional.py
--- a/fissure-segmentation_amd/functional.py
+++ b/fissure-segmentation_amd/functional.py
@@ -81,9 +81,44 @@
     return _deterministic or torch.are_deterministic_algorithms_enabled()
 
 
+class EdgeStats:
+
+    def __init__(self, pq, bn, select, c2=None):
+        self.pq, self.bn, self.select, self.c2 = pq, bn, bool(select), c2
+        self.fused = self.training = False
+        self.idx = self.ysel = self.arg = self.ssum = self.ws = None
+
+    def taken_by(self, pq, idx, gamma, training):
+        return self.fused and idx.data_ptr() == self.idx.data_ptr() and idx.shape == self.idx.shape and \
+            pq.data_ptr() == self.pq.data_ptr() and gamma.data_ptr() == self.bn.weight.data_ptr() and bool(training) == self.training
+
+
+def _edge_stats_job(es, pq, B, N, k, dev):
+    es.fused, es.pq = False, pq
+    bn = es.bn
+    es.training = bool(bn.training or bn.running_mean is None)
+    if pq is None or bn.weight is None or pq.dtype != torch.float32 or tuple(pq.shape) != (B, N, 128) or not pq.is_contiguous() or \
+            N % 64 != 0 or (not es.select and not es.training) or bn.weight.dtype != torch.float32:
+        return None
+    if es.select:
+        es.ysel = torch.empty(B, N, 64, dtype=torch.float32, device=dev)
+        es.arg = torch.empty(B, N, 64, dtype=torch.uint8, device=dev)
+    es.ssum = torch.empty(B, N, 64, dtype=torch.float32, device=dev) if es.training else None
+    if es.select:
+        es.ws = _lib.workspace("fsg_edgeconv1", B, N, 64, device=dev) if es.training else None
+    else:
+        es.ws = _lib.workspace("fsg_edgeconv2", B, N, k, es.c2, device=dev)
+    def a(t):
+        return t.data_ptr() if t is not None else None
+    return _lib.KnnEdgeStats(a(pq), 128, a(bn.weight) if es.select else None, int(es.training), a(es.ysel), a(es.arg), a(es.ssum),
+                             a(es.ws) if es.training else None, 0)
+
+
 def knn_graph(x, k, c_knn=None, fix_diag=True, drop_first=False, return_dist=False, force_rows_kernel=False,
-              _debug_flags=0, out=None, prepared=None, pq_weight=None):
+              _debug_flags=0, out=None, prepared=None, pq_weight=None, edge_stats=None):
     _need_gpu(x)
+    if edge_stats is not None:
+        edge_stats.fused = False
     if x.dim() != 3:
         raise ValueError(f"expected (B,C,N), got {tuple(x.shape)}")
     x = x.detach()
@@ -104,9 +139,12 @@
         (_lib.KNN_FORCE_ROWS if force_rows_kernel else 0) | _debug_flags
     if prepared is not None and c_knn == C and not return_dist and not force_rows_kernel and not _debug_flags:
         ws, x_pm = prepared
+        job = _edge_stats_job(edge_stats, edge_stats.pq, B, N, k, x.device) if edge_stats is not None else None
         with torch.cuda.device(x.device):
             _lib.call("fsg_knn_dense_prepared_f32", _p(x_pm), B, N, C, k, flags, _p(idx), None, _p(ws), ws.numel() * ws.element_size(),
-                      _stream())
+                      _stream(), ctypes.byref(job) if job is not None else None)
+        if job is not None:
+            edge_stats.fused, edge_stats.idx = bool(job.fused), idx
         return idx
     xx = _lib.workspace("fsg_knn_dense", B, N, c_knn, device=x.device)
     ws_bytes = xx.numel() if xx is not None else 0
@@ -115,9 +153,13 @@
         if (C == c_knn and c_knn <= 4 and tuple(pq_weight.shape) == (rows, C) and 256 % rows == 0 and not return_dist and
                 not (_debug_flags & _lib.KNN_FORCE_MFMA)):
             pq = torch.empty(B, N, rows, dtype=torch.float32, device=x.device)
+            job = _edge_stats_job(edge_stats, pq, B, N, k, x.device) if edge_stats is not None else None
             with torch.cuda.device(x.device):
                 _lib.call("fsg_knn_dense_ws_pq_f32", _p(x), B, N, x.stride(0), x.stride(1), c_knn, k, flags, _p(idx), None, _p(xx),
-                          ws_bytes, _p(_f32c(pq_weight.detach())), rows, _p(pq), _stream())
+                          ws_bytes, _p(_f32c(pq_weight.detach())), rows, _p(pq), _stream(),
+                          ctypes.byref(job) if job is not None else None)
+            if job is not None:
+                edge_stats.fused, edge_stats.idx = bool(job.fused), idx
             return idx, pq
     with torch.cuda.device(x.device):
         rc = 3
@@ -729,28 +771,32 @@
 class _EdgeConv1(torch.autograd.Function):
     @staticmethod
     @_amp_fwd
-    def forward(ctx, pq, idx, gamma, beta, running_mean, running_var, training, momentum, eps, slope, knn_ws=None, w_next=None):
+    def forward(ctx, pq, idx, gamma, beta, running_mean, running_var, training, momentum, eps, slope, knn_ws=None, w_next=None,
+                edge_stats=None):
         pq = _f32c(pq)
         B, N, two_co = pq.shape
         Co, k, dev = two_co // 2, idx.shape[2], pq.device
         gamma, beta = _f32c(gamma), _f32c(beta)
         out = torch.empty(B, Co, N, dtype=torch.float32, device=dev)
         out_pm = torch.empty(B, N, Co, dtype=torch.float32, device=dev)
-        ysel = torch.empty(B, N, Co, dtype=torch.float32, device=dev)
-        arg = torch.empty(B, N, Co, dtype=torch.uint8, device=dev)
+        given = edge_stats is not None and edge_stats.select and edge_stats.taken_by(pq, idx, gamma, training)
+        if given:
+            ysel, arg, ssum, ws = edge_stats.ysel, edge_stats.arg, edge_stats.ssum, edge_stats.ws
+        else:
+            ysel = torch.empty(B, N, Co, dtype=torch.float32, device=dev)
+            arg = torch.empty(B, N, Co, dtype=torch.uint8, device=dev)
+            ssum = torch.empty(B, N, Co, dtype=torch.float32, device=dev) if training else None
+            ws = _lib.workspace("fsg_edgeconv1", B, N, Co, device=dev) if training else None
         if training:
-            ssum = torch.empty(B, N, Co, dtype=torch.float32, device=dev)
             mean = torch.empty(Co, dtype=torch.float32, device=dev)
             invstd = torch.empty(Co, dtype=torch.float32, device=dev)
-            ws = _lib.workspace("fsg_edgeconv1", B, N, Co, device=dev)
         else:
-            ssum, ws = None, None
             mean, invstd = _bn_eval_stats(running_mean, running_var, eps)
         with torch.cuda.device(dev):
             _lib.call("fsg_edgeconv1_fwd_f32", _p(pq), _p(idx), _p(gamma), _p(beta),
                       _p(running_mean if training else None), _p(running_var if training else None), B, N, k, Co,
                       int(training), momentum, eps, slope, _p(None if knn_ws is not None else out), _p(out_pm), _p(ysel), _p(arg),
-                      _p(ssum), _p(mean), _p(invstd), _p(ws), _stream())
+                      _p(ssum), _p(mean), _p(invstd), _p(ws), _stream(), int(given))
             pq_next = _apply_pass(ysel, gamma, beta, mean, invstd, B, N, Co, slope, out, out_pm, knn_ws, w_next)
         ctx.save_for_backward(pq, idx, gamma, beta, mean, invstd, ysel, arg, ssum)
         ctx.meta = (B, N, k, Co, bool(training), slope)
@@ -780,14 +826,15 @@
                       _p(beta), _p(mean),
                       _p(invstd), _p(ysel), _p(arg), _p(ssum), B, N, k, Co, int(training), slope, _p(gpq), _p(dgamma),
                       _p(dbeta), _p(h), _p(ws), _stream())
-        return gpq, None, dgamma, dbeta, None, None, None, None, None, None, None, None
+        return gpq, None, dgamma, dbeta, None, None, None, None, None, None, None, None, None
 
 
 def edgeconv1_supported(out_channels, k):
     return out_channels % 64 == 0 and k <= 64
 
 
-def edgeconv1(x, idx, conv_weight, bn, slope, x_pm=None, both=False, w_cat=None, knn_ws=None, w_next=None, pq_given=None):
+def edgeconv1(x, idx, conv_weight, bn, slope, x_pm=None, both=False, w_cat=None, knn_ws=None, w_next=None, pq_given=None,
+              edge_stats=None):
     _need_gpu(x, idx, conv_weight)
     Co, C2 = conv_weight.shape[0], conv_weight.shape[1]
     C = C2 // 2
@@ -803,7 +850,7 @@
     if idx.dtype != torch.int32:
         idx = idx.to(torch.int32)
     idx = idx.contiguous()
-    res = _EdgeConv1.apply(pq, idx, *bn_args, float(slope), knn_ws, w_next if knn_ws is not None else None)
+    res = _EdgeConv1.apply(pq, idx, *bn_args, float(slope), knn_ws, w_next if knn_ws is not None else None, edge_stats)
     return _edgeconv_outputs(res, both, w_next is not None)
 
 
@@ -811,7 +858,7 @@
     @staticmethod
     @_amp_fwd
     def forward(ctx, pq, idx, w2, g1, b1, rm1, rv1, g2, b2, rm2, rv2, training, mom1, mom2, eps1, eps2, slope, knn_ws=None,
-                w_next=None):
+                w_next=None, edge_stats=None):
         pq, w2 = _f32c(pq), _f32c(w2)
         g1, b1, g2, b2 = _f32c(g1), _f32c(b1), _f32c(g2), _f32c(b2)
         B, N, _ = pq.shape
@@ -821,14 +868,16 @@
             return torch.empty(*shape, dtype=dtype, device=dev)
         out, out_pm = new(B, C2, N), new(B, N, C2)
         ysel2, arg2 = new(B, N, C2), new(B, N, C2, dtype=torch.uint8)
+        given = bool(training) and edge_stats is not None and not edge_stats.select and edge_stats.c2 == C2 and \
+            edge_stats.taken_by(pq, idx, g1, training)
         if training:
-            ssum1, ssum2 = new(B, N, 64), new(B, N, C2)
+            ssum1, ssum2 = edge_stats.ssum if given else new(B, N, 64), new(B, N, C2)
             mean1, invstd1, mean2, invstd2 = new(64), new(64), new(C2), new(C2)
         else:
             ssum1 = ssum2 = None
             mean1, invstd1 = _bn_eval_stats(rm1, rv1, eps1)
             mean2, invstd2 = _bn_eval_stats(rm2, rv2, eps2)
-        ws = _lib.workspace("fsg_edgeconv2", B, N, k, C2, device=dev)
+        ws = edge_stats.ws if given else _lib.workspace("fsg_edgeconv2", B, N, k, C2, device=dev)
         t = bool(training)
         ctx.bf16 = bf16_operands()
         with torch.cuda.device(dev):
@@ -836,7 +885,7 @@
                       _p(rm1 if t else None),
                       _p(rv1 if t else None), _p(g2), _p(b2), _p(rm2 if t else None), _p(rv2 if t else None), B, N, k, C2,
                       int(t), mom1, mom2, eps1, eps2, slope, _p(None if knn_ws is not None else out), _p(out_pm), _p(ssum1), _p(mean1),
-                      _p(invstd1), _p(ysel2), _p(arg2), _p(ssum2), _p(mean2), _p(invstd2), _p(ws), _stream())
+                      _p(invstd1), _p(ysel2), _p(arg2), _p(ssum2), _p(mean2), _p(invstd2), _p(ws), _stream(), int(given))
             pq_next = _apply_pass(ysel2, g2, b2, mean2, invstd2, B, N, C2, slope, out, out_pm, knn_ws, w_next)
         ctx.save_for_backward(pq, idx, w2, g1, b1, mean1, invstd1, ssum1, g2, b2, mean2, invstd2, ysel2, arg2)
         ctx.meta = (B, N, k, C2, t, slope)
@@ -867,7 +916,7 @@
                       _p(b1), _p(mean1), _p(invstd1), _p(ssum1), _p(g2), _p(b2), _p(mean2), _p(invstd2), _p(ysel2),
                       _p(arg2), B, N, k, C2, int(training), slope, _p(gpq), _p(gw2), _p(dg1), _p(db1), _p(dg2), _p(db2),
                       _p(ws), _stream())
-        return (gpq, None, gw2, dg1, db1, None, None, dg2, db2) + (None,) * 10
+        return (gpq, None, gw2, dg1, db1, None, None, dg2, db2) + (None,) * 11
 
 
 def edgeconv2_supported(c_mid, c_out, k):
@@ -889,7 +938,7 @@
 
 
 def edgeconv2(x, idx, conv1_weight, bn1, conv2_weight, bn2, slope, x_pm=None, both=False, w_cat=None, knn_ws=None, w_next=None,
-              pq_given=None):
+              pq_given=None, edge_stats=None):
     _need_gpu(x, idx, conv1_weight, conv2_weight)
     C1, CC = conv1_weight.shape[0], conv1_weight.shape[1]
     C = CC // 2
@@ -911,7 +960,7 @@
     idx = idx.contiguous()
     res = _EdgeConv2.apply(pq, idx, w2, bn1.weight, bn1.bias, bn1.running_mean, bn1.running_var,
                            bn2.weight, bn2.bias, bn2.running_mean, bn2.running_var, t1, m1, m2,
-                           float(bn1.eps), float(bn2.eps), float(slope), knn_ws, w_next if knn_ws is not None else None)
+                           float(bn1.eps), float(bn2.eps), float(slope), knn_ws, w_next if knn_ws is not None else None, edge_stats)
     return _edgeconv_outputs(res, both, w_next is not None)
 
 
diff --git a/fissure-segmentation_amd/models/dgcnn.py b/fissure-segmentation_amd/models/dgcnn.py
--- a/fissure-segmentation_amd/models/dgcnn.py
+++ b/fissure-segmentation_amd/models/dgcnn.py
@@ -80,7 +80,16 @@
         it = iter(ws)
         return [next(it) if b.fused else None for b in blocks]
 
-    def forward(self, x, fixed_knn_graph=None, x_pm=None, both=False, w_cat=None, knn_ws=None, w_next=None, pq_given=None):
+    def edge_stats(self, pq=None):
+        mlp = self.shared_mlp
+        if not self.fused or mlp[0].layers[0].out_channels != 64:
+            return None
+        if len(mlp) == 1:
+            return F_hip.EdgeStats(pq, mlp[0].layers[1], select=True)
+        return F_hip.EdgeStats(pq, mlp[0].layers[1], select=False, c2=mlp[1].layers[0].out_channels)
+
+    def forward(self, x, fixed_knn_graph=None, x_pm=None, both=False, w_cat=None, knn_ws=None, w_next=None, pq_given=None,
+                edge_stats=None):
         if len(self.shared_mlp) == 1 and len(self.shared_mlp[0].layers) == 3 and \
                 F_hip.edgeconv1_supported(self.shared_mlp[0].layers[0].out_channels, self.k):
             graph = fixed_knn_graph
@@ -88,7 +97,7 @@
                 graph = F_hip.knn_graph(x, self.k, c_knn=3 if self.first_layer else None, fix_diag=True)
             conv, bn, act = self.shared_mlp[0].layers
             return F_hip.edgeconv1(x, graph, conv.weight, bn, act.negative_slope, x_pm=x_pm, both=both, w_cat=w_cat,
-                                   knn_ws=knn_ws, w_next=w_next, pq_given=pq_given)
+                                   knn_ws=knn_ws, w_next=w_next, pq_given=pq_given, edge_stats=edge_stats)
         if len(self.shared_mlp) == 2 and all(len(m.layers) == 3 for m in self.shared_mlp) and \
                 F_hip.edgeconv2_supported(self.shared_mlp[0].layers[0].out_channels,
                                           self.shared_mlp[1].layers[0].out_channels, self.k):
@@ -97,7 +106,7 @@
                 graph = F_hip.knn_graph(x, self.k, c_knn=3 if self.first_layer else None, fix_diag=True)
             (conv1, bn1, act), (conv2, bn2, _) = self.shared_mlp[0].layers, self.shared_mlp[1].layers
             return F_hip.edgeconv2(x, graph, conv1.weight, bn1, conv2.weight, bn2, act.negative_slope, x_pm=x_pm,
-                                   both=both, w_cat=w_cat, knn_ws=knn_ws, w_next=w_next, pq_given=pq_given)
+                                   both=both, w_cat=w_cat, knn_ws=knn_ws, w_next=w_next, pq_given=pq_given, edge_stats=edge_stats)
         e = create_neighbor_features(x, self.k, fixed_knn_graph, knn_only_over_coords=self.first_layer)
         for layer in self.shared_mlp:
             e = layer(e)
@@ -206,6 +215,7 @@
         self.ec1 = EdgeConv(self.in_features, [64, 64], k, first_layer=True)
         self.ec2 = EdgeConv(64, [64], k)
         self.ec3 = EdgeConv(64, [64], k)
+        self.fuse_edge_stats = True
         self.global_feature = nn.Sequential(SharedFullyConnected(192, 1024, dim=1), nn.AdaptiveMaxPool1d(1))
         self.segmentation = nn.Sequential(SharedFullyConnected(192 + 1024, 256, dim=1),
                                           SharedFullyConnected(256, 256, dim=1),
@@ -237,12 +247,15 @@
         if self.dynamic and all(e.fused for e in (self.ec1, self.ec2, self.ec3)):
             graphs = list(torch.empty(3, B, N, self.k, dtype=torch.int32, device=x.device).unbind(0))
             ws2, ws3 = F_hip.knn_prep_workspace(B, N, 64, x.device), F_hip.knn_prep_workspace(B, N, 64, x.device)
-            g1, pq1 = F_hip.knn_graph(x, self.k, c_knn=3, fix_diag=True, out=graphs[0], pq_weight=w1)
-            x1, p1, p1c, pq2 = self.ec1(x, g1, both="twice", w_cat=w1, knn_ws=ws2, w_next=w2, pq_given=pq1)
-            g2 = F_hip.knn_graph(x1, self.k, fix_diag=True, out=graphs[1], prepared=None if ws2 is None else (ws2, p1))
-            x2, p2, p2c, pq3 = self.ec2(x1, g2, x_pm=p1, both="twice", w_cat=w2, knn_ws=ws3, w_next=w3, pq_given=pq2)
-            g3 = F_hip.knn_graph(x2, self.k, fix_diag=True, out=graphs[2], prepared=None if ws3 is None else (ws3, p2))
-            _, p3 = self.ec3(x2, g3, x_pm=p2, both=True, w_cat=w3, pq_given=pq3)
+            es1 = self.ec1.edge_stats() if self.fuse_edge_stats else None
+            g1, pq1 = F_hip.knn_graph(x, self.k, c_knn=3, fix_diag=True, out=graphs[0], pq_weight=w1, edge_stats=es1)
+            x1, p1, p1c, pq2 = self.ec1(x, g1, both="twice", w_cat=w1, knn_ws=ws2, w_next=w2, pq_given=pq1, edge_stats=es1)
+            es2 = self.ec2.edge_stats(pq2) if self.fuse_edge_stats and pq2 is not None else None
+            g2 = F_hip.knn_graph(x1, self.k, fix_diag=True, out=graphs[1], prepared=None if ws2 is None else (ws2, p1), edge_stats=es2)
+            x2, p2, p2c, pq3 = self.ec2(x1, g2, x_pm=p1, both="twice", w_cat=w2, knn_ws=ws3, w_next=w3, pq_given=pq2, edge_stats=es2)
+            es3 = self.ec3.edge_stats(pq3) if self.fuse_edge_stats and pq3 is not None else None
+            g3 = F_hip.knn_graph(x2, self.k, fix_diag=True, out=graphs[2], prepared=None if ws3 is None else (ws3, p2), edge_stats=es3)
+            _, p3 = self.ec3(x2, g3, x_pm=p2, both=True, w_cat=w3, pq_given=pq3, edge_stats=es3)
             if torch.is_grad_enabled() and any(p.requires_grad for p in self.parameters()):
                 F_hip.build_reverse_graphs([g1, g2, g3])
         else:
diff --git a/include/fsg_hip.h b/include/fsg_hip.h
--- a/include/fsg_hip.h
+++ b/include/fsg_hip.h
@@ -36,12 +36,24 @@
                          int k, int flags, int32_t *idx_out, float *dist_out, void *workspace,
                          size_t workspace_bytes, fsg_stream_t stream);
 
+typedef struct fsg_knn_edge_stats {
+    const float *pq;
+    int ld;
+    const float *gamma;
+    int training;
+    float *ysel;
+    uint8_t *arg;
+    float *ssum;
+    float *partials;
+    int fused;
+} fsg_knn_edge_stats;
+
 int fsg_knn_dense_ws_pq_f32(const float *x, int B, int N, int64_t stride_b, int64_t stride_c, int c_knn, int k, int flags,
                             int32_t *idx_out, float *dist_out, void *workspace, size_t workspace_bytes, const float *w_pq,
-                            int rows_pq, float *pq_out, fsg_stream_t stream);
+                            int rows_pq, float *pq_out, fsg_stream_t stream, fsg_knn_edge_stats *edge_stats);
 
 int fsg_knn_dense_prepared_f32(const float *x_pm, int B, int N, int c_knn, int k, int flags, int32_t *idx_out, float *dist_out,
-                               void *workspace, size_t workspace_bytes, fsg_stream_t stream);
+                               void *workspace, size_t workspace_bytes, fsg_stream_t stream, fsg_knn_edge_stats *edge_stats);
 
 int fsg_edge_gather_fwd_f32(const float *x, const int32_t *idx, float *edge, int B, int C, int N,
                             int k, fsg_stream_t stream);
@@ -86,7 +98,7 @@
                           float *running_mean, float *running_var, int B, int N, int k, int Co, int training,
                           float momentum, float eps, float slope, float *out, float *out_pm, float *ysel,
                           uint8_t *arg, float *ssum, float *mean, float *invstd, float *workspace,
-                          fsg_stream_t stream);
+                          fsg_stream_t stream, int stats_given);
 int fsg_edgeconv1_bwd_f32(const float *grad_out, const float *grad_out_pm, int64_t ld_pm, const float *grad_out_pm2,
                           int64_t ld_pm2, const float *pq, const int32_t *rowptr, const int32_t *col,
                           const float *gamma, const float *beta, const float *mean, const float *invstd,
@@ -102,7 +114,7 @@
                           int training, float momentum1, float momentum2, float eps1, float eps2, float slope,
                           float *out, float *out_pm, float *ssum1, float *mean1, float *invstd1, float *ysel2,
                           uint8_t *arg2, float *ssum2, float *mean2, float *invstd2, void *workspace,
-                          fsg_stream_t stream);
+                          fsg_stream_t stream, int stats_given);
 int fsg_edgeconv2_bwd_f32(const float *grad_out, const float *grad_out_pm, int64_t ld_pm, const float *grad_out_pm2,
                           int64_t ld_pm2, const float *pq, const int32_t *idx,
                           const int32_t *rowptr, const int32_t *col, const float *w2, const float *gamma1,
@@ -117,7 +129,7 @@
                            int training, float momentum1, float momentum2, float eps1, float eps2, float slope,
                            float *out, float *out_pm, float *ssum1, float *mean1, float *invstd1, float *ysel2,
                            uint8_t *arg2, float *ssum2, float *mean2, float *invstd2, void *workspace,
-                           fsg_stream_t stream);
+                           fsg_stream_t stream, int stats_given);
 int fsg_edgeconv2_bwd_bf16(const float *grad_out, const float *grad_out_pm, int64_t ld_pm, const float *grad_out_pm2,
                            int64_t ld_pm2, const float *pq, const int32_t *idx,
                            const int32_t *rowptr, const int32_t *col, const float *w2, const float *gamma1,
```
